# OCSYT/SoftwareRenderer

Measured on AMD Instinct MI355X. Metric: Mfragments/s (depth-tested + textured fragments, whole frame), higher is better.
Workload: dtype f32; 1 GPU; cfg3: 4096x4096, 1000000 triangles in 16 u16 meshes, 2048^2 RGBA8 nearest texture, program Dust2LambertFog, Back/LessEqual/Alpha; pipelining=1, parallelism=1 GPU

## Files before the change

softwarerenderer_amd/csrc/swr_binning.hip.h:

```cpp
#pragma once
#include "swr_device.h"

#define SWR_ORDER_BUCKETS 256

namespace swr {

struct BinArgs {
    const unsigned long long* __restrict__ slot_tb;
    const TriRec* __restrict__ recs;
    uint32_t slot_lo, slot_hi;
    uint32_t spt;
    int tiles_x;
    int band_ty0, band_ty1;
    BandMap band;
    int width, height;
    uint32_t* __restrict__ tile_count;
    const uint32_t* __restrict__ tile_start;
    uint32_t* __restrict__ tile_list;
    uint32_t list_capacity;
    Counters* __restrict__ counters;
    Ctrl* __restrict__ ctrl;
    uint32_t seq;
    uint32_t replayable;
    const unsigned long long* __restrict__ total;
    uint8_t* __restrict__ want;
    uint32_t tpw;
    uint32_t bin_blocks;
    int order_tiles_y;
    const uint8_t* __restrict__ tile_bucket;
    const uint32_t* __restrict__ order_hist;
    uint32_t* __restrict__ order_cursor;
    uint4* __restrict__ tile_order;
};

__device__ __forceinline__ bool pair_may_cover(const float sx[3], const float sy[3], int minX, int maxX, int minY, int maxY,
                                               int tx, int ty, int width, int height, bool is_line) {
    if (is_line) return true;
    const int x0 = tx * SWR_TILE, y0 = ty * SWR_TILE;
    const int startX = max(minX, x0), endX = min(maxX, min(x0 + SWR_TILE - 1, width - 1));
    const int startY = max(minY, y0), endY = min(maxY, min(y0 + SWR_TILE - 1, height - 1));
    if (startX > endX || startY > endY) return false;
    const float ea[3] = { sy[1] - sy[2], sy[2] - sy[0], sy[0] - sy[1] };
    const float eb[3] = { sx[2] - sx[1], sx[0] - sx[2], sx[1] - sx[0] };
    const float rx[3] = { sx[1], sx[2], sx[0] };
    const float ry[3] = { sy[1], sy[2], sy[0] };
    const float fxs = (float)startX, fxe = (float)endX, fys = (float)startY, fye = (float)endY;
    const float lim = 1.0e15f;
    const bool tame = fabsf(sx[0]) < lim && fabsf(sx[1]) < lim && fabsf(sx[2]) < lim && fabsf(sy[0]) < lim && fabsf(sy[1]) < lim && fabsf(sy[2]) < lim;
    if (!tame) return true;
    bool any_neg = false, any_pos = false;
#pragma unroll
    for (int k = 0; k < 3; ++k) {
        const float a = ea[k], b = eb[k];
        const float dxs = fxs - rx[k], dxe = fxe - rx[k], dys = fys - ry[k], dye = fye - ry[k];
        const float ax_s = a * dxs, ax_e = a * dxe, by_s = b * dys, by_e = b * dye;
        const float emax = fmaxf(ax_s, ax_e) + fmaxf(by_s, by_e);
        const float emin = fminf(ax_s, ax_e) + fminf(by_s, by_e);
        const float m = fabsf(a) * fmaxf(fabsf(dxs), fabsf(dxe)) + fabsf(b) * fmaxf(fabsf(dys), fabsf(dye));
        const float delta = m * (64.0f / 16777216.0f);
        any_neg = any_neg || emax < -delta;
        any_pos = any_pos || emin > delta;
    }
    return !(any_neg && any_pos);
}

__device__ __forceinline__ void bin_overflow(const BinArgs& a) {
    a.counters->overflow = 1u;
    if (a.ctrl->host_flag) __hip_atomic_store(a.ctrl->host_flag + 1, 1u, __ATOMIC_RELAXED, __HIP_MEMORY_SCOPE_SYSTEM);
    if (a.replayable) {
        atomicMin(&a.ctrl->first_bad, a.seq);
        atomicMax(&a.ctrl->need, 2ull * (unsigned long long)a.list_capacity + 4096ull);
        __hip_atomic_store(&a.ctrl->poison, 1u, __ATOMIC_RELAXED, __HIP_MEMORY_SCOPE_AGENT);
        if (a.ctrl->host_flag) __hip_atomic_store(a.ctrl->host_flag, 1u, __ATOMIC_RELAXED, __HIP_MEMORY_SCOPE_SYSTEM);
    }
}

__device__ __forceinline__ uint32_t order_bucket(uint32_t w) {
    if (w == 0u) return 0u;
    const int e = 31 - __clz((int)w);
    const uint32_t m = e >= 3 ? ((w >> (e - 3)) & 7u) : ((w << (3 - e)) & 7u);
    return min((uint32_t)(e * 8) + m + 1u, (uint32_t)SWR_ORDER_BUCKETS - 1u);
}
__device__ __forceinline__ uint32_t tile_weight(uint32_t frags, uint32_t pairs) { return frags + 16u * pairs; }

__device__ __forceinline__ uint32_t order_tile_of_thread(uint32_t block, int tiles_x, int tiles_y) {
    const int sbx = (tiles_x + 15) >> 4;
    const int bx = (int)(block % (uint32_t)sbx), by = (int)(block / (uint32_t)sbx);
    const int t = threadIdx.x, q = t >> 6, w = t & 63;
    const int tx = bx * 16 + (q & 1) * 8 + (w & 7), ty = by * 16 + (q >> 1) * 8 + (w >> 3);
    return (tx < tiles_x && ty < tiles_y) ? (uint32_t)(ty * tiles_x + tx) : 0xffffffffu;
}
__host__ __device__ inline uint32_t order_blocks(int tiles_x, int tiles_y) { return (uint32_t)(((tiles_x + 15) / 16) * ((tiles_y + 15) / 16)); }

__device__ __forceinline__ void tile_place_block(const BinArgs& a, uint32_t block, uint32_t* s_suf, uint32_t* s_cnt) {
    const uint32_t t = threadIdx.x;
    s_suf[t] = a.order_hist[t];
    s_cnt[t] = 0u;
    __syncthreads();
    for (uint32_t off = 1; off < (uint32_t)SWR_ORDER_BUCKETS; off <<= 1) {
        const uint32_t v = t + off < (uint32_t)SWR_ORDER_BUCKETS ? s_suf[t + off] : 0u;
        __syncthreads();
        s_suf[t] += v;
        __syncthreads();
    }
    const uint32_t i = order_tile_of_thread(block, a.tiles_x, a.order_tiles_y);
    uint32_t b = 0, rank = 0;
    if (i != 0xffffffffu) {
        b = a.tile_bucket[i];
        rank = atomicAdd(&s_cnt[b], 1u);
    }
    __syncthreads();
    const uint32_t mine = s_cnt[t];
    __syncthreads();
    if (mine) s_cnt[t] = (s_suf[t] - a.order_hist[t]) + atomicAdd(&a.order_cursor[t], mine);
    __syncthreads();
    if (i != 0xffffffffu) {
        const uint32_t n_tiles = (uint32_t)(a.tiles_x * a.order_tiles_y);
        const uint32_t st = a.tile_start[i];
        const unsigned long long nxt = i + 1u < n_tiles ? (unsigned long long)a.tile_start[i + 1u] : *a.total;
        a.tile_order[s_cnt[b] + rank] = make_uint4(i, st, (uint32_t)(nxt - st), 0u);
    }
}

struct SlotData {
    int tminx, tminy, nx, ny;
    float sx[3], sy[3];
    int minX, maxX, minY, maxY;
    bool is_line;
};
__device__ __forceinline__ SlotData slot_none() {
    SlotData s;
    s.tminx = s.tminy = s.nx = s.ny = 0;
    s.sx[0] = s.sx[1] = s.sx[2] = s.sy[0] = s.sy[1] = s.sy[2] = 0.f;
    s.minX = s.minY = 0; s.maxX = s.maxY = -1; s.is_line = false;
    return s;
}
__device__ __forceinline__ bool slot_tiles(const BinArgs& a, unsigned long long tb, SlotData& s) {
    if (tb == SWR_TB_INVALID) return false;
    s.tminx = (int)(tb & 0xffff);
    const int tmaxx = (int)((tb >> 16) & 0xffff);
    s.tminy = max((int)((tb >> 32) & 0xffff), a.band_ty0);
    const int tmaxy = min((int)((tb >> 48) & 0xffff), a.band_ty1 - 1);
    s.nx = tmaxx - s.tminx + 1;
    s.ny = tmaxy - s.tminy + 1;
    if (s.ny <= 0) { s.nx = 0; s.ny = 0; return false; }
    return true;
}
__device__ __forceinline__ SlotData slot_load(const BinArgs& a, uint32_t slot, unsigned long long tb, bool with_rec_small) {
    SlotData s = slot_none();
    if (slot_tiles(a, tb, s) && (with_rec_small || s.nx * s.ny > 8)) {
        const float4* __restrict__ rq = reinterpret_cast<const float4*>(a.recs + slot);
        const float4 r0 = rq[0], r1 = rq[1], r3 = rq[3];
        s.sx[0] = r0.x; s.sx[1] = r0.y; s.sx[2] = r0.z; s.sy[0] = r0.w; s.sy[1] = r1.x; s.sy[2] = r1.y;
        const uint32_t bbx = __float_as_uint(r3.y), bby = __float_as_uint(r3.z);
        s.minX = (int)(bbx & 0xffffu); s.maxX = (int)(bbx >> 16); s.minY = (int)(bby & 0xffffu); s.maxY = (int)(bby >> 16);
        s.is_line = (__float_as_uint(r3.w) & SWR_FLAG_LINE) != 0u;
    }
    return s;
}

template <bool FILL>
__device__ __forceinline__ void bin_big(const BinArgs& a, const SlotData& sd, uint32_t slot, bool big) {
    const int lane = threadIdx.x & 63;
    const int nt = sd.nx * sd.ny;
    unsigned long long med = __ballot(big && nt <= 64);
    while (med) {
        bool want[4];
        uint32_t tile[4], sslot[4], base[4];
#pragma unroll
        for (int j = 0; j < 4; ++j) {
            want[j] = false; tile[j] = 0u; sslot[j] = 0u; base[j] = 0u;
            if (med) {
                const int src = __ffsll((long long)med) - 1;
                med &= med - 1;
                const int s_tminx = __shfl(sd.tminx, src), s_tminy = __shfl(sd.tminy, src);
                const int s_nx = __shfl(sd.nx, src), s_nt = __shfl(nt, src);
                sslot[j] = (uint32_t)__shfl((int)slot, src);
                float bsx[3], bsy[3];
#pragma unroll
                for (int k = 0; k < 3; ++k) { bsx[k] = __shfl(sd.sx[k], src); bsy[k] = __shfl(sd.sy[k], src); }
                const int bminX = __shfl(sd.minX, src), bmaxX = __shfl(sd.maxX, src), bminY = __shfl(sd.minY, src), bmaxY = __shfl(sd.maxY, src);
                const bool b_line = __shfl((int)sd.is_line, src) != 0;
                if (lane < s_nt) {
                    const int ty = s_tminy + lane / s_nx, tx = s_tminx + lane % s_nx;
                    want[j] = band_local_row(a.band, ty) >= 0 && pair_may_cover(bsx, bsy, bminX, bmaxX, bminY, bmaxY, tx, ty, a.width, a.height, b_line);
                    tile[j] = (uint32_t)(band_local_row(a.band, ty) * a.tiles_x + tx);
                }
                if (want[j]) {
                    if (FILL) base[j] = atomicAdd(&a.tile_count[tile[j]], 1u);
                    else atomicAdd(&a.tile_count[tile[j]], 1u);
                }
            }
        }
        if (FILL) {
#pragma unroll
            for (int j = 0; j < 4; ++j) {
                if (want[j]) {
                    const uint32_t at = a.tile_start[tile[j]] + base[j];
                    if (at < a.list_capacity) a.tile_list[at] = sslot[j];
                    else bin_overflow(a);
                }
            }
        }
    }
    unsigned long long m = __ballot(big && nt > 64);
    while (m) {
        const int src = __ffsll((long long)m) - 1;
        m &= m - 1;
        const int s_tminx = __shfl(sd.tminx, src), s_tminy = __shfl(sd.tminy, src);
        const int s_nx = __shfl(sd.nx, src), s_nt = __shfl(nt, src);
        const uint32_t s_slot = (uint32_t)__shfl((int)slot, src);
        float bsx[3], bsy[3];
#pragma unroll
        for (int k = 0; k < 3; ++k) { bsx[k] = __shfl(sd.sx[k], src); bsy[k] = __shfl(sd.sy[k], src); }
        const int bminX = __shfl(sd.minX, src), bmaxX = __shfl(sd.maxX, src), bminY = __shfl(sd.minY, src), bmaxY = __shfl(sd.maxY, src);
        const bool b_line = __shfl((int)sd.is_line, src) != 0;
        for (int i0 = 0; i0 < s_nt; i0 += 64) {
            const int i = i0 + lane;
            bool want = i < s_nt;
            int ty = 0, tx = 0;
            if (want) {
                ty = s_tminy + i / s_nx; tx = s_tminx + i % s_nx;
                want = band_local_row(a.band, ty) >= 0 && pair_may_cover(bsx, bsy, bminX, bmaxX, bminY, bmaxY, tx, ty, a.width, a.height, b_line);
            }
            if (want) {
                const uint32_t tile = (uint32_t)(band_local_row(a.band, ty) * a.tiles_x + tx);
                if (FILL) {
                    const uint32_t at = a.tile_start[tile] + atomicAdd(&a.tile_count[tile], 1u);
                    if (at < a.list_capacity) a.tile_list[at] = s_slot;
                    else bin_overflow(a);
                } else {
                    atomicAdd(&a.tile_count[tile], 1u);
                }
            }
        }
    }
}

#define SWR_BIN_TABLE_LOG2 8
#define SWR_BIN_TABLE (1 << SWR_BIN_TABLE_LOG2)
template <bool FILL>
__device__ __forceinline__ void bin_block_slots(const BinArgs& a, uint32_t slot, unsigned long long tb, uint32_t want_in, uint32_t* s_key, uint32_t* s_val) {
    const SlotData sd = slot_load(a, slot, tb, !FILL);
    const int nt = sd.nx * sd.ny;
    const bool big = nt > 8;
    const int nt_small = big ? 0 : nt;
    if (!__syncthreads_or(nt != 0)) return;
    for (int e = threadIdx.x; e < SWR_BIN_TABLE; e += 256) { s_key[e] = 0u; s_val[e] = 0u; }
    __syncthreads();
    uint32_t packed[8];
    int wtx = sd.tminx, wty = sd.tminy;
    uint32_t wmask = (FILL && nt_small) ? want_in : 0u;
#pragma unroll
    for (int i = 0; i < 8; ++i) {
        packed[i] = 0u;
        if (i < nt_small) {
            bool want;
            if (FILL) want = ((wmask >> i) & 1u) != 0u;
            else {
                want = band_local_row(a.band, wty) >= 0 && pair_may_cover(sd.sx, sd.sy, sd.minX, sd.maxX, sd.minY, sd.maxY, wtx, wty, a.width, a.height, sd.is_line);
                wmask |= want ? (1u << i) : 0u;
            }
            if (want) {
                const uint32_t tile = (uint32_t)(band_local_row(a.band, wty) * a.tiles_x + wtx);
                uint32_t e = (tile * 0x9E3779B1u) >> (32 - SWR_BIN_TABLE_LOG2);
                bool placed = false;
                for (int probe = 0; probe < 16; ++probe) {
                    const uint32_t prev = atomicCAS(&s_key[e], 0u, tile + 1u);
                    if (prev == 0u || prev == tile + 1u) { placed = true; break; }
                    e = (e + 1u) & (SWR_BIN_TABLE - 1u);
                }
                if (placed) {
                    const uint32_t rank = atomicAdd(&s_val[e], 1u);
                    packed[i] = e | (rank << 12) | 0x80000000u;
                } else if (FILL) {
                    const uint32_t at = a.tile_start[tile] + atomicAdd(&a.tile_count[tile], 1u);
                    if (at < a.list_capacity) a.tile_list[at] = slot;
                    else bin_overflow(a);
                } else {
                    atomicAdd(&a.tile_count[tile], 1u);
                }
            }
            ++wtx;
            if (wtx >= sd.tminx + sd.nx) { wtx = sd.tminx; ++wty; }
        }
    }
    if (!FILL && nt_small) a.want[slot] = (uint8_t)wmask;
    __syncthreads();
    for (int e = threadIdx.x; e < SWR_BIN_TABLE; e += 256) {
        const uint32_t key = s_key[e];
        if (key) {
            const uint32_t tile = key - 1u, n = s_val[e];
            if (FILL) s_val[e] = a.tile_start[tile] + atomicAdd(&a.tile_count[tile], n);
            else atomicAdd(&a.tile_count[tile], n);
        }
    }
    if (FILL) {
        __syncthreads();
#pragma unroll
        for (int i = 0; i < 8; ++i) {
            if (packed[i] & 0x80000000u) {
                const uint32_t at = s_val[packed[i] & 0xfffu] + ((packed[i] >> 12) & 0x7ffffu);
                if (at < a.list_capacity) a.tile_list[at] = slot;
                else bin_overflow(a);
            }
        }
    }
    bin_big<FILL>(a, sd, slot, big);
}

template <bool FILL>
__global__ __launch_bounds__(256) void k_bin(BinArgs a) {
    SWR_FRONT_ENTER();
    __shared__ uint32_t s_key[SWR_BIN_TABLE];
    __shared__ uint32_t s_val[SWR_BIN_TABLE];
    if (FILL && batch_poisoned(a.ctrl, a.seq)) return;
    if (FILL && blockIdx.x >= a.bin_blocks) {
        static_assert(SWR_BIN_TABLE >= SWR_ORDER_BUCKETS, "tile_place_block borrows the hash table's LDS");
        tile_place_block(a, blockIdx.x - a.bin_blocks, s_key, s_val);
        return;
    }
    const uint32_t wave_id = (blockIdx.x * 256u + threadIdx.x) >> 6, lane_id = threadIdx.x & 63u;
    const bool has_tri = lane_id < a.tpw;
    const uint32_t first = a.slot_lo + (wave_id * a.tpw + lane_id) * a.spt;
    auto in_round = [&](uint32_t si) { return has_tri && si < a.spt && first + si < a.slot_hi; };
    auto tb_of = [&](uint32_t si) { return in_round(si) ? a.slot_tb[first + si] : SWR_TB_INVALID; };
    auto want_of = [&](uint32_t si) { return (FILL && in_round(si)) ? (uint32_t)a.want[first + si] : 0u; };
    unsigned long long tb = tb_of(0);
    uint32_t wm = want_of(0);
    for (uint32_t si = 0; si < a.spt; ++si) {
        const unsigned long long tb_next = tb_of(si + 1);
        const uint32_t wm_next = want_of(si + 1);
        bin_block_slots<FILL>(a, first + si, tb, wm, s_key, s_val);
        tb = tb_next; wm = wm_next;
    }
}

#define SWR_SCAN_BLOCK 256
__device__ __forceinline__ unsigned long long block_sum(unsigned long long v, unsigned long long* s_part) {
#pragma unroll
    for (int off = 32; off > 0; off >>= 1) {
        unsigned lo = (unsigned)v, hi = (unsigned)(v >> 32);
        v += ((unsigned long long)(unsigned)__shfl_xor((int)hi, off) << 32) | (unsigned)__shfl_xor((int)lo, off);
    }
    if ((threadIdx.x & 63u) == 0u) s_part[threadIdx.x >> 6] = v;
    __syncthreads();
    unsigned long long t = 0;
    for (int w = 0; w < SWR_SCAN_BLOCK / 64; ++w) t += s_part[w];
    return t;
}

__global__ __launch_bounds__(SWR_SCAN_BLOCK) void k_scan_sums(const uint32_t* __restrict__ count, uint32_t n,
                                                    unsigned long long* __restrict__ sums) {
    SWR_FRONT_ENTER();
    __shared__ unsigned long long s_part[SWR_SCAN_BLOCK / 64];
    const uint32_t i = blockIdx.x * (uint32_t)SWR_SCAN_BLOCK + threadIdx.x;
    const unsigned long long t = block_sum(i < n ? count[i] : 0u, s_part);
    if (threadIdx.x == 0) sums[blockIdx.x] = t;
}

__global__ __launch_bounds__(SWR_SCAN_BLOCK) void k_scan_apply(uint32_t* __restrict__ count, uint32_t* __restrict__ start,
                                                     uint32_t n, const unsigned long long* __restrict__ sums,
                                                     unsigned long long* __restrict__ total_out,
                                                     unsigned long long capacity, uint32_t seq, Ctrl* __restrict__ ctrl,
                                                     Counters* __restrict__ counters, int poison_on_overflow,
                                                     const uint32_t* __restrict__ tile_work, uint32_t* __restrict__ order_hist,
                                                     uint8_t* __restrict__ tile_bucket) {
    SWR_FRONT_ENTER();
    __shared__ unsigned long long s_part[SWR_SCAN_BLOCK / 64];
    __shared__ unsigned long long s_wave[SWR_SCAN_BLOCK / 64];
    __shared__ uint32_t s_oh[SWR_ORDER_BUCKETS];
    static_assert(SWR_ORDER_BUCKETS <= SWR_SCAN_BLOCK, "one thread per bucket clears / flushes the block's histogram");
    const uint32_t tid = threadIdx.x, lane = tid & 63u, wv = tid >> 6;
    if (tid < (uint32_t)SWR_ORDER_BUCKETS) s_oh[tid] = 0u;
    unsigned long long mine = 0ull;
    for (uint32_t j = tid; j < blockIdx.x; j += (uint32_t)SWR_SCAN_BLOCK) mine += sums[j];
    const unsigned long long off = block_sum(mine, s_part);
    const uint32_t i = blockIdx.x * (uint32_t)SWR_SCAN_BLOCK + tid;
    const uint32_t c = i < n ? count[i] : 0u;
    if (i < n) {
        const uint32_t ob = order_bucket(tile_weight(tile_work[i], c));
        tile_bucket[i] = (uint8_t)ob;
        atomicAdd(&s_oh[ob], 1u);
    }
    unsigned long long incl = c;
#pragma unroll
    for (int o = 1; o < 64; o <<= 1) {
        unsigned lo = (unsigned)incl, hi = (unsigned)(incl >> 32);
        unsigned long long v = ((unsigned long long)(unsigned)__shfl_up((int)hi, o) << 32) | (unsigned)__shfl_up((int)lo, o);
        if (lane >= (uint32_t)o) incl += v;
    }
    if (lane == 63u) s_wave[wv] = incl;
    __syncthreads();
    if (tid < (uint32_t)SWR_ORDER_BUCKETS && s_oh[tid]) atomicAdd(&order_hist[tid], s_oh[tid]);
    unsigned long long wave_off = 0;
    for (uint32_t w = 0; w < wv; ++w) wave_off += s_wave[w];
    const unsigned long long excl = off + wave_off + incl - c;
    if (i < n) {
        start[i] = (uint32_t)min(excl, 0xffffffffull);
        count[i] = 0u;
    }
    if (blockIdx.x == gridDim.x - 1 && tid == (uint32_t)SWR_SCAN_BLOCK - 1u) {
        const unsigned long long total = excl + c;
        *total_out = total;
        if (total > capacity) {
            if (!poison_on_overflow) return;
            atomicMin(&ctrl->first_bad, seq);
            atomicMax(&ctrl->need, total);
            __hip_atomic_store(&ctrl->poison, 1u, __ATOMIC_RELAXED, __HIP_MEMORY_SCOPE_AGENT);
            if (ctrl->host_flag) __hip_atomic_store(ctrl->host_flag, 1u, __ATOMIC_RELAXED, __HIP_MEMORY_SCOPE_SYSTEM);
        } else if (poison_on_overflow && !batch_poisoned(ctrl, seq)) {
            atomicAdd(&counters->tile_pairs, total);
        }
    }
}

#define SWR_SORT_LDS 2048

__device__ __forceinline__ void cmpx_lds(uint32_t* s, uint32_t i, uint32_t p, uint32_t n) {
    if (p < n) {
        uint32_t a = s[i], b = s[p];
        if (a > b) { s[i] = b; s[p] = a; }
    }
}
__device__ __forceinline__ void cmpx_glb(uint32_t* g, uint32_t i, uint32_t p, uint32_t n) {
    if (p < n) {
        uint32_t a = g[i], b = g[p];
        if (a > b) { g[i] = b; g[p] = a; }
    }
}

#define SWR_SORT_TPB 1
#define SWR_SORT_TPW 4
#define SWR_SORT_WAVE_SYNC() do { __builtin_amdgcn_fence(__ATOMIC_ACQ_REL, "workgroup"); __builtin_amdgcn_wave_barrier(); } while (0)
__device__ __forceinline__ void sort_tile(uint32_t n, uint32_t start, uint32_t* __restrict__ tile_list, uint32_t tile,
                                          uint32_t* __restrict__ pair_tile, uint32_t* s_keys, uint32_t key_in) {
    if (n == 0) return;
    const uint32_t lane = threadIdx.x & 63u;
    for (uint32_t i = lane; i < n; i += 64) pair_tile[start + i] = tile;
    if (n < 2) return;
    uint32_t* seg = tile_list + start;

    if (n <= 64) {
        uint32_t key = lane < n ? key_in : 0xffffffffu;
#define SWR_CMPX(other_expr, lower_cond) { const uint32_t other = (uint32_t)(other_expr); \
                                            key = (lower_cond) ? min(key, other) : max(key, other); }
#define SWR_DPP(ctrl) __builtin_amdgcn_update_dpp(0, (int)key, ctrl, 0xf, 0xf, false)
#define SWR_XOR1  SWR_CMPX(SWR_DPP(0xB1), (lane & 1u) == 0u)
#define SWR_XOR2  SWR_CMPX(SWR_DPP(0x4E), (lane & 2u) == 0u)
#define SWR_XOR4  { const int up = SWR_DPP(0x124), dn = SWR_DPP(0x12C);               \
                    SWR_CMPX((lane & 4u) ? up : dn, (lane & 4u) == 0u) }
#define SWR_XOR8  SWR_CMPX(SWR_DPP(0x128), (lane & 8u) == 0u)
#define SWR_XOR16 SWR_CMPX(__shfl((int)key, (int)(lane ^ 16u)), (lane & 16u) == 0u)
        SWR_XOR1
        SWR_CMPX(SWR_DPP(0x1B), (lane & 2u) == 0u) SWR_XOR1
        SWR_CMPX(SWR_DPP(0x141), (lane & 4u) == 0u) SWR_XOR2 SWR_XOR1
        SWR_CMPX(SWR_DPP(0x140), (lane & 8u) == 0u) SWR_XOR4 SWR_XOR2 SWR_XOR1
        SWR_CMPX(__shfl((int)key, (int)(lane ^ 31u)), (lane & 16u) == 0u) SWR_XOR8 SWR_XOR4 SWR_XOR2 SWR_XOR1
        SWR_CMPX(__shfl((int)key, (int)(lane ^ 63u)), (lane & 32u) == 0u) SWR_XOR16 SWR_XOR8 SWR_XOR4 SWR_XOR2 SWR_XOR1
#undef SWR_XOR16
#undef SWR_XOR8
#undef SWR_XOR4
#undef SWR_XOR2
#undef SWR_XOR1
#undef SWR_DPP
#undef SWR_CMPX
        if (lane < n) seg[lane] = key;
        return;
    }

    uint32_t m = 1;
    while (m < n) m <<= 1;
    const bool in_lds = n <= SWR_SORT_LDS;
    uint32_t* buf = in_lds ? s_keys : seg;
    if (in_lds) {
        for (uint32_t i = lane; i < n; i += 64) s_keys[i] = seg[i];
        SWR_SORT_WAVE_SYNC();
    }
    for (uint32_t k = 2; k <= m; k <<= 1) {
        for (uint32_t t = lane; t < (m >> 1); t += 64) {
            uint32_t blk = t / (k >> 1), off = t % (k >> 1);
            uint32_t i = blk * k + off, p = blk * k + (k - 1 - off);
            if (i < n) { if (in_lds) cmpx_lds(buf, i, p, n); else cmpx_glb(buf, i, p, n); }
        }
        SWR_SORT_WAVE_SYNC();
        for (uint32_t j = k >> 2; j > 0; j >>= 1) {
            for (uint32_t t = lane; t < (m >> 1); t += 64) {
                uint32_t i = 2 * j * (t / j) + (t % j), p = i + j;
                if (i < n) { if (in_lds) cmpx_lds(buf, i, p, n); else cmpx_glb(buf, i, p, n); }
            }
            SWR_SORT_WAVE_SYNC();
        }
    }
    if (in_lds) {
        for (uint32_t i = lane; i < n; i += 64) seg[i] = s_keys[i];
    }
}

__global__ __launch_bounds__(64 * SWR_SORT_TPB) void k_sort_tiles(const uint32_t* __restrict__ tile_start,
                                                   const uint32_t* __restrict__ tile_count,
                                                   uint32_t* __restrict__ tile_list, uint32_t n_tiles,
                                                   uint32_t* __restrict__ pair_tile, const Ctrl* __restrict__ ctrl, uint32_t seq,
                                                   const uint4* __restrict__ tile_order ) {
    SWR_FRONT_ENTER();
    __shared__ uint32_t s_keys_all[SWR_SORT_TPB][SWR_SORT_LDS];
    static_assert(sizeof(s_keys_all) <= SWR_FRONT_MAX_LDS, "k_sort_tiles must fit beside the raster kernel (swr_device.h)");
    if (batch_poisoned(ctrl, seq)) return;
    static_assert(SWR_SORT_TPW <= 64, "one lane per tile of the wave fetches its count and start");
    const uint32_t first = (blockIdx.x * SWR_SORT_TPB + (threadIdx.x >> 6)) * SWR_SORT_TPW;
    const uint32_t lane = threadIdx.x & 63u;
    const uint32_t waves = gridDim.x * SWR_SORT_TPB, entry = (first / SWR_SORT_TPW) + lane * waves;
    const bool mine = lane < SWR_SORT_TPW && entry < n_tiles;
    const uint4 desc_l = mine ? tile_order[entry] : make_uint4(0u, 0u, 0u, 0u);
    const uint32_t tile_l = desc_l.x;
    const uint32_t cnt_l = desc_l.z, st_l = desc_l.y;
    uint32_t keys[SWR_SORT_TPW];
#pragma unroll
    for (int t = 0; t < SWR_SORT_TPW; ++t) {
        const uint32_t n = (uint32_t)__builtin_amdgcn_readlane((int)cnt_l, t), start = (uint32_t)__builtin_amdgcn_readlane((int)st_l, t);
        keys[t] = (lane < n && n <= 64u) ? tile_list[start + lane] : 0xffffffffu;
    }
#pragma unroll
    for (int t = 0; t < SWR_SORT_TPW; ++t) {
        const uint32_t n = (uint32_t)__builtin_amdgcn_readlane((int)cnt_l, t), start = (uint32_t)__builtin_amdgcn_readlane((int)st_l, t);
        sort_tile(n, start, tile_list, (uint32_t)__builtin_amdgcn_readlane((int)tile_l, t), pair_tile, s_keys_all[threadIdx.x >> 6], keys[t]);
        SWR_SORT_WAVE_SYNC();
    }
}

}
```

softwarerenderer_amd/csrc/swr_device.h:

```cpp
#pragma once

#ifndef __HIPCC_RTC__
#include <hip/hip_runtime.h>
#include <stdint.h>
#endif
#include "swr.h"

#ifndef SWR_NUMERICS_FMA
#define SWR_NUMERICS_FMA 0
#endif
#define SWR_NM_TRANSFORM_FMA        1u
#define SWR_NM_TRANSFORM_NORMAL_FMA 2u
#ifndef SWR_DOT_PAIRWISE
#define SWR_DOT_PAIRWISE 0
#endif

#define SWR_PROG_CUSTOM 5
#define SWR_TILE 16
#define SWR_FLOAT_MINVALUE (-3.40282347e+38f)
#define SWR_EPSILON 1e-6f
#define SWR_FLAG_INTERP 0x80000000u
#define SWR_FLAG_LINE   0x40000000u
#define SWR_FLAG_FASTDIV 0x20000000u
#define SWR_FLAG_SIMPLE 0x10000000u
#define SWR_DRAW_MASK   0x0fffffffu
#define SWR_INFO_SIMPLE 0x80000000u

#define SWR_TB_INVALID 0xffffffffffffffffull

#define SWR_FRONT_MAX_LDS 10240
#define SWR_FRONT_MAX_VGPRS 96
#define SWR_RASTER_MAX_VGPRS 104
#define SWR_FRONT_ENTER() __builtin_amdgcn_s_setprio(3)
#define SWR_GEOM_BLOCK 128

namespace swr {

struct VOut {
    float clip[4];
    float color[4];
    float uv[2];
    float wn[3];
    float wpos[3];
};
static_assert(sizeof(VOut) == 64, "VOut must be 64 bytes");

struct TriRec {
    float sx[3], sy[3];
    float depth[3];
    float inv_area;
    uint32_t vref[3];
    uint32_t bbox_x;
    uint32_t bbox_y;
    uint32_t draw_flags;
};
static_assert(sizeof(TriRec) == 64, "TriRec must be 64 bytes");

struct DrawParams {
    float model[16], view[16], proj[16];
    swr_uniforms u;
    const swr_vertex* verts;
    const uint16_t* idx;
    const uint8_t* tex;
    int tex_w, tex_h;
    int program, cull, depth_test, blend;
    uint32_t n_verts, n_tris;
    uint32_t vert_base;
    uint32_t tri_base;
    float fog_r1;
    float tex_wf, tex_hf;
    float fog_den;
    uint32_t frag_draw;
    uint32_t nm_flags;
};
static_assert(offsetof(DrawParams, fog_den) == offsetof(DrawParams, fog_r1) + 12, "k_vertex writes fog_den three floats after fog_r1");

struct Counters {
    unsigned long long triangles_in, triangles_setup, triangles_clipped;
    unsigned long long fragments_tested, fragments_shaded, fragments_written;
    unsigned long long tile_pairs;
    unsigned int overflow;
    unsigned int pad;
};

struct Ctrl {
    uint32_t poison;
    uint32_t first_bad;
    unsigned long long need;
    uint32_t* host_flag;
};
__device__ __forceinline__ bool batch_poisoned(const Ctrl* __restrict__ c, uint32_t seq) { return c->first_bad <= seq; }

struct FrameParams {
    int width, height;
    int tiles_x, tiles_y;
    int band_ty0, band_ty1;
    int band_y0;
    int band_rows;
    int il_k, il_world, il_rank;
    int band_tile_rows;
    float near_clip;
};

struct BandMap { int ty0, ty1, il_k, il_world, il_rank; };
__host__ __device__ __forceinline__ int band_local_row(const BandMap& b, int ty) {
    if (b.il_k <= 0) return (ty >= b.ty0 && ty < b.ty1) ? ty - b.ty0 : -1;
    const int stripe = ty / b.il_k;
    if (stripe % b.il_world != b.il_rank) return -1;
    return (stripe / b.il_world) * b.il_k + (ty - stripe * b.il_k);
}
__host__ __device__ __forceinline__ int band_global_row(const BandMap& b, int local) {
    if (b.il_k <= 0) return b.ty0 + local;
    const int ls = local / b.il_k;
    return (ls * b.il_world + b.il_rank) * b.il_k + (local - ls * b.il_k);
}
__host__ __device__ __forceinline__ BandMap band_map(const FrameParams& fp) {
    BandMap b; b.ty0 = fp.band_ty0; b.ty1 = fp.band_ty1; b.il_k = fp.il_k; b.il_world = fp.il_world; b.il_rank = fp.il_rank;
    return b;
}

__device__ __forceinline__ bool is_neg_bits(float f) { return (__float_as_uint(f) >> 31) != 0u; }
__device__ __forceinline__ bool is_nan(float f) { return f != f; }
__device__ __forceinline__ bool is_nan_or_inf(float f) { return (__float_as_uint(f) & 0x7f800000u) == 0x7f800000u; }

__device__ __forceinline__ int f2i(float f) {
    int r;
    asm("v_cvt_i32_f32 %0, %1" : "=v"(r) : "v"(f));
    return r;
}
__device__ __forceinline__ float mathf_min(float a, float b) {
    if (a != b) { if (!is_nan(a)) return a < b ? a : b; return a; }
    return is_neg_bits(a) ? a : b;
}
__device__ __forceinline__ float mathf_max(float a, float b) {
    if (a != b) { if (!is_nan(a)) return b < a ? a : b; return a; }
    return is_neg_bits(b) ? a : b;
}
__device__ __forceinline__ float math_clamp(float v, float lo, float hi) {
    if (v < lo) return lo;
    else if (v > hi) return hi;
    return v;
}

__device__ __forceinline__ float rcp_refined(float d) {
    const float r0 = __builtin_amdgcn_rcpf(d);
    const float e = __builtin_fmaf(-d, r0, 1.0f);
    return __builtin_fmaf(e, r0, r0);
}
__device__ __forceinline__ float div_core(float n, float d, float r1) {
    const float q0 = n * r1;
    const float e2 = __builtin_fmaf(-d, q0, n);
    const float q1 = __builtin_fmaf(e2, r1, q0);
    const float e3 = __builtin_fmaf(-d, q1, n);
    return __builtin_fmaf(e3, r1, q1);
}
#define SWR_DIV_LO_BITS 0x2B800000u
#define SWR_DIV_HI_BITS 0x53800000u
__device__ __forceinline__ bool div_operand_safe(float v) {
    return __builtin_fabsf(v) >= 0x1p-40f && __builtin_fabsf(v) <= 0x1p40f;
}
__device__ __forceinline__ bool div_operands_safe3(float a, float b, float c) {
    const uint32_t ua = __float_as_uint(a) & 0x7fffffffu, ub = __float_as_uint(b) & 0x7fffffffu, uc = __float_as_uint(c) & 0x7fffffffu;
    return min(min(ua, ub), uc) >= SWR_DIV_LO_BITS && max(max(ua, ub), uc) <= SWR_DIV_HI_BITS;
}
__device__ __forceinline__ bool div_operands_safe3_arith(float a, float b, float c) {
    const float fa = __builtin_fabsf(a), fb = __builtin_fabsf(b), fc = __builtin_fabsf(c);
    const float sum = (fa + fb) + fc;
    const float lo = __builtin_fminf(__builtin_fminf(fa, fb), fc);
    return lo >= 0x1p-40f && sum <= 0x1p40f;
}
#define SWR_RCP_HI_BITS 0x69000000u
__device__ __forceinline__ float recip_core(float d) {
    const float r1 = rcp_refined(d);
    const float e2 = __builtin_fmaf(-d, r1, 1.0f);
    const float q1 = __builtin_fmaf(e2, r1, r1);
    const float e3 = __builtin_fmaf(-d, q1, 1.0f);
    return __builtin_fmaf(e3, r1, q1);
}
__device__ __forceinline__ float sqrt_core(float x) {
    const float s = __builtin_amdgcn_sqrtf(x);
    const float sd = __uint_as_float(__float_as_uint(s) - 1u), su = __uint_as_float(__float_as_uint(s) + 1u);
    const float rd = __builtin_fmaf(-sd, s, x), ru = __builtin_fmaf(-su, s, x);
    float r = rd <= 0.0f ? sd : s;
    r = ru > 0.0f ? su : r;
    return r;
}

template <bool FUSED>
__device__ __forceinline__ float nm_madd(float a, float b, float c) {
    if (FUSED) return __builtin_fmaf(a, b, c);
    float p = a * b;
    return p + c;
}
template <bool FUSED>
__device__ __forceinline__ void vec4_transform_t(const float v[4], const float* __restrict__ m, float out[4]) {
#pragma unroll
    for (int j = 0; j < 4; ++j) {
        float r = m[j] * v[0];
        r = nm_madd<FUSED>(m[4 + j], v[1], r);
        r = nm_madd<FUSED>(m[8 + j], v[2], r);
        r = nm_madd<FUSED>(m[12 + j], v[3], r);
        out[j] = r;
    }
}
template <bool FUSED>
__device__ __forceinline__ void vec3_transform_normal_t(const float n[3], const float* __restrict__ m, float out[3]) {
#pragma unroll
    for (int j = 0; j < 3; ++j) {
        float r = m[j] * n[0];
        r = nm_madd<FUSED>(m[4 + j], n[1], r);
        r = nm_madd<FUSED>(m[8 + j], n[2], r);
        out[j] = r;
    }
}
__device__ __forceinline__ void vec4_transform(const float v[4], const float* __restrict__ m, float out[4], bool fused) {
    if (fused) vec4_transform_t<true>(v, m, out); else vec4_transform_t<false>(v, m, out);
}
__device__ __forceinline__ void vec3_transform_normal(const float n[3], const float* __restrict__ m, float out[3], bool fused) {
    if (fused) vec3_transform_normal_t<true>(n, m, out); else vec3_transform_normal_t<false>(n, m, out);
}
__device__ __forceinline__ float dot3(float ax, float ay, float az, float bx, float by, float bz) {
#if SWR_DOT_PAIRWISE == 1
    const float p = ax * bx + ay * by, q = az * bz + 0.0f;
    return p + q;
#elif SWR_DOT_PAIRWISE == 2
    const float p = ax * bx + az * bz, q = ay * by + 0.0f;
    return p + q;
#else
    return (ax * bx + ay * by) + az * bz;
#endif
}
__device__ __forceinline__ float nm_lerp(float a, float b, float t) {
#if SWR_NUMERICS_FMA
    return __builtin_fmaf(a, 1.0f - t, b * t);
#else
    float x = a * (1.0f - t);
    float y = b * t;
    return x + y;
#endif
}

__device__ __forceinline__ float edge_function(float ax, float ay, float bx, float by, float cx, float cy) {
    float p = (cx - ax) * (by - ay);
    float q = (cy - ay) * (bx - ax);
    return p - q;
}

__device__ __forceinline__ bool depth_func(int test, float nd, float od) {
    switch (test) {
    case SWR_DEPTH_LESSEQUAL:    return nd >= od;
    case SWR_DEPTH_LESS:         return nd > od;
    case SWR_DEPTH_GREATER:      return nd < od;
    case SWR_DEPTH_GREATEREQUAL: return nd <= od;
    case SWR_DEPTH_EQUAL:        return fabsf(nd - od) < SWR_EPSILON;
    case SWR_DEPTH_NOTEQUAL:     return fabsf(nd - od) >= SWR_EPSILON;
    default:                     return true;
    }
}

__device__ __forceinline__ float4 blend(float4 s, float4 d, int mode) {
    float4 o;
    switch (mode) {
    case SWR_BLEND_ALPHA: {
        float a = s.w, ia = 1.0f - s.w;
        float x;
        x = s.x * a; o.x = x + d.x * ia;
        x = s.y * a; o.y = x + d.y * ia;
        x = s.z * a; o.z = x + d.z * ia;
        x = s.w * a; o.w = x + d.w * ia;
        return o; }
    case SWR_BLEND_ADDITIVE:
        o.x = mathf_min(s.x + d.x, 1.0f); o.y = mathf_min(s.y + d.y, 1.0f);
        o.z = mathf_min(s.z + d.z, 1.0f); o.w = mathf_min(s.w + d.w, 1.0f);
        return o;
    case SWR_BLEND_MULTIPLY:
        o.x = s.x * d.x; o.y = s.y * d.y; o.z = s.z * d.z; o.w = s.w * d.w;
        return o;
    default:
        return s;
    }
}

__device__ __forceinline__ bool line_test(float p0x, float p0y, float p1x, float p1y, int x, int y, float& t_out) {
    const float dx = p1x - p0x, dy = p1y - p0y;
    const float len_sq = dx * dx + dy * dy;
    const float px = (float)x + 0.5f - p0x, py = (float)y + 0.5f - p0y;
    float t = 0.0f;
    if (len_sq > 0) t = (px * dx + py * dy) / len_sq;
    t = mathf_max(0.0f, mathf_min(1.0f, t));
    const float cx = p0x + t * dx, cy = p0y + t * dy;
    const float ddx = ((float)x + 0.5f) - cx, ddy = ((float)y + 0.5f) - cy;
    const float dist_sq = ddx * ddx + ddy * ddy;
    t_out = t;
    return dist_sq <= 0.5f * 0.5f;
}

__device__ __forceinline__ float4 texture_unpack(uint32_t p) {
    const float inv255 = 1.0f / 255.0f;
    float4 o;
    o.x = (float)(p & 0xffu) * inv255;
    o.y = (float)((p >> 8) & 0xffu) * inv255;
    o.z = (float)((p >> 16) & 0xffu) * inv255;
    o.w = (float)(p >> 24) * inv255;
    return o;
}
__device__ __forceinline__ uint32_t texture_nearest_index(int w, int h, float wf, float hf, float tu, float tv) {
    float u = tu - (float)f2i(tu);
    float v = tv - (float)f2i(tv);
    u += (u < 0) ? 1.0f : 0.0f;
    v += (v < 0) ? 1.0f : 0.0f;
    int x = f2i(u * wf);
    int y = f2i(v * hf);
    if ((uint32_t)x >= (uint32_t)w) { x = (x == w) ? 0 : x % w; if (x < 0) x += w; }
    if ((uint32_t)y >= (uint32_t)h) { y = (y == h) ? 0 : y % h; if (y < 0) y += h; }
    return (uint32_t)y * (uint32_t)w + (uint32_t)x;
}
__device__ __forceinline__ uint32_t texture_nearest_index(int w, int h, float tu, float tv) {
    return texture_nearest_index(w, h, (float)w, (float)h, tu, tv);
}
__device__ __forceinline__ float4 texture_sample(const uint8_t* __restrict__ tex, int w, int h, float tu, float tv) {
    return texture_unpack(reinterpret_cast<const uint32_t*>(tex)[texture_nearest_index(w, h, tu, tv)]);
}

template <bool BLOCKED>
__device__ __forceinline__ uint32_t bilinear_texel_offset(int w, int x, int y) {
    if (BLOCKED) return ((((uint32_t)y >> 2) * ((uint32_t)w >> 2) + ((uint32_t)x >> 2)) << 4) + (((uint32_t)y & 3u) << 2) + ((uint32_t)x & 3u);
    return (uint32_t)y * (uint32_t)w + (uint32_t)x;
}
template <bool BLOCKED>
__device__ __forceinline__ float4 texture_sample_bilinear(const uint8_t* __restrict__ tex, int w, int h, float tu, float tv) {
    const float x = tu * (float)w - 0.5f, y = tv * (float)h - 0.5f;
    const float x0 = floorf(x), y0 = floorf(y);
    const float fx = x - x0, fy = y - y0;
    int ix0 = f2i(x0) % w; if (ix0 < 0) ix0 += w;
    int iy0 = f2i(y0) % h; if (iy0 < 0) iy0 += h;
    const int ix1 = ix0 + 1 == w ? 0 : ix0 + 1, iy1 = iy0 + 1 == h ? 0 : iy0 + 1;
    const uint32_t* __restrict__ t32 = reinterpret_cast<const uint32_t*>(tex);
    const uint32_t p00 = t32[bilinear_texel_offset<BLOCKED>(w, ix0, iy0)];
    const uint32_t p10 = t32[bilinear_texel_offset<BLOCKED>(w, ix1, iy0)];
    const uint32_t p01 = t32[bilinear_texel_offset<BLOCKED>(w, ix0, iy1)];
    const uint32_t p11 = t32[bilinear_texel_offset<BLOCKED>(w, ix1, iy1)];
    const float inv255 = 1.0f / 255.0f;
    float o[4];
#pragma unroll
    for (int c = 0; c < 4; ++c) {
        const float c00 = (float)((p00 >> (8 * c)) & 0xffu) * inv255, c10 = (float)((p10 >> (8 * c)) & 0xffu) * inv255;
        const float c01 = (float)((p01 >> (8 * c)) & 0xffu) * inv255, c11 = (float)((p11 >> (8 * c)) & 0xffu) * inv255;
        const float top = c00 * (1.0f - fx) + c10 * fx;
        const float bot = c01 * (1.0f - fx) + c11 * fx;
        o[c] = top * (1.0f - fy) + bot * fy;
    }
    return make_float4(o[0], o[1], o[2], o[3]);
}
__device__ __forceinline__ float4 texture_fetch(const uint8_t* __restrict__ tex, int w_signed, int h_signed, float tu, float tv) {
    if (h_signed >= 0) return texture_sample(tex, w_signed, h_signed, tu, tv);
    return w_signed < 0 ? texture_sample_bilinear<true>(tex, -w_signed, -h_signed, tu, tv) : texture_sample_bilinear<false>(tex, w_signed, -h_signed, tu, tv);
}

}
```

softwarerenderer_amd/csrc/swr_flush.h:

```cpp
#pragma once
#include "swr_raster_select.h"

namespace {
int kernel_class(int program) { return program == SWR_PROG_DEBUG_VARYINGS || program >= SWR_PROG_USER_BASE ? program : 0; }

void destroy_mesh(swr_mesh* m) {
    if (m->d_verts) (void)hipFree(m->d_verts);
    if (m->d_idx) (void)hipFree(m->d_idx);
    if (m->d_bounds) (void)hipFree(m->d_bounds);
    delete m;
}
const size_t kMeshPoolBytes = (size_t)1 << 30;
void trim_mesh_pool(swr_context* c) {
    while (c->mesh_pool_bytes > kMeshPoolBytes && !c->mesh_pool.empty()) {
        swr_mesh* m = c->mesh_pool.front();
        c->mesh_pool.erase(c->mesh_pool.begin());
        c->mesh_pool_bytes -= m->cap_verts + m->cap_idx;
        destroy_mesh(m);
    }
}
void pool_mesh(swr_context* c, swr_mesh* m) {
    c->mesh_pool.push_back(m);
    c->mesh_pool_bytes += m->cap_verts + m->cap_idx;
    if (c->mesh_pool_bytes > 2 * kMeshPoolBytes) trim_mesh_pool(c);
}
void free_garbage(swr_context* c) {
    for (swr_mesh* m : c->garbage) pool_mesh(c, m);
    c->garbage.clear();
    c->prog_garbage.clear();
    trim_mesh_pool(c);
}

int validate_locked(swr_context* c);

int drain_streams(swr_context* c) {
    SWR_HIP(c, hipStreamSynchronize(c->stream));
    if (c->front_stream) SWR_HIP(c, hipStreamSynchronize(c->front_stream));
    for (auto& s : c->sets) s.raster_pending = false;
    c->f_tail_pending = c->r_front_pending = false;
    return SWR_OK;
}

int sync_locked(swr_context* c) {
    ++c->host_syncs;
    int rc = drain_streams(c);
    if (rc) return rc;
    rc = validate_locked(c);
    collect_spans(c);
    free_garbage(c);
    for (auto& fs : c->slots) fs.busy = false;
    return rc;
}

enum { MODE_SYNC = 0, MODE_ASYNC = 1 };
struct UploadLayout { size_t off_vb, off_tb, off_bp, off_vis, off_consts, bytes; };
static UploadLayout upload_layout(size_t nd, size_t v_blocks, size_t t_blocks, bool any_cull, bool user) {
    const auto r256 = [](size_t x) { return (x + 255) & ~(size_t)255; };
    UploadLayout u;
    u.off_vb = r256(nd * sizeof(DrawParams));
    u.off_tb = r256(u.off_vb + v_blocks * sizeof(BlockMap));
    u.off_bp = r256(u.off_tb + t_blocks * sizeof(BlockMap));
    u.off_vis = r256(u.off_bp + (any_cull ? nd * sizeof(void*) : 0));
    const size_t vis_end = u.off_vis + (any_cull ? nd * 4 : 0);
    u.off_consts = r256(vis_end);
    u.bytes = user ? u.off_consts + nd * 64 * sizeof(float) : vis_end;
    return u;
}
template <class T> T* at(void* base, size_t off) { return reinterpret_cast<T*>(static_cast<char*>(base) + off); }

struct OrderView { uint4* tile_order; uint32_t* tile_work; uint32_t* hist; uint32_t* cursor; uint8_t* tile_bucket; };
static size_t order_bytes(uint32_t n_tiles) { return (size_t)n_tiles * (sizeof(uint4) + 4 + 1 + 4) + 2 * SWR_ORDER_BUCKETS * 4; }
static OrderView order_view(RasterSet& S, uint32_t n_tiles) {
    uint4* order = S.d_order.as<uint4>();
    uint32_t* work = reinterpret_cast<uint32_t*>(order + n_tiles), *hist = work + n_tiles, *cursor = hist + SWR_ORDER_BUCKETS;
    return { order, work, hist, cursor, reinterpret_cast<uint8_t*>(cursor + SWR_ORDER_BUCKETS) };
}

struct Pass {
    const Batch& b;
    RasterSet& S;
    hipStream_t F;
    int mode;
    bool cc, cd;
    UploadLayout up = {};
};

static bool b_needs_vnorm(const Batch& b) { return !b.draws.empty() && kernel_class(b.draws[0].p.program) != 0; }
static bool b_has_user_program(const Batch& b) { return !b.draws.empty() && b.draws[0].p.program >= SWR_PROG_USER_BASE; }
static bool b_has_user_vertex(const Batch& b) { return b_has_user_program(b) && b.draws[0].prog && b.draws[0].prog->vertex_fn; }
const unsigned long long kMaxPairs = 1ull << 30;

size_t pair_capacity(const swr_context* c) {
    size_t cap = std::min(c->d_tile_list.cap / 4, c->d_pair_tile.cap / 4);
    for (int i = 0; i < (c->pipelining ? 2 : 1); ++i) {
        const RasterSet& s = c->sets[i];
        cap = std::min(cap, std::min(std::min(s.d_masks.cap / 32, s.d_pcounts.cap / 8), s.d_pair_refs.cap / 16));
    }
    return cap;
}
int ensure_pairs(swr_context* c, size_t n) {
    int rc;
    if ((rc = ensure(c, c->d_tile_list, n * 4))) return rc;
    if ((rc = ensure(c, c->d_pair_tile, n * 4))) return rc;
    for (int i = 0; i < (c->pipelining ? 2 : 1); ++i) {
        RasterSet& s = c->sets[i];
        if ((rc = ensure(c, s.d_masks, n * 32))) return rc;
        if ((rc = ensure(c, s.d_pair_refs, n * 16))) return rc;
        if ((rc = ensure(c, s.d_pcounts, n * 8 + 64))) return rc;
    }
    return SWR_OK;
}

int run_clear(swr_context* c, const Batch& b, bool& cc, bool& cd) {
    size_t n = band_pixels(c);
    if (n && (cc || cd)) {
        ScopedSpan sp(c, ST_CLEAR);
        int blocks = (int)std::min<size_t>((n + 255) / 256, 2048 * 8);
        float4 rgba = make_float4(b.clear_rgba[0], b.clear_rgba[1], b.clear_rgba[2], b.clear_rgba[3]);
        hipLaunchKernelGGL(k_clear, dim3(blocks), dim3(256), 0, c->stream, b.color, b.depth, n, rgba,
                           cc ? 1 : 0, cd ? 1 : 0, (const Ctrl*)c->d_ctrl.as<Ctrl>(), b.seq);
        SWR_HIP(c, hipGetLastError());
    }
    cc = cd = false;
    return SWR_OK;
}

int launch_raster(swr_context* c, Pass& P, uint32_t n_tiles);

int bin_and_raster(swr_context* c, Pass& P, uint32_t lo, uint32_t hi, bool counts_clear = false) {
    const uint32_t n_tiles = (uint32_t)c->tiles_x * (uint32_t)c->band_tile_rows;
    if (n_tiles == 0 || lo >= hi) return SWR_OK;
    int rc;
    const Batch& b = P.b; RasterSet& S = P.S;
    const hipStream_t F = P.F; const int mode = P.mode;
    const Ctrl* ctrl = c->d_ctrl.as<Ctrl>();
    unsigned long long* d_total = c->d_total.as<unsigned long long>();
    const OrderView ov = order_view(S, n_tiles);
    BinArgs ba;
    ba.slot_tb = c->d_slot_tb.as<unsigned long long>();
    ba.recs = S.d_recs.as<TriRec>();
    ba.slot_lo = lo; ba.slot_hi = hi;
    ba.spt = b.wireframe ? 6u : 2u;
    ba.width = c->W; ba.height = c->H;
    ba.tiles_x = c->tiles_x; ba.band_ty0 = c->band_ty0; ba.band_ty1 = c->band_ty1;
    ba.band = host_band_map(c);
    ba.tile_count = S.d_tile_count.as<uint32_t>();
    ba.tile_start = S.d_tile_start.as<uint32_t>();
    ba.tile_list = c->d_tile_list.as<uint32_t>();
    ba.list_capacity = (uint32_t)std::min<size_t>(pair_capacity(c), 0xffffffffu);
    ba.counters = c->d_counters.as<Counters>();
    ba.ctrl = c->d_ctrl.as<Ctrl>();
    ba.seq = b.seq; ba.replayable = mode == MODE_ASYNC ? 1u : 0u;
    ba.total = c->d_total.as<unsigned long long>();
    ba.want = c->d_want.as<uint8_t>();
    const uint32_t bin_threads = (hi - lo + ba.spt - 1u) / ba.spt;
    ba.tpw = 64u;
    while (ba.tpw > 4u && bin_threads < ba.tpw * 1024u) ba.tpw >>= 1;
    const uint32_t bin_blocks = (bin_threads + 4u * ba.tpw - 1u) / (4u * ba.tpw);
    {
        ScopedSpan sp(c, ST_BIN, F);
        if (!counts_clear) {
            SWR_HIP(c, hipMemsetAsync(ba.tile_count, 0, (size_t)n_tiles * 4, F));
            SWR_HIP(c, hipMemsetAsync(ov.hist, 0, 2 * SWR_ORDER_BUCKETS * 4, F));
        }
        hipLaunchKernelGGL(k_bin<false>, dim3(bin_blocks), dim3(256), 0, F, ba);
        const unsigned scan_blocks = (n_tiles + (unsigned)SWR_SCAN_BLOCK - 1u) / (unsigned)SWR_SCAN_BLOCK;
        unsigned long long* sums = d_total + 32;
        hipLaunchKernelGGL(k_scan_sums, dim3(scan_blocks), dim3(SWR_SCAN_BLOCK), 0, F, (const uint32_t*)ba.tile_count, n_tiles, sums);
        const unsigned long long cap = mode == MODE_ASYNC ? (unsigned long long)ba.list_capacity : ~0ull;
        hipLaunchKernelGGL(k_scan_apply, dim3(scan_blocks), dim3(SWR_SCAN_BLOCK), 0, F, ba.tile_count,
                           S.d_tile_start.as<uint32_t>(), n_tiles, (const unsigned long long*)sums, d_total,
                           cap, b.seq, c->d_ctrl.as<Ctrl>(), c->d_counters.as<Counters>() + 64,
                           mode == MODE_ASYNC ? 1 : 0, (const uint32_t*)ov.tile_work, ov.hist, ov.tile_bucket);
        SWR_HIP(c, hipGetLastError());
    }
    uint32_t cover_items = ba.list_capacity;
    if (mode == MODE_SYNC) {
        unsigned long long total = 0;
        SWR_HIP(c, hipMemcpyAsync(&total, d_total, 8, hipMemcpyDeviceToHost, F));
        SWR_HIP(c, hipStreamSynchronize(F));
        if (total > kMaxPairs && hi - lo > 2) {
            uint32_t mid = lo + (((hi - lo) / 2u) & ~1u);
            if (mid == lo) mid = lo + 2;
            if ((rc = bin_and_raster(c, P, lo, mid))) return rc;
            return bin_and_raster(c, P, mid, hi);
        }
        if (total == 0) return run_clear(c, b, P.cc, P.cd);
        if (total > 0xffffffffull) return fail(c, SWR_ERR_UNSUPPORTED, "a single triangle covers more tile pairs than one round can hold");
        c->host_tile_pairs += total;
        if ((rc = ensure_pairs(c, (size_t)std::min<unsigned long long>(total + total / 4 + 4096, std::max(total, kMaxPairs))))) return rc;
        ba.tile_list = c->d_tile_list.as<uint32_t>();
        ba.list_capacity = (uint32_t)std::min<size_t>(pair_capacity(c), 0xffffffffu);
        cover_items = (uint32_t)total;
    }
    {
        ScopedSpan sp(c, ST_BIN, F);
        BinArgs bf = ba;
        if (mode == MODE_ASYNC && c->debug_fill_capacity) bf.list_capacity = std::min(bf.list_capacity, c->debug_fill_capacity);
        bf.bin_blocks = bin_blocks;
        bf.order_tiles_y = c->band_tile_rows;
        bf.tile_bucket = ov.tile_bucket; bf.order_hist = ov.hist; bf.order_cursor = ov.cursor; bf.tile_order = ov.tile_order;
        hipLaunchKernelGGL(k_bin<true>, dim3(bin_blocks + order_blocks(c->tiles_x, c->band_tile_rows)), dim3(256), 0, F, bf);
        SWR_HIP(c, hipGetLastError());
    }
    {
        ScopedSpan sp(c, ST_SORT, F);
        hipLaunchKernelGGL(k_sort_tiles, dim3((n_tiles + SWR_SORT_TPB * SWR_SORT_TPW - 1u) / (SWR_SORT_TPB * SWR_SORT_TPW)), dim3(64 * SWR_SORT_TPB), 0, F, S.d_tile_start.as<uint32_t>(),
                           S.d_tile_count.as<uint32_t>(), c->d_tile_list.as<uint32_t>(), n_tiles, c->d_pair_tile.as<uint32_t>(), ctrl, b.seq,
                           (const uint4*)ov.tile_order);
        SWR_HIP(c, hipGetLastError());
    }
    if (cover_items) {
        ScopedSpan sp(c, ST_COVER, F);
        CoverArgs ca;
        ca.recs = S.d_recs.as<TriRec>();
        ca.tile_list = c->d_tile_list.as<uint32_t>();
        ca.pair_tile = c->d_pair_tile.as<uint32_t>();
        ca.masks = S.d_masks.as<uint4>();
        ca.info = S.d_pcounts.as<uint2>();
        ca.refs = S.d_pair_refs.as<uint4>();
        ca.n_pairs = d_total;
        ca.ctrl = ctrl; ca.seq = b.seq;
        ca.fp = frame_params(c, b.near_clip);
        ca.dbg = d_total + 8;
        const dim3 cg((unsigned)((((cover_items + (uint32_t)SWR_COVER_BLOCK - 1u) / (uint32_t)SWR_COVER_BLOCK) + 7u) & ~7u)), cb(SWR_COVER_BLOCK);
        if (b.wireframe) hipLaunchKernelGGL(k_cover<true>, cg, cb, 0, F, ca);
        else hipLaunchKernelGGL(k_cover<false>, cg, cb, 0, F, ca);
        SWR_HIP(c, hipGetLastError());
    }
    if (F != c->stream) {
        SWR_HIP(c, hipEventRecord(S.front_done, F));
        SWR_HIP(c, hipStreamWaitEvent(c->stream, S.front_done, 0));
    } else if (c->pipelining && mode == MODE_ASYNC) {
        SWR_HIP(c, hipEventRecord(c->r_front_ev, c->stream));
        c->r_front_pending = true;
    }
    if ((rc = launch_raster(c, P, n_tiles))) return rc;
    if (c->pipelining && S.raster_done) {
        SWR_HIP(c, hipEventRecord(S.raster_done, c->stream));
        S.raster_pending = true;
    }
    return SWR_OK;
}

int launch_raster(swr_context* c, Pass& P, uint32_t n_tiles) {
    const Batch& b = P.b; RasterSet& S = P.S;
    const OrderView ov = order_view(S, n_tiles);
    ScopedSpan sp(c, ST_RASTER);
    RasterArgs ra;
    ra.fp = frame_params(c, b.near_clip);
    ra.recs = S.d_recs.as<TriRec>();
    ra.vout = S.d_vout.as<VOut>();
    ra.vout_bytes = (uint32_t)std::min<size_t>(S.d_vout.cap, 0xfffffff0u);
    ra.vnorm = b_needs_vnorm(b) ? S.d_vnorm.as<float4>() : nullptr;
    ra.user_consts = b_has_user_program(b) ? at<const float>(S.d_upload.p, P.up.off_consts) : nullptr;
    ra.draws = at<const DrawParams>(S.d_upload.p, 0);
    ra.tile_start = S.d_tile_start.as<uint32_t>();
    ra.tile_count = S.d_tile_count.as<uint32_t>();
    ra.pair_refs = S.d_pair_refs.as<uint4>();
    ra.color = b.color; ra.depth = b.depth;
    ra.tile_stats = c->d_tile_stats.as<uint32_t>();
    memcpy(ra.clear_rgba, b.clear_rgba, 16);
    ra.clear_color_on = P.cc ? 1 : 0;
    ra.clear_depth_on = P.cd ? 1 : 0;
    ra.tile_order = ov.tile_order;
    ra.tile_work = ov.tile_work;
    ra.n_tiles = n_tiles;
    ra.dbg = c->d_total.as<unsigned long long>() + 8;
    ra.ctrl = c->d_ctrl.as<Ctrl>(); ra.seq = b.seq;
    RasterTraits traits;
    traits.wireframe = b.wireframe;
    for (auto& d : b.draws) traits.add(d.p.program, d.p.blend, d.p.depth_test);
    ra.depth_only_grows = traits.depth_only_grows ? 1 : 0;
    const RasterKernel kernel = select_raster_kernel(traits);
    using RasterFn = void (*)(RasterArgs, const uint4*, const uint2*);
    static const RasterFn table[] = {
        k_raster_c<false, true, SWR_PROG_DEBUG_VARYINGS, -1, -1, true>,
        k_raster_c<false, true, SWR_PROG_DEBUG_VARYINGS>,
        k_raster_c<true, true>,
        k_raster_c<false, true, -1, -1, -1, true>,
        k_raster_c<false, true, SWR_PROG_PHONG_4POINT, SWR_BLEND_ALPHA, SWR_DEPTH_LESSEQUAL>,
        k_raster_c<false, true>,
        k_raster_c<false, false, SWR_PROG_DUST2_LAMBERT_FOG, SWR_BLEND_ALPHA, SWR_DEPTH_LESSEQUAL>,
        k_raster_c<false, false, SWR_PROG_GOURAUD, SWR_BLEND_ALPHA, SWR_DEPTH_LESSEQUAL>,
        k_raster_c<false, false>,
    };
    static_assert(sizeof table / sizeof table[0] == (size_t)RasterKernel::user, "one kernel per built-in RasterKernel, in its order");
    const dim3 g((n_tiles + 511u) & ~511u), t(64);
    const uint4* mk = (const uint4*)S.d_masks.as<uint4>();
    const uint2* pc = (const uint2*)S.d_pcounts.as<uint2>();
    if (kernel == RasterKernel::user || kernel == RasterKernel::user_none) {
        void* args[] = { &ra, &mk, &pc };
        hipFunction_t fn = b.draws[0].prog->fn[kernel == RasterKernel::user_none ? 1 : 0];
        SWR_HIP(c, hipModuleLaunchKernel(fn, g.x, 1, 1, t.x, 1, 1, 0, c->stream, args, nullptr));
    } else {
        hipLaunchKernelGGL(table[(int)kernel], g, t, 0, c->stream, ra, mk, pc);
    }
    SWR_HIP(c, hipGetLastError());
    P.cc = P.cd = false;
    return SWR_OK;
}

struct BatchGeometry {
    std::vector<DrawParams> hp;
    std::vector<BlockMap> vblocks, tblocks;
    uint64_t V = 0, T = 0; bool any_cull = false;
};
static BatchGeometry batch_geometry(const Batch& b) {
    BatchGeometry g;
    const size_t nd = b.draws.size();
    g.hp.resize(nd);
    std::vector<uint32_t> frag_reps;
    for (size_t i = 0; i < nd; ++i) {
        DrawParams p = b.draws[i].p;
        p.vert_base = (uint32_t)g.V; p.tri_base = (uint32_t)g.T;
        for (uint32_t f = 0; f < p.n_verts; f += SWR_GEOM_BLOCK) g.vblocks.push_back({ (uint32_t)i, f });
        for (uint32_t f = 0; f < p.n_tris; f += SWR_GEOM_BLOCK) g.tblocks.push_back({ (uint32_t)i, f });
        g.V += p.n_verts; g.T += p.n_tris;
        g.any_cull = g.any_cull || b.draws[i].frustum_cull;
        p.frag_draw = (uint32_t)i;
        for (uint32_t j : frag_reps) {
            const DrawParams& q = g.hp[j];
            if (q.program == p.program && q.blend == p.blend && q.depth_test == p.depth_test && q.tex == p.tex && q.tex_w == p.tex_w &&
                q.tex_h == p.tex_h && memcmp(&q.u, &p.u, sizeof p.u) == 0 &&
                (p.program < SWR_PROG_USER_BASE || *b.draws[j].uconsts == *b.draws[i].uconsts)) { p.frag_draw = j; break; }
        }
        if (p.frag_draw == (uint32_t)i && p.n_verts > 0 && !b.draws[i].frustum_cull && frag_reps.size() < 64) frag_reps.push_back((uint32_t)i);
        g.hp[i] = p;
    }
    return g;
}

int launch_geometry(swr_context* c, const Pass& P, const BatchGeometry& g, uint32_t n_tiles, int count_stats) {
    const Batch& b = P.b; RasterSet& S = P.S; const hipStream_t F = P.F;
    const UserProg* vprog = b_has_user_vertex(b) ? b.draws[0].prog.get() : nullptr;
    const auto launch = [&](hipFunction_t user_fn, const void* builtin, size_t blocks, void** args) {
        return user_fn ? hipModuleLaunchKernel(user_fn, (unsigned)blocks, 1, 1, SWR_GEOM_BLOCK, 1, 1, 0, F, args, nullptr)
                       : hipLaunchKernel(builtin, dim3((unsigned)blocks), dim3(SWR_GEOM_BLOCK), args, 0, F);
    };
    const uint32_t nd = (uint32_t)b.draws.size();
    const DrawParams* d_draws = at<const DrawParams>(S.d_upload.p, 0);
    const BlockMap* d_vblocks = at<const BlockMap>(S.d_upload.p, P.up.off_vb);
    const BlockMap* d_tblocks = at<const BlockMap>(S.d_upload.p, P.up.off_tb);
    const uint32_t* d_visible = nullptr;
    if (g.any_cull) {
        ScopedSpan sp(c, ST_VERTEX, F);
        uint32_t* vis = at<uint32_t>(S.d_upload.p, P.up.off_vis);
        hipLaunchKernelGGL(k_frustum_cull, dim3((nd + 63) / 64), dim3(64), 0, F, d_draws,
                           at<const float4* const>(S.d_upload.p, P.up.off_bp), nd, vis);
        SWR_HIP(c, hipGetLastError());
        d_visible = vis;
    }
    float4* a_vnorm = b_needs_vnorm(b) ? S.d_vnorm.as<float4>() : (float4*)nullptr;
    if (!g.vblocks.empty()) {
        ScopedSpan sp(c, ST_VERTEX, F);
        VOut* a_vout = S.d_vout.as<VOut>();
        float* a_fog = at<float>(S.d_upload.p, offsetof(DrawParams, fog_r1));
        uint32_t* a_zero = S.d_tile_count.as<uint32_t>();
        uint32_t a_n_zero = n_tiles;
        uint32_t* a_hist = order_view(S, n_tiles).hist;
        const float* a_consts = at<const float>(S.d_upload.p, P.up.off_consts);
        void* args[] = { &d_draws, &d_vblocks, &a_vout, &d_visible, &a_fog, &a_vnorm, &a_zero, &a_n_zero, &a_hist, &a_consts };
        SWR_HIP(c, launch(vprog ? vprog->vertex_fn : nullptr, (const void*)k_vertex, g.vblocks.size(), args));
    }
    {
        ScopedSpan sp(c, ST_SETUP, F);
        FrameParams fp = frame_params(c, b.near_clip);
        const VOut* a_vout = S.d_vout.as<VOut>();
        VOut* a_pool = S.d_vout.as<VOut>() + g.V;
        uint32_t a_pool_base = (uint32_t)g.V;
        TriRec* a_recs = S.d_recs.as<TriRec>();
        unsigned long long* a_tb = c->d_slot_tb.as<unsigned long long>();
        Counters* a_counters = c->d_counters.as<Counters>();
        const Ctrl* a_ctrl = c->d_ctrl.as<Ctrl>();
        uint32_t a_seq = b.seq;
        int a_count = count_stats, a_wire = b.wireframe ? 1 : 0;
        void* args[] = { &d_draws, &d_tblocks, &a_vout, &a_pool, &a_pool_base, &a_recs, &a_tb, &fp, &a_counters, &a_ctrl, &a_seq,
                         &a_count, &a_wire, &d_visible, &a_vnorm };
        SWR_HIP(c, launch(vprog ? vprog->setup_fn : nullptr, (const void*)k_setup, g.tblocks.size(), args));
    }
    return SWR_OK;
}

int execute_batch(swr_context* c, const Batch& b, int mode, int count_stats) {
    bool cc = b.clear_color, cd = b.clear_depth;
    if (b.draws.empty()) return run_clear(c, b, cc, cd);
    int rc;
    if ((rc = ensure_front_stream(c))) return rc;
    const BatchGeometry g = batch_geometry(b);
    const uint64_t V = g.V, T = g.T;
    const uint32_t n_tiles = (uint32_t)c->tiles_x * (uint32_t)c->band_tile_rows;
    const bool piped = mode == MODE_ASYNC && (c->pipelining == 1 || (c->pipelining == 2 && (T <= c->pipeline_max_tris ||
                                                                                            n_tiles <= c->pipeline_max_tiles)));
    Pass P{ b, c->sets[c->pipelining ? (b.seq & 1u) : 0u], piped ? c->front_stream : c->stream, mode, cc, cd };
    RasterSet& S = P.S; const hipStream_t F = P.F;
    if (c->pipelining && mode != MODE_ASYNC) SWR_HIP(c, hipStreamSynchronize(c->front_stream));
    if (c->pipelining && mode == MODE_ASYNC) {
        if (!piped && c->f_tail_pending) {
            SWR_HIP(c, hipEventRecord(c->f_tail_ev, c->front_stream));
            SWR_HIP(c, hipStreamWaitEvent(c->stream, c->f_tail_ev, 0));
            c->f_tail_pending = false;
        }
        if (piped && c->r_front_pending) {
            SWR_HIP(c, hipStreamWaitEvent(c->front_stream, c->r_front_ev, 0));
            c->r_front_pending = false;
        }
        if (piped) c->f_tail_pending = true;
    }
    const uint64_t spt = b.wireframe ? 6 : 2;
    if (V + 4 * T >= (1ull << 26) || spt * T >= 0xffffffffull)
        return fail(c, SWR_ERR_UNSUPPORTED, "internal error: a batch beyond 2^26 vertex-stage records reached execute_batch (record_draw flushes before)");
    if (T == 0) return run_clear(c, b, cc, cd);
    if (n_tiles > (1u << 20))
        return fail(c, SWR_ERR_UNSUPPORTED, "more than 2^20 tiles in one band (a target beyond 16384 x 16384): render it in tile-row bands (swr_set_band)");

    P.up = upload_layout(b.draws.size(), g.vblocks.size(), g.tblocks.size(), g.any_cull, b_has_user_program(b));
    if ((rc = ensure(c, S.d_upload, P.up.bytes))) return rc;
    if ((rc = ensure(c, S.d_vout, (size_t)(V + 4 * T) * sizeof(VOut)))) return rc;
    if (b_needs_vnorm(b) && (rc = ensure(c, S.d_vnorm, S.d_vout.cap / 4))) return rc;
    if ((rc = ensure(c, S.d_recs, (size_t)(spt * T) * sizeof(TriRec)))) return rc;
    if ((rc = ensure(c, c->d_slot_tb, (size_t)(spt * T) * 8))) return rc;
    if ((rc = ensure(c, c->d_want, (size_t)(spt * T) + 64))) return rc;
    if ((rc = ensure(c, S.d_tile_count, (size_t)n_tiles * 4))) return rc;
    if ((rc = ensure(c, S.d_tile_start, (size_t)n_tiles * 4))) return rc;
    if ((rc = ensure(c, S.d_order, order_bytes(n_tiles)))) return rc;
    if (c->tile_stats_tiles != n_tiles) {
        if (c->tile_stats_tiles) {
            hipLaunchKernelGGL(k_reduce_tile_stats, dim3(1), dim3(1024), 0, c->stream, c->d_tile_stats.as<uint32_t>(),
                               (uint32_t)c->tile_stats_tiles, c->d_total.as<unsigned long long>() + 4, 1);
            SWR_HIP(c, hipGetLastError());
        }
        if ((rc = ensure(c, c->d_tile_stats, (size_t)n_tiles * 12))) return rc;
        SWR_HIP(c, hipMemsetAsync(c->d_tile_stats.p, 0, (size_t)n_tiles * 12, c->stream));
        c->tile_stats_tiles = n_tiles;
    }
    if (piped && S.raster_pending) SWR_HIP(c, hipStreamWaitEvent(F, S.raster_done, 0));
    if (S.hist_tiles != n_tiles) {
        SWR_HIP(c, hipMemsetAsync(order_view(S, n_tiles).tile_work, 0, (size_t)n_tiles * 4, F));
        S.hist_tiles = n_tiles;
    }
    const size_t nd = b.draws.size();
    char* stage = (char*)slot_acquire(c, P.up.bytes);
    if (!stage) return fail(c, SWR_ERR_OOM, "hipHostMalloc failed for the upload staging block");
    memcpy(stage, g.hp.data(), nd * sizeof(DrawParams));
    if (!g.vblocks.empty()) memcpy(stage + P.up.off_vb, g.vblocks.data(), g.vblocks.size() * sizeof(BlockMap));
    memcpy(stage + P.up.off_tb, g.tblocks.data(), g.tblocks.size() * sizeof(BlockMap));
    if (g.any_cull) {
        const float4** bp = at<const float4*>(stage, P.up.off_bp);
        for (size_t i = 0; i < nd; ++i) bp[i] = b.draws[i].frustum_cull ? b.draws[i].mesh->d_bounds : nullptr;
    }
    if (b_has_user_program(b)) {
        float* uc = at<float>(stage, P.up.off_consts);
        for (size_t i = 0; i < nd; ++i) memcpy(uc + 64 * i, b.draws[i].uconsts->data(), 64 * sizeof(float));
    }
    SWR_HIP(c, hipMemcpyAsync(S.d_upload.p, stage, P.up.bytes, hipMemcpyHostToDevice, F));
    if ((rc = launch_geometry(c, P, g, n_tiles, count_stats))) return rc;
    const bool counts_clear = !g.vblocks.empty() && n_tiles != 0;
    rc = bin_and_raster(c, P, 0, (uint32_t)(spt * T), counts_clear);
    slot_submit(c);
    if (rc) return rc;
    if (c->pipelining && mode != MODE_ASYNC) SWR_HIP(c, hipStreamSynchronize(c->stream));
    if (P.cc || P.cd) return run_clear(c, b, P.cc, P.cd);
    return SWR_OK;
}

void retire_batch(swr_context* c, Batch& b, bool complete = false) {
    for (auto& d : b.draws) {
        if (d.mesh && d.mesh->transient) { if (complete) pool_mesh(c, d.mesh); else c->garbage.push_back(d.mesh); }
        if (d.prog && !complete) c->prog_garbage.push_back(std::move(d.prog));
    }
    b.draws.clear();
}

int check_list_overflow(swr_context* c) {
    if (!c->host_poison || !((volatile uint32_t*)c->host_poison)[1]) return SWR_OK;
    c->host_poison[1] = 0;
    return fail(c, SWR_ERR_HIP, "internal error: a (triangle, tile) pair did not fit its tile list and was dropped (Counters::overflow)");
}

int reset_ctrl(swr_context* c) {
    Ctrl fresh; fresh.poison = 0; fresh.first_bad = 0xffffffffu; fresh.need = 0; fresh.host_flag = c->host_poison;
    SWR_HIP(c, hipMemcpy(c->d_ctrl.p, &fresh, sizeof fresh, hipMemcpyHostToDevice));
    return SWR_OK;
}

int validate_locked(swr_context* c) {
    if (c->inflight.empty()) return check_list_overflow(c);
    int rc = SWR_OK;
    if (*(volatile uint32_t*)c->host_poison) {
        Ctrl h;
        SWR_HIP(c, hipMemcpy(&h, c->d_ctrl.p, sizeof h, hipMemcpyDeviceToHost));
        *c->host_poison = 0;
        c->host_poison[1] = 0;
        if ((rc = reset_ctrl(c))) return rc;
        std::vector<Batch> todo;
        todo.swap(c->inflight);
        c->replays++;
        for (auto& b : todo) {
            if (!rc && b.seq >= h.first_bad) {
                rc = execute_batch(c, b, MODE_SYNC, b.seq != h.first_bad);
                retire_batch(c, b);
            } else {
                retire_batch(c, b, true);
            }
        }
        if (!rc) rc = drain_streams(c);
        if (!rc) rc = check_list_overflow(c);
        return rc;
    }
    for (auto& b : c->inflight) retire_batch(c, b, true);
    c->inflight.clear();
    return check_list_overflow(c);
}

int flush_locked(swr_context* c) {
    if (c->W <= 0 || c->H <= 0 || band_pixels(c) == 0) {
        for (auto& d : c->draws) if (d.mesh && d.mesh->transient) c->garbage.push_back(d.mesh);
        c->draws.clear(); c->pend_verts = c->pend_tris = 0;
        c->pend_clear_color = c->pend_clear_depth = false;
        return SWR_OK;
    }
    if (c->draws.empty() && !c->pend_clear_color && !c->pend_clear_depth) return SWR_OK;
    Batch b;
    b.draws.swap(c->draws);
    b.clear_color = c->pend_clear_color; b.clear_depth = c->pend_clear_depth;
    memcpy(b.clear_rgba, c->clear_rgba, 16);
    b.near_clip = c->near_clip;
    b.wireframe = c->debug_mode == SWR_DEBUG_WIREFRAME;
    if (b.wireframe && b_needs_vnorm(b)) {
        for (auto& d : b.draws) if (d.mesh && d.mesh->transient) c->garbage.push_back(d.mesh);
        c->pend_verts = c->pend_tris = 0;
        return fail(c, SWR_ERR_UNSUPPORTED, b_has_user_program(b) ? "user programs are not available in DebugMode.Wireframe"
                                                                   : "SWR_PROG_DEBUG_VARYINGS is not available in DebugMode.Wireframe");
    }
    b.seq = c->next_seq++;
    b.color = c->color; b.depth = c->depth;
    c->pend_clear_color = c->pend_clear_depth = false;
    c->pend_verts = c->pend_tris = 0;
    if (!b.draws.empty()) c->totals.flushes++;
    const bool optimistic = !c->sync_flush && pair_capacity(c) > 0;
    int rc = execute_batch(c, b, optimistic ? MODE_ASYNC : MODE_SYNC, 1);
    if (optimistic && !rc) {
        c->inflight.push_back(std::move(b));
        if (c->inflight.size() >= 64) {
            if ((rc = drain_streams(c))) return rc;
            rc = validate_locked(c);
        }
    } else {
        retire_batch(c, b);
    }
    return rc;
}

int flush_and_sync_locked(swr_context* c) {
    int rc = flush_locked(c);
    return rc ? rc : sync_locked(c);
}

int ensure_bounds(swr_context* c, swr_mesh* m) {
    if (m->bounds_ready) return SWR_OK;
    if (!m->d_bounds) SWR_HIP(c, hipMalloc((void**)&m->d_bounds, sizeof(float4)));
    hipLaunchKernelGGL(k_bounding_sphere, dim3(1), dim3(1024), 0, use_front_stream(c), (const swr_vertex*)m->d_verts, (uint32_t)m->n_verts, m->d_bounds);
    SWR_HIP(c, hipGetLastError());
    m->bounds_ready = true;
    return SWR_OK;
}

static bool band_rejects(const swr_context* c, const swr_mesh* m, const float* model, const float* view, const float* proj) {
    if (!m->has_box || c->il_k > 0 || (c->band_ty0 <= 0 && c->band_ty1 >= c->tiles_y)) return false;
    double mv[16], M[16], amv[16], A[16];
    for (int r = 0; r < 4; ++r)
        for (int k = 0; k < 4; ++k) {
            double a = 0, b = 0;
            for (int j = 0; j < 4; ++j) { a += (double)model[r * 4 + j] * (double)view[j * 4 + k]; b += std::fabs((double)model[r * 4 + j]) * std::fabs((double)view[j * 4 + k]); }
            mv[r * 4 + k] = a; amv[r * 4 + k] = b;
        }
    for (int r = 0; r < 4; ++r)
        for (int k = 0; k < 4; ++k) {
            double a = 0, b = 0;
            for (int j = 0; j < 4; ++j) { a += mv[r * 4 + j] * (double)proj[j * 4 + k]; b += amv[r * 4 + j] * std::fabs((double)proj[j * 4 + k]); }
            M[r * 4 + k] = a; A[r * 4 + k] = b;
        }
    const double u16 = 16.0 / 16777216.0;
    double smin = 1e300, smax = -1e300, ey = 0, ew = 0, wmin = 1e300, ndc_abs = 0;
    for (int corner = 0; corner < 8; ++corner) {
        const double x = (corner & 1) ? m->box_hi[0] : m->box_lo[0];
        const double y = (corner & 2) ? m->box_hi[1] : m->box_lo[1];
        const double z = (corner & 4) ? m->box_hi[2] : m->box_lo[2];
        const double cy = x * M[1] + y * M[5] + z * M[9] + M[13];
        const double cw = x * M[3] + y * M[7] + z * M[11] + M[15];
        const double sy_abs = std::fabs(x) * A[1] + std::fabs(y) * A[5] + std::fabs(z) * A[9] + A[13];
        const double sw_abs = std::fabs(x) * A[3] + std::fabs(y) * A[7] + std::fabs(z) * A[11] + A[15];
        if (!std::isfinite(cy) || !std::isfinite(cw) || !std::isfinite(sy_abs) || !std::isfinite(sw_abs)) return false;
        ey = std::max(ey, u16 * sy_abs); ew = std::max(ew, u16 * sw_abs);
        if (!(cw > 0)) return false;
        wmin = std::min(wmin, cw);
        const double ndc = cy / cw;
        ndc_abs = std::max(ndc_abs, std::fabs(ndc));
        const double sy = (1.0 - (ndc * 0.5 + 0.5)) * (double)c->H;
        if (!std::isfinite(sy)) return false;
        smin = std::min(smin, sy); smax = std::max(smax, sy);
    }
    if (!(wmin - ew > 1e-6 * wmin)) return false;
    const double margin = 2.0 + 0.5 * (double)c->H * (ey + ndc_abs * ew) / (wmin - ew);
    if (!std::isfinite(margin)) return false;
    const double y0 = (double)band_y0(c), y1 = (double)std::min(c->H, c->band_ty1 * SWR_TILE);
    return smax + margin < y0 || smin - margin > y1;
}

int record_draw(swr_context* c, swr_mesh* mesh, const float* model, const float* view, const float* proj,
                int program, const swr_uniforms* u, const swr_texture* tex, int cull, int depth_test, int blend, bool frustum_cull = false) {
    if (!mesh || !model || !view || !proj) return fail(c, SWR_ERR_INVALID_ARG, "null argument to render_mesh");
    std::shared_ptr<UserProg> uprog;
    if (program >= SWR_PROG_USER_BASE) {
        auto it = c->progs.find(program);
        if (it == c->progs.end()) return fail(c, SWR_ERR_INVALID_ARG, "unknown or destroyed user program id");
        if (c->debug_mode == SWR_DEBUG_WIREFRAME)
            return fail(c, SWR_ERR_UNSUPPORTED, "user programs are not available in DebugMode.Wireframe");
        uprog = it->second;
    } else if (program < SWR_PROG_FLAT_COLOR || program > SWR_PROG_DEBUG_VARYINGS) {
        return fail(c, SWR_ERR_INVALID_ARG, "unknown program id");
    }
    if ((program == SWR_PROG_DUST2_LAMBERT_FOG || program == SWR_PROG_PHONG_4POINT) && !u)
        return fail(c, SWR_ERR_INVALID_ARG, "this program needs a uniform block");
    if (cull < 0 || cull > 2 || depth_test < 0 || depth_test > 7 || blend < 0 || blend > 3)
        return fail(c, SWR_ERR_INVALID_ARG, "enum value out of range");
    if (c->W <= 0 || c->H <= 0) return SWR_OK;
    const int n_tris = mesh->n_idx / 3;
    if (n_tris == 0) return SWR_OK;
    if (!(uprog && uprog->vertex_fn) && band_rejects(c, mesh, model, view, proj)) return SWR_OK;
    if ((uint64_t)mesh->n_verts + 4 * (uint64_t)n_tris >= (1ull << 26))
        return fail(c, SWR_ERR_UNSUPPORTED, "mesh exceeds 2^26 vertex-stage records (vertices + 4 x triangles: about 16.7 M triangles): split it");
    if (c->pend_verts + (uint64_t)mesh->n_verts + 4 * (c->pend_tris + (uint64_t)n_tris) >= (1ull << 26)) {
        int rc = flush_locked(c); if (rc) return rc;
    }
    if (!c->draws.empty() && kernel_class(c->draws.back().p.program) != kernel_class(program)) {
        int rc = flush_locked(c); if (rc) return rc;
    }
    DrawCmd d;
    memset(&d.p, 0, sizeof d.p);
    memcpy(d.p.model, model, 64); memcpy(d.p.view, view, 64); memcpy(d.p.proj, proj, 64);
    if (u) d.p.u = *u;
    d.p.verts = mesh->d_verts; d.p.idx = mesh->d_idx;
    d.p.tex = tex ? tex->d_rgba : nullptr;
    d.p.tex_w = tex ? tex->w : 0; d.p.tex_h = tex ? (tex->bilinear ? -tex->h : tex->h) : 0;
    if (tex && tex->bilinear && tex->d_blocked) { d.p.tex = tex->d_blocked; d.p.tex_w = -tex->w; }
    d.p.tex_wf = tex ? (float)tex->w : 0.0f; d.p.tex_hf = tex ? (float)tex->h : 0.0f;
    d.p.program = program; d.p.cull = cull; d.p.depth_test = depth_test; d.p.blend = blend;
    d.p.n_verts = (uint32_t)mesh->n_verts; d.p.n_tris = (uint32_t)n_tris;
    d.p.nm_flags = c->nm_flags;
    d.mesh = mesh;
    d.frustum_cull = frustum_cull;
    if (uprog) {
        d.uconsts = std::make_shared<const std::vector<float>>(uprog->constants, uprog->constants + 64);
        d.prog = std::move(uprog);
    }
    if (frustum_cull) { int rc = ensure_bounds(c, mesh); if (rc) return rc; }
    c->draws.push_back(d);
    c->pend_verts += mesh->n_verts; c->pend_tris += n_tris;
    return SWR_OK;
}

int make_mesh(swr_context* c, const swr_vertex* v, int nv, const uint16_t* idx, int ni, bool transient, swr_mesh** out) {
    if (nv < 0 || ni < 0 || (nv > 0 && !v) || (ni > 0 && !idx) || !out) return fail(c, SWR_ERR_INVALID_ARG, "bad mesh arguments");
    const int used = (ni / 3) * 3;
    for (int i = 0; i < used; ++i)
        if ((int)idx[i] >= nv) return fail(c, SWR_ERR_INVALID_ARG, "index out of range (C#: IndexOutOfRangeException)");
    swr_mesh* m = nullptr;
    if (transient) {
        size_t best = (size_t)-1;
        for (size_t i = 0; i < c->mesh_pool.size(); ++i) {
            swr_mesh* q = c->mesh_pool[i];
            if (q->cap_verts >= (size_t)nv * sizeof(swr_vertex) && q->cap_idx >= (size_t)ni * 2 + 8 &&
                (best == (size_t)-1 || q->cap_verts + q->cap_idx < c->mesh_pool[best]->cap_verts + c->mesh_pool[best]->cap_idx)) best = i;
        }
        if (best != (size_t)-1) {
            m = c->mesh_pool[best];
            c->mesh_pool.erase(c->mesh_pool.begin() + (std::ptrdiff_t)best);
            c->mesh_pool_bytes -= m->cap_verts + m->cap_idx;
            m->bounds_ready = false; m->has_box = false;
        }
    }
    if (!m) m = new swr_mesh();
    m->n_verts = nv; m->n_idx = ni; m->transient = transient;
    if (nv > 0) {
        bool ok = true;
        for (int k = 0; k < 3; ++k) { m->box_lo[k] = v[0].position[k]; m->box_hi[k] = v[0].position[k]; }
        for (int i = 0; i < nv; ++i)
            for (int k = 0; k < 3; ++k) {
                const float p = v[i].position[k];
                if (!(p == p)) ok = false;
                m->box_lo[k] = std::min(m->box_lo[k], p); m->box_hi[k] = std::max(m->box_hi[k], p);
            }
        m->has_box = ok;
    }
    hipError_t e = hipSuccess;
    if (nv && m->cap_verts < (size_t)nv * sizeof(swr_vertex)) {
        e = hipMalloc((void**)&m->d_verts, (size_t)nv * sizeof(swr_vertex));
        if (e == hipSuccess) m->cap_verts = (size_t)nv * sizeof(swr_vertex);
    }
    if (e == hipSuccess && ni && m->cap_idx < (size_t)ni * 2 + 8) {
        e = hipMalloc((void**)&m->d_idx, (size_t)ni * 2 + 8);
        if (e == hipSuccess) m->cap_idx = (size_t)ni * 2 + 8;
    }
    if (e == hipSuccess && nv) e = hipMemcpyAsync(m->d_verts, v, (size_t)nv * sizeof(swr_vertex), hipMemcpyHostToDevice, use_front_stream(c));
    if (e == hipSuccess && ni) e = hipMemcpyAsync(m->d_idx, idx, (size_t)ni * 2, hipMemcpyHostToDevice, use_front_stream(c));
    if (e != hipSuccess) {
        destroy_mesh(m);
        c->err = std::string("mesh upload failed: ") + hipGetErrorString(e);
        return e == hipErrorOutOfMemory ? SWR_ERR_OOM : SWR_ERR_HIP;
    }
    *out = m;
    return SWR_OK;
}

int present_is_stale(swr_context* c, int slot, bool& stale) {
    stale = false;
    if (!*(volatile uint32_t*)c->host_poison) return SWR_OK;
    Ctrl h;
    SWR_HIP(c, hipMemcpy(&h, c->d_ctrl.p, sizeof h, hipMemcpyDeviceToHost));
    stale = h.first_bad <= c->present_seq[slot];
    return SWR_OK;
}
}
```

softwarerenderer_amd/csrc/swr_geometry.hip.h:

```cpp
#pragma once
#include "swr_device.h"

namespace swr {

struct BlockMap { uint32_t draw; uint32_t first; };

#ifndef SWR_USER_VERTEX
__global__ __launch_bounds__(SWR_GEOM_BLOCK) void k_vertex(const DrawParams* __restrict__ draws,
                                                const BlockMap* __restrict__ blocks,
                                                VOut* __restrict__ vout, const uint32_t* __restrict__ visible,
                                                float* __restrict__ fog_r1_of_draw0 ,
                                                float4* __restrict__ vnorm ,
                                                uint32_t* __restrict__ zero_words, uint32_t n_zero ,
                                                uint32_t* __restrict__ zero_hist ) {
    SWR_FRONT_ENTER();
    for (uint32_t i = blockIdx.x * (uint32_t)SWR_GEOM_BLOCK + threadIdx.x; i < n_zero; i += gridDim.x * (uint32_t)SWR_GEOM_BLOCK) zero_words[i] = 0u;
    if (blockIdx.x == 0) for (uint32_t i = threadIdx.x; i < 512u; i += (uint32_t)SWR_GEOM_BLOCK) zero_hist[i] = 0u;
    const BlockMap bm = blocks[blockIdx.x];
    if (visible && !visible[bm.draw]) return;
    const DrawParams* __restrict__ dp = draws + bm.draw;
    const uint32_t local = bm.first + threadIdx.x;
    __shared__ float4 s_out[SWR_GEOM_BLOCK / 64][256];
    static_assert(sizeof(s_out) <= SWR_FRONT_MAX_LDS, "k_vertex must fit beside the raster kernel (swr_device.h)");
    float4 o0 = make_float4(0.f, 0.f, 0.f, 0.f), o1 = o0, o2 = o0, o3 = o0;
    const bool live = local < dp->n_verts;
    const uint32_t wv_ = threadIdx.x >> 6, lane_ = threadIdx.x & 63u;
    const uint32_t first_ = bm.first + wv_ * 64u;
    const uint32_t n_live_ = dp->n_verts > first_ ? min(dp->n_verts - first_, 64u) : 0u;
    {
        const float4* __restrict__ src = reinterpret_cast<const float4*>(dp->verts + first_);
        float4* sw = &s_out[wv_][0];
#pragma unroll
        for (int k = 0; k < 3; ++k) {
            const uint32_t e = (uint32_t)k * 64u + lane_;
            if (e < 3u * n_live_) sw[e] = src[e];
        }
        __builtin_amdgcn_fence(__ATOMIC_ACQ_REL, "workgroup");
        __builtin_amdgcn_wave_barrier();
    }
    if (live) {
    if (local == 0u) {
        const float den = dp->u.fog_end - dp->u.fog_start;
        fog_r1_of_draw0[(size_t)bm.draw * (sizeof(DrawParams) / sizeof(float))] = div_operand_safe(den) ? rcp_refined(den) : 0.0f;
        fog_r1_of_draw0[(size_t)bm.draw * (sizeof(DrawParams) / sizeof(float)) + 3] = den;
    }

    const float4 q0 = s_out[wv_][3 * lane_], q1 = s_out[wv_][3 * lane_ + 1], q2 = s_out[wv_][3 * lane_ + 2];

    float p[4] = { q0.x, q0.y, q0.z, 1.0f };
    float world[4], viewp[4], clip[4];
    const bool fma_t = (dp->nm_flags & SWR_NM_TRANSFORM_FMA) != 0u, fma_tn = (dp->nm_flags & SWR_NM_TRANSFORM_NORMAL_FMA) != 0u;
    vec4_transform(p, dp->model, world, fma_t);
    vec4_transform(world, dp->view, viewp, fma_t);
    vec4_transform(viewp, dp->proj, clip, fma_t);
    float n[3] = { q1.y, q1.z, q1.w }, tn[3];
    vec3_transform_normal(n, dp->model, tn, fma_tn);
    float len = sqrtf(dot3(tn[0], tn[1], tn[2], tn[0], tn[1], tn[2]));

    o0 = make_float4(clip[0], clip[1], clip[2], clip[3]);
    o1 = q2;
    o2 = make_float4(q0.w, q1.x, tn[0] / len, tn[1] / len);
    o3 = make_float4(tn[2] / len, world[0], world[1], world[2]);
    if (vnorm) vnorm[dp->vert_base + local] = make_float4(n[0], n[1], n[2], 0.0f);
    }
    {
        const uint32_t wv = wv_, lane = lane_;
        float4* sw = &s_out[wv][0];
        __builtin_amdgcn_fence(__ATOMIC_ACQ_REL, "workgroup");
        __builtin_amdgcn_wave_barrier();
        sw[4 * lane + 0] = o0; sw[4 * lane + 1] = o1; sw[4 * lane + 2] = o2; sw[4 * lane + 3] = o3;
        __builtin_amdgcn_fence(__ATOMIC_ACQ_REL, "workgroup");
        __builtin_amdgcn_wave_barrier();
        const uint32_t first = first_, n_live = n_live_;
        float4* dst = reinterpret_cast<float4*>(vout + dp->vert_base + first);
#pragma unroll
        for (int k = 0; k < 4; ++k) {
            const uint32_t e = (uint32_t)k * 64u + lane;
            if ((e >> 2) < n_live) dst[e] = sw[e];
        }
    }
}
#else
__global__ __launch_bounds__(SWR_GEOM_BLOCK) void k_vertex_user(const DrawParams* __restrict__ draws,
                                                const BlockMap* __restrict__ blocks,
                                                VOut* __restrict__ vout, const uint32_t* __restrict__ visible,
                                                float* __restrict__ fog_r1_of_draw0,
                                                float4* __restrict__ vnorm ,
                                                uint32_t* __restrict__ zero_words, uint32_t n_zero,
                                                uint32_t* __restrict__ zero_hist,
                                                const float* __restrict__ user_consts ) {
    SWR_FRONT_ENTER();
    for (uint32_t i = blockIdx.x * (uint32_t)SWR_GEOM_BLOCK + threadIdx.x; i < n_zero; i += gridDim.x * (uint32_t)SWR_GEOM_BLOCK) zero_words[i] = 0u;
    if (blockIdx.x == 0) for (uint32_t i = threadIdx.x; i < 512u; i += (uint32_t)SWR_GEOM_BLOCK) zero_hist[i] = 0u;
    const BlockMap bm = blocks[blockIdx.x];
    if (visible && !visible[bm.draw]) return;
    const DrawParams* __restrict__ dp = draws + bm.draw;
    const uint32_t local = bm.first + threadIdx.x;
    __shared__ float4 s_out[SWR_GEOM_BLOCK / 64][256];
    static_assert(sizeof(s_out) <= SWR_FRONT_MAX_LDS, "k_vertex_user must fit beside the raster kernel (swr_device.h)");
    float4 o0 = make_float4(0.f, 0.f, 0.f, 0.f), o1 = o0, o2 = o0, o3 = o0;
    const bool live = local < dp->n_verts;
    const uint32_t wv = threadIdx.x >> 6, lane = threadIdx.x & 63u;
    const uint32_t first = bm.first + wv * 64u;
    const uint32_t n_live = dp->n_verts > first ? min(dp->n_verts - first, 64u) : 0u;
    float4* sw = &s_out[wv][0];
    {
        const float4* __restrict__ src = reinterpret_cast<const float4*>(dp->verts + first);
#pragma unroll
        for (int k = 0; k < 3; ++k) {
            const uint32_t e = (uint32_t)k * 64u + lane;
            if (e < 3u * n_live) sw[e] = src[e];
        }
        __builtin_amdgcn_fence(__ATOMIC_ACQ_REL, "workgroup");
        __builtin_amdgcn_wave_barrier();
    }
    if (live) {
        if (local == 0u) {
            const float den = dp->u.fog_end - dp->u.fog_start;
            fog_r1_of_draw0[(size_t)bm.draw * (sizeof(DrawParams) / sizeof(float))] = div_operand_safe(den) ? rcp_refined(den) : 0.0f;
            fog_r1_of_draw0[(size_t)bm.draw * (sizeof(DrawParams) / sizeof(float)) + 3] = den;
        }
        const float4 q0 = sw[3 * lane], q1 = sw[3 * lane + 1], q2 = sw[3 * lane + 2];
        swr_vs_in in;
        in.position = make_float3(q0.x, q0.y, q0.z);
        in.uv = make_float2(q0.w, q1.x);
        in.normal = make_float3(q1.y, q1.z, q1.w);
        in.color = q2;
        const swr_vs_env env = { dp->model, dp->view, dp->proj, dp->u, user_consts + 64u * bm.draw, dp->nm_flags };
        swr_vs_out out;
        out.clip_position = make_float4(0.f, 0.f, 0.f, 0.f); out.color = make_float4(0.f, 0.f, 0.f, 0.f);
        out.tex_coord = make_float2(0.f, 0.f); out.normal = make_float3(0.f, 0.f, 0.f);
        out.world_normal = make_float3(0.f, 0.f, 0.f); out.data4 = make_float4(0.f, 0.f, 0.f, 0.f);
        swr_vertex(in, env, out);
        o0 = out.clip_position;
        o1 = out.color;
        o2 = make_float4(out.tex_coord.x, out.tex_coord.y, out.world_normal.x, out.world_normal.y);
        o3 = make_float4(out.world_normal.z, out.data4.x, out.data4.y, out.data4.z);
        vnorm[dp->vert_base + local] = make_float4(out.normal.x, out.normal.y, out.normal.z, out.data4.w);
    }
    {
        __builtin_amdgcn_fence(__ATOMIC_ACQ_REL, "workgroup");
        __builtin_amdgcn_wave_barrier();
        sw[4 * lane + 0] = o0; sw[4 * lane + 1] = o1; sw[4 * lane + 2] = o2; sw[4 * lane + 3] = o3;
        __builtin_amdgcn_fence(__ATOMIC_ACQ_REL, "workgroup");
        __builtin_amdgcn_wave_barrier();
        float4* dst = reinterpret_cast<float4*>(vout + dp->vert_base + first);
#pragma unroll
        for (int k = 0; k < 4; ++k) {
            const uint32_t e = (uint32_t)k * 64u + lane;
            if ((e >> 2) < n_live) dst[e] = sw[e];
        }
    }
}
#endif

struct SVert {
    VOut v; bool interp; float nrm[3];
#ifdef SWR_USER_VERTEX
    float d4w;
#endif
};

__device__ __forceinline__ void svert_lerp(const SVert& a, const SVert& b, float t, SVert& r) {
#pragma unroll
    for (int i = 0; i < 4; ++i) r.v.clip[i] = nm_lerp(a.v.clip[i], b.v.clip[i], t);
#pragma unroll
    for (int i = 0; i < 2; ++i) r.v.uv[i] = nm_lerp(a.v.uv[i], b.v.uv[i], t);
#pragma unroll
    for (int i = 0; i < 4; ++i) r.v.color[i] = nm_lerp(a.v.color[i], b.v.color[i], t);
#pragma unroll
    for (int i = 0; i < 3; ++i) r.v.wn[i] = nm_lerp(a.v.wn[i], b.v.wn[i], t);
#pragma unroll
    for (int i = 0; i < 3; ++i) r.v.wpos[i] = nm_lerp(a.v.wpos[i], b.v.wpos[i], t);
#pragma unroll
    for (int i = 0; i < 3; ++i) r.nrm[i] = nm_lerp(a.nrm[i], b.nrm[i], t);
#ifdef SWR_USER_VERTEX
    r.d4w = nm_lerp(a.d4w, b.d4w, t);
#endif
    r.interp = true;
}

__device__ __forceinline__ void store_vout(VOut* __restrict__ dst, const VOut& v) {
    float4* o = reinterpret_cast<float4*>(dst);
    o[0] = make_float4(v.clip[0], v.clip[1], v.clip[2], v.clip[3]);
    o[1] = make_float4(v.color[0], v.color[1], v.color[2], v.color[3]);
    o[2] = make_float4(v.uv[0], v.uv[1], v.wn[0], v.wn[1]);
    o[3] = make_float4(v.wn[2], v.wpos[0], v.wpos[1], v.wpos[2]);
}
__device__ __forceinline__ void load_vout(const VOut* __restrict__ src, VOut& v) {
    const float4* s = reinterpret_cast<const float4*>(src);
    float4 a = s[0], b = s[1], c = s[2], d = s[3];
    v.clip[0] = a.x; v.clip[1] = a.y; v.clip[2] = a.z; v.clip[3] = a.w;
    v.color[0] = b.x; v.color[1] = b.y; v.color[2] = b.z; v.color[3] = b.w;
    v.uv[0] = c.x; v.uv[1] = c.y; v.wn[0] = c.z; v.wn[1] = c.w;
    v.wn[2] = d.x; v.wpos[0] = d.y; v.wpos[1] = d.z; v.wpos[2] = d.w;
}

__device__ __forceinline__ int setup_triangle(const FrameParams& fp, int cull, uint32_t draw,
                                              const SVert& v0, const SVert& v1, const SVert& v2,
                                              uint32_t r0, uint32_t r1, uint32_t r2,
                                              TriRec* __restrict__ rec, unsigned long long* __restrict__ tb, bool wireframe,
                                              float4* __restrict__ rec_regs = nullptr ) {
    const int rw = fp.width, rh = fp.height;
    const SVert* o[3] = { &v2, &v1, &v0 };
    float sx[3], sy[3], dz[3];
#pragma unroll
    for (int i = 0; i < 3; ++i) {
        float invW = 1.0f / o[i]->v.clip[3];
        float nx = o[i]->v.clip[0] * invW, ny = o[i]->v.clip[1] * invW, nz = o[i]->v.clip[2] * invW;
        if (is_nan_or_inf(nx) || is_nan_or_inf(ny) || is_nan_or_inf(nz)) return 0;
        sx[i] = (nx * 0.5f + 0.5f) * (float)rw;
        sy[i] = (1.0f - (ny * 0.5f + 0.5f)) * (float)rh;
        dz[i] = (nz + 1.0f) * 0.5f;
    }
    if (v0.v.clip[3] == 0 || v1.v.clip[3] == 0 || v2.v.clip[3] == 0) return 0;
    float area = edge_function(sx[0], sy[0], sx[1], sy[1], sx[2], sy[2]);
    if (area == 0) return 0;
    bool front = area < 0;
    if ((cull == SWR_CULL_BACK && !front) || (cull == SWR_CULL_FRONT && front)) return 0;
    const uint32_t flags = draw | (o[0]->interp ? SWR_FLAG_INTERP : 0u);

    if (wireframe) {
#pragma unroll
        for (int e = 0; e < 3; ++e) {
            const int i0 = e, i1 = (e + 1) % 3;
            const float p0x = sx[i0], p0y = sy[i0], p1x = sx[i1], p1y = sy[i1];
            const int minX = f2i(mathf_max(mathf_min(p0x, p1x), 0.0f));
            const int maxX = f2i(mathf_min(mathf_max(p0x, p1x), (float)(rw - 1)));
            const int minY = f2i(mathf_max(mathf_min(p0y, p1y), 0.0f));
            const int maxY = f2i(mathf_min(mathf_max(p0y, p1y), (float)(rh - 1)));
            if (minX > maxX || minY > maxY) continue;
            float4* out = reinterpret_cast<float4*>(rec + e);
            out[0] = make_float4(p0x, p1x, 0.0f, p0y);
            out[1] = make_float4(p1y, 0.0f, dz[0], dz[1]);
            out[2] = make_float4(dz[2], 0.0f, __uint_as_float(r2), __uint_as_float(r1));
            out[3] = make_float4(__uint_as_float(r2),
                                 __uint_as_float((uint32_t)minX | ((uint32_t)maxX << 16)),
                                 __uint_as_float((uint32_t)minY | ((uint32_t)maxY << 16)),
                                 __uint_as_float(flags | SWR_FLAG_LINE));
            tb[e] = (unsigned long long)(minX / SWR_TILE) | ((unsigned long long)(maxX / SWR_TILE) << 16) |
                    ((unsigned long long)(minY / SWR_TILE) << 32) | ((unsigned long long)(maxY / SWR_TILE) << 48);
        }
        return 0;
    }

    float inv_area = 1.0f / area;
    float minXf = mathf_min(mathf_min(sx[0], sx[1]), sx[2]);
    float maxXf = mathf_max(mathf_max(sx[0], sx[1]), sx[2]);
    float minYf = mathf_min(mathf_min(sy[0], sy[1]), sy[2]);
    float maxYf = mathf_max(mathf_max(sy[0], sy[1]), sy[2]);
    int minX = max(f2i(floorf(minXf)), 0);
    int maxX = min(f2i(ceilf(maxXf)), rw - 1);
    int minY = max(f2i(floorf(minYf)), 0);
    int maxY = min(f2i(ceilf(maxYf)), rh - 1);
    if (minX > maxX || minY > maxY) return 0;

    float4* out = rec_regs ? rec_regs : reinterpret_cast<float4*>(rec);
    {
    out[0] = make_float4(sx[0], sx[1], sx[2], sy[0]);
    out[1] = make_float4(sy[1], sy[2], dz[0], dz[1]);
    out[2] = make_float4(dz[2], inv_area, __uint_as_float(r2), __uint_as_float(r1));
    out[3] = make_float4(__uint_as_float(r0),
                         __uint_as_float((uint32_t)minX | ((uint32_t)maxX << 16)),
                         __uint_as_float((uint32_t)minY | ((uint32_t)maxY << 16)),
                         __uint_as_float(flags));
    }
    tb[0] = (unsigned long long)(minX / SWR_TILE) | ((unsigned long long)(maxX / SWR_TILE) << 16) |
            ((unsigned long long)(minY / SWR_TILE) << 32) | ((unsigned long long)(maxY / SWR_TILE) << 48);
    return 1;
}

#define SWR_FRAG_DRAW(dp, bm) ((dp)->frag_draw)
__global__ __launch_bounds__(SWR_GEOM_BLOCK) void k_setup(const DrawParams* __restrict__ draws,
                                               const BlockMap* __restrict__ blocks,
                                               const VOut* __restrict__ vout_ro,
                                               VOut* __restrict__ clip_pool,
                                               uint32_t clip_pool_base,
                                               TriRec* __restrict__ recs,
                                               unsigned long long* __restrict__ slot_tb,
                                               FrameParams fp,
                                               Counters* __restrict__ counters ,
                                               const Ctrl* __restrict__ ctrl, uint32_t seq, int count_stats, int wireframe,
                                               const uint32_t* __restrict__ visible,
                                               float4* __restrict__ vnorm ) {
    SWR_FRONT_ENTER();
    const BlockMap bm = blocks[blockIdx.x];
    const DrawParams* __restrict__ dp = draws + bm.draw;
    const uint32_t local = bm.first + threadIdx.x;
    const bool in_range = local < dp->n_tris;
    const bool drawn = !visible || visible[bm.draw] != 0u;
    const bool active = in_range && drawn;
    unsigned n_setup = 0, n_clipped = 0;
    float4 rec_q[4] = { make_float4(0.f, 0.f, 0.f, 0.f), make_float4(0.f, 0.f, 0.f, 0.f), make_float4(0.f, 0.f, 0.f, 0.f), make_float4(0.f, 0.f, 0.f, 0.f) };
    bool rec_valid = false;

    if (in_range && !drawn) {
        const uint32_t per_fan = wireframe ? 3u : 1u;
        const uint32_t slot = 2u * per_fan * (dp->tri_base + local);
        for (uint32_t k = 0; k < 2u * per_fan; ++k) slot_tb[slot + k] = SWR_TB_INVALID;
    }
    if (active) {
        const uint32_t gt = dp->tri_base + local;
        const uint32_t per_fan = wireframe ? 3u : 1u;
        const uint32_t slot = 2u * per_fan * gt;
        unsigned long long tbs[6] = { SWR_TB_INVALID, SWR_TB_INVALID, SWR_TB_INVALID, SWR_TB_INVALID, SWR_TB_INVALID, SWR_TB_INVALID };

        const uint16_t* __restrict__ ip = dp->idx + 3u * local;
        const uint32_t r0 = dp->vert_base + ip[0], r1 = dp->vert_base + ip[1], r2 = dp->vert_base + ip[2];
        SVert v[3];
        {
            const float4 c0 = reinterpret_cast<const float4*>(vout_ro + r0)[0], c1 = reinterpret_cast<const float4*>(vout_ro + r1)[0],
                         c2 = reinterpret_cast<const float4*>(vout_ro + r2)[0];
            v[0].v.clip[0] = c0.x; v[0].v.clip[1] = c0.y; v[0].v.clip[2] = c0.z; v[0].v.clip[3] = c0.w;
            v[1].v.clip[0] = c1.x; v[1].v.clip[1] = c1.y; v[1].v.clip[2] = c1.z; v[1].v.clip[3] = c1.w;
            v[2].v.clip[0] = c2.x; v[2].v.clip[1] = c2.y; v[2].v.clip[2] = c2.z; v[2].v.clip[3] = c2.w;
        }
        const bool interp = dp->program != SWR_PROG_FLAT_COLOR;
        v[0].interp = v[1].interp = v[2].interp = interp;

        const bool b0 = v[0].v.clip[3] <= 0, b1 = v[1].v.clip[3] <= 0, b2 = v[2].v.clip[3] <= 0;
        if (!(b0 && b1 && b2)) {
            if (b0 || b1 || b2) {
                n_clipped = 1;
                load_vout(vout_ro + r0, v[0].v);
                load_vout(vout_ro + r1, v[1].v);
                load_vout(vout_ro + r2, v[2].v);
                if (vnorm) {
                    const float4 n0 = vnorm[r0], n1 = vnorm[r1], n2 = vnorm[r2];
                    v[0].nrm[0] = n0.x; v[0].nrm[1] = n0.y; v[0].nrm[2] = n0.z;
                    v[1].nrm[0] = n1.x; v[1].nrm[1] = n1.y; v[1].nrm[2] = n1.z;
                    v[2].nrm[0] = n2.x; v[2].nrm[1] = n2.y; v[2].nrm[2] = n2.z;
#ifdef SWR_USER_VERTEX
                    v[0].d4w = n0.w; v[1].d4w = n1.w; v[2].d4w = n2.w;
#endif
                } else {
                    for (int i = 0; i < 3; ++i) v[i].nrm[0] = v[i].nrm[1] = v[i].nrm[2] = 0.0f;
#ifdef SWR_USER_VERTEX
                    for (int i = 0; i < 3; ++i) v[i].d4w = 0.0f;
#endif
                }
                SVert poly[4];
                int n = 0;
                const float nearc = fp.near_clip;
#pragma unroll
                for (int i = 0; i < 3; ++i) {
                    const SVert& cur = v[i];
                    const SVert& nxt = v[(i + 1) % 3];
                    bool cur_in = cur.v.clip[2] >= nearc * cur.v.clip[3];
                    bool nxt_in = nxt.v.clip[2] >= nearc * nxt.v.clip[3];
                    if (cur_in) { poly[n & 3] = cur; ++n; }
                    if (cur_in != nxt_in) {
                        float z0 = cur.v.clip[2], w0 = cur.v.clip[3], z1 = nxt.v.clip[2], w1 = nxt.v.clip[3];
                        float denom = (z1 - z0) - nearc * (w1 - w0);
                        float t;
                        if (fabsf(denom) < SWR_EPSILON) {
                            t = 0.5f;
                        } else {
                            t = (z0 - nearc * w0) / (nearc * (w1 - w0) - (z1 - z0));
                            t = math_clamp(t, 0.0f, 1.0f);
                        }
                        svert_lerp(cur, nxt, t, poly[n & 3]); ++n;
                    }
                }
                if (n >= 3) {
                    VOut* pool = clip_pool + 4ull * gt;
                    const uint32_t pbase = clip_pool_base + 4u * gt;
                    for (int k = 0; k < n; ++k) store_vout(pool + k, poly[k].v);
#ifdef SWR_USER_VERTEX
                    if (vnorm) for (int k = 0; k < n; ++k) vnorm[pbase + (uint32_t)k] = make_float4(poly[k].nrm[0], poly[k].nrm[1], poly[k].nrm[2], poly[k].d4w);
#else
                    if (vnorm) for (int k = 0; k < n; ++k) vnorm[pbase + (uint32_t)k] = make_float4(poly[k].nrm[0], poly[k].nrm[1], poly[k].nrm[2], 0.0f);
#endif
                    n_setup += setup_triangle(fp, dp->cull, SWR_FRAG_DRAW(dp, bm), poly[0], poly[1], poly[2],
                                              pbase, pbase + 1, pbase + 2, recs + slot, &tbs[0], wireframe != 0);
                    if (n == 4) n_setup += setup_triangle(fp, dp->cull, SWR_FRAG_DRAW(dp, bm), poly[0], poly[2], poly[3],
                                                          pbase, pbase + 2, pbase + 3, recs + slot + per_fan, &tbs[3], wireframe != 0);
                }
            } else {
                if (!wireframe) {
                    rec_valid = setup_triangle(fp, dp->cull, SWR_FRAG_DRAW(dp, bm), v[0], v[1], v[2], r0, r1, r2, recs + slot, &tbs[0], false, rec_q) != 0;
                    n_setup += rec_valid ? 1u : 0u;
                } else
                n_setup += setup_triangle(fp, dp->cull, SWR_FRAG_DRAW(dp, bm), v[0], v[1], v[2], r0, r1, r2, recs + slot, &tbs[0], wireframe != 0);
            }
        }
        if (wireframe) {
#pragma unroll
            for (int k = 0; k < 6; ++k) slot_tb[slot + k] = tbs[k];
        } else {
            *reinterpret_cast<ulonglong2*>(slot_tb + slot) = make_ulonglong2(tbs[0], tbs[3]);
        }
    }

    {
        __shared__ float4 s_rec[SWR_GEOM_BLOCK / 64][256];
        static_assert(sizeof(s_rec) + 16 <= SWR_FRONT_MAX_LDS, "k_setup must fit beside the raster kernel (swr_device.h)");
        const uint32_t wv = threadIdx.x >> 6, lane = threadIdx.x & 63u;
        const unsigned long long vmask = __ballot(rec_valid);
        if (vmask) {
            float4* sw = &s_rec[wv][0];
            sw[4 * lane + 0] = rec_q[0]; sw[4 * lane + 1] = rec_q[1]; sw[4 * lane + 2] = rec_q[2]; sw[4 * lane + 3] = rec_q[3];
            __builtin_amdgcn_fence(__ATOMIC_ACQ_REL, "workgroup");
            __builtin_amdgcn_wave_barrier();
            float4* dst = reinterpret_cast<float4*>(recs + 2u * (size_t)(dp->tri_base + bm.first + wv * 64u));
#pragma unroll
            for (int k = 0; k < 4; ++k) {
                const uint32_t e = (uint32_t)k * 64u + lane, j = e >> 2;
                if ((vmask >> j) & 1ull) dst[8u * j + (e & 3u)] = sw[e];
            }
        }
    }
    __shared__ unsigned s_cnt[3];
    if (threadIdx.x < 3) s_cnt[threadIdx.x] = 0;
    __syncthreads();
    unsigned long long act_mask = __ballot(active);
    unsigned long long set_mask1 = __ballot(n_setup >= 1), set_mask2 = __ballot(n_setup >= 2);
    unsigned long long clip_mask = __ballot(n_clipped != 0);
    if ((threadIdx.x & 63) == 0) {
        atomicAdd(&s_cnt[0], (unsigned)__popcll(act_mask));
        atomicAdd(&s_cnt[1], (unsigned)(__popcll(set_mask1) + __popcll(set_mask2)));
        atomicAdd(&s_cnt[2], (unsigned)__popcll(clip_mask));
    }
    __syncthreads();
    if (threadIdx.x == 0 && count_stats && !batch_poisoned(ctrl, seq)) {
        Counters* c = counters + (blockIdx.x & 63);
        atomicAdd(&c->triangles_in, (unsigned long long)s_cnt[0]);
        if (s_cnt[1]) atomicAdd(&c->triangles_setup, (unsigned long long)s_cnt[1]);
        if (s_cnt[2]) atomicAdd(&c->triangles_clipped, (unsigned long long)s_cnt[2]);
    }
}

}
```

softwarerenderer_amd/csrc/swr_raster_c.hip.h:

```cpp
#pragma once
#ifndef __HIPCC_RTC__
#include <type_traits>
#endif
#include "swr_device.h"
#include "swr_raster.hip.h"

namespace swr {

#define SWR_WAVE_LDS_FENCE_REAL() do { __builtin_amdgcn_fence(__ATOMIC_RELEASE, "wavefront"); __builtin_amdgcn_wave_barrier(); \
                                       __builtin_amdgcn_fence(__ATOMIC_ACQUIRE, "wavefront"); } while (0)
#ifndef SWR_WAVE_LDS_SYNC
#ifdef SWR_WAVE_LDS_FENCE
#define SWR_WAVE_LDS_SYNC() SWR_WAVE_LDS_FENCE_REAL()
#else
#define SWR_WAVE_LDS_SYNC() ((void)0)
#endif
#endif

#define SWR_BALLOT(cond) __builtin_amdgcn_ballot_w64((bool)(cond))

__device__ __forceinline__ int wave_incl_scan(int v, int lane) {
    (void)lane;
    v += __builtin_amdgcn_update_dpp(0, v, 0x111, 0xf, 0xf, false);
    v += __builtin_amdgcn_update_dpp(0, v, 0x112, 0xf, 0xf, false);
    v += __builtin_amdgcn_update_dpp(0, v, 0x114, 0xf, 0xf, false);
    v += __builtin_amdgcn_update_dpp(0, v, 0x118, 0xf, 0xf, false);
    v += __builtin_amdgcn_update_dpp(0, v, 0x142, 0xa, 0xf, false);
    v += __builtin_amdgcn_update_dpp(0, v, 0x143, 0xc, 0xf, false);
    return v;
}
__device__ __forceinline__ float wave_min(float x) {
    asm("s_nop 1\n"
                 "v_min_f32_dpp %0, %0, %0 row_shr:1 row_mask:0xf bank_mask:0xf\n s_nop 1\n"
                 "v_min_f32_dpp %0, %0, %0 row_shr:2 row_mask:0xf bank_mask:0xf\n s_nop 1\n"
                 "v_min_f32_dpp %0, %0, %0 row_shr:4 row_mask:0xf bank_mask:0xf\n s_nop 1\n"
                 "v_min_f32_dpp %0, %0, %0 row_shr:8 row_mask:0xf bank_mask:0xf\n s_nop 1\n"
                 "v_min_f32_dpp %0, %0, %0 row_bcast:15 row_mask:0xa bank_mask:0xf\n s_nop 1\n"
                 "v_min_f32_dpp %0, %0, %0 row_bcast:31 row_mask:0xc bank_mask:0xf\n s_nop 1"
                 : "+v"(x));
    return __int_as_float(__builtin_amdgcn_readlane(__float_as_int(x), 63));
}

struct CoverArgs {
    const TriRec* __restrict__ recs;
    const uint32_t* __restrict__ tile_list;
    const uint32_t* __restrict__ pair_tile;
    uint4* __restrict__ masks;
    uint2* __restrict__ info;
    uint4* __restrict__ refs;
    const unsigned long long* __restrict__ n_pairs;
    const Ctrl* __restrict__ ctrl;
    uint32_t seq;
    FrameParams fp;
    unsigned long long* dbg;
};

#define SWR_COVER_BLOCK 256
#define SWR_COVER_HQ 1
#define SWR_COVER_WQ 4
template <bool LINES>
__global__ __launch_bounds__(SWR_COVER_BLOCK) void k_cover(CoverArgs a) {
    SWR_FRONT_ENTER();
    constexpr int CB = SWR_COVER_BLOCK;
    constexpr int NB = 1 + (16 / SWR_COVER_HQ) * (16 / SWR_COVER_WQ);
    __shared__ uint16_t s_rows[CB][18];
    __shared__ uint32_t s_hist[NB];
    __shared__ uint16_t s_perm[CB];
    __shared__ uint32_t s_wmax[CB / 64];
    static_assert(sizeof(s_rows) + sizeof(s_hist) + sizeof(s_perm) + sizeof(s_wmax) + 64 <= SWR_FRONT_MAX_LDS, "k_cover must fit beside the raster kernel");
    if (batch_poisoned(a.ctrl, a.seq)) return;
    const uint32_t n_pairs = (uint32_t)*a.n_pairs;
    uint32_t block;
    {
        const uint32_t nb = (n_pairs + (uint32_t)CB - 1u) / (uint32_t)CB, per_xcd = (nb + 7u) >> 3;
        const uint32_t xcd = blockIdx.x & 7u, k = blockIdx.x >> 3;
        if (k >= per_xcd) return;
        block = xcd * per_xcd + k;
    }
    const uint32_t p_own = block * (uint32_t)CB + threadIdx.x;
    for (int i = threadIdx.x; i < NB; i += CB) s_hist[i] = 0u;
    if (threadIdx.x < CB / 64) s_wmax[threadIdx.x] = 0u;
    __syncthreads();
    uint32_t bucket = 0, rank = 0;
    {
        int area = 0;
        if (p_own < n_pairs) {
            const uint32_t slot = a.tile_list[p_own], tile = a.pair_tile[p_own];
            s_rows[threadIdx.x][0] = (uint16_t)slot; s_rows[threadIdx.x][1] = (uint16_t)(slot >> 16);
            s_rows[threadIdx.x][2] = (uint16_t)tile; s_rows[threadIdx.x][3] = (uint16_t)(tile >> 16);
            const int tx = (int)(tile % (uint32_t)a.fp.tiles_x), ty = band_global_row(band_map(a.fp), (int)(tile / (uint32_t)a.fp.tiles_x));
            const int x0 = tx * SWR_TILE, y0 = ty * SWR_TILE;
            const float4 r3 = reinterpret_cast<const float4*>(a.recs + slot)[3];
            {
                const float2 r2zw = reinterpret_cast<const float2*>(a.recs + slot)[5];
                a.refs[p_own] = make_uint4(slot, __float_as_uint(r2zw.x), __float_as_uint(r2zw.y), __float_as_uint(r3.x));
            }
            const uint32_t bbx = __float_as_uint(r3.y), bby = __float_as_uint(r3.z);
            const int w = min((int)(bbx >> 16), min(x0 + SWR_TILE - 1, a.fp.width - 1)) - max((int)(bbx & 0xffffu), x0) + 1;
            const int h = min((int)(bby >> 16), min(y0 + SWR_TILE - 1, a.fp.height - 1)) - max((int)(bby & 0xffffu), y0) + 1;
            area = (w > 0 && h > 0) ? w * h : 0;
            if (area > 0) area = 1 + ((h + SWR_COVER_HQ - 1) / SWR_COVER_HQ - 1) * (16 / SWR_COVER_WQ) + ((w + SWR_COVER_WQ - 1) / SWR_COVER_WQ - 1);
        }
        bucket = (uint32_t)area;
        rank = atomicAdd(&s_hist[bucket], 1u);
    }
    __syncthreads();
    static_assert(NB == 65, "one lane per bucket 1..64");
    if (threadIdx.x < 64) {
        const uint32_t b = (uint32_t)(NB - 1) - threadIdx.x;
        const uint32_t cnt_b = s_hist[b];
        const uint32_t incl = (uint32_t)wave_incl_scan((int)cnt_b, (int)threadIdx.x);
        s_hist[b] = incl - cnt_b;
        if (threadIdx.x == 63) s_hist[0] = incl;
    }
    __syncthreads();
    s_perm[s_hist[bucket] + rank] = (uint16_t)threadIdx.x;
    __syncthreads();
    const uint32_t owner = s_perm[threadIdx.x];
    const uint32_t p = block * (uint32_t)CB + owner;
    uint16_t* mrow16 = s_rows[owner];
    const uint32_t slot_w = (uint32_t)mrow16[0] | ((uint32_t)mrow16[1] << 16), tile_w = (uint32_t)mrow16[2] | ((uint32_t)mrow16[3] << 16);
#pragma unroll
    for (int i = 0; i < 16; ++i) mrow16[i] = 0;
    auto emit = [&a](const uint16_t* rows, uint32_t pi, float zb) {
        uint32_t mw[8];
        int cnt = 0;
#ifdef SWR_NO_SIMPLE_SELECT
        uint32_t not_run = 1u;
#else
        uint32_t not_run = 0u;
#endif
#pragma unroll
        for (int i = 0; i < 8; ++i) {
            const uint32_t lo = rows[2 * i], hi = rows[2 * i + 1];
            not_run |= (lo & (lo + (lo & (0u - lo)))) | (hi & (hi + (hi & (0u - hi))));
            mw[i] = lo | (hi << 16);
            cnt += __popc(mw[i]);
        }
        if (cnt) {
            a.masks[2 * (size_t)pi] = make_uint4(mw[0], mw[1], mw[2], mw[3]);
            a.masks[2 * (size_t)pi + 1] = make_uint4(mw[4], mw[5], mw[6], mw[7]);
        }
        a.info[pi] = make_uint2((uint32_t)cnt | (not_run == 0u ? SWR_INFO_SIMPLE : 0u), __float_as_uint(zb));
    };
    if (p < n_pairs) {
        const uint32_t slot = slot_w, tile = tile_w;
        const int tx = (int)(tile % (uint32_t)a.fp.tiles_x), ty = band_global_row(band_map(a.fp), (int)(tile / (uint32_t)a.fp.tiles_x));
        const int x0 = tx * SWR_TILE, y0 = ty * SWR_TILE;
        const int tile_end_x = min(x0 + SWR_TILE - 1, a.fp.width - 1), tile_end_y = min(y0 + SWR_TILE - 1, a.fp.height - 1);
        const float4* __restrict__ rq = reinterpret_cast<const float4*>(a.recs + slot);
        const float4 r0 = rq[0], r1 = rq[1], r2 = rq[2], r3 = rq[3];
        const float s0x = r0.x, s1x = r0.y, s2x = r0.z, s0y = r0.w, s1y = r1.x, s2y = r1.y;
        const uint32_t bbx = __float_as_uint(r3.y), bby = __float_as_uint(r3.z);
        const int startX = max((int)(bbx & 0xffffu), x0), endX = min((int)(bbx >> 16), tile_end_x);
        const int startY = max((int)(bby & 0xffffu), y0), endY = min((int)(bby >> 16), tile_end_y);
        const bool is_line = LINES && (__float_as_uint(r3.w) & SWR_FLAG_LINE) != 0u;
        float zbound = __uint_as_float(0x7f800000u);
        if (!is_line && startX <= endX && startY <= endY) {
            const float fxs = (float)startX, fxe = (float)endX, fys = (float)startY, fye = (float)endY;
            const float sx[3] = { r0.x, r0.y, r0.z }, sy[3] = { r0.w, r1.x, r1.y };
            const float dd[3] = { r1.z, r1.w, r2.x };
            const float inv_area = r2.y;
            const float ea[3] = { sy[1] - sy[2], sy[2] - sy[0], sy[0] - sy[1] };
            const float eb[3] = { sx[2] - sx[1], sx[0] - sx[2], sx[1] - sx[0] };
            const float rx[3] = { sx[1], sx[2], sx[0] }, ry[3] = { sy[1], sy[2], sy[0] };
            float c00 = 0.f, c10 = 0.f, c01 = 0.f, c11 = 0.f, S = 0.f, T = 0.f;
#pragma unroll
            for (int k = 0; k < 3; ++k) {
                const float kk = dd[k] * inv_area;
                const float dxs = fxs - rx[k], dxe = fxe - rx[k], dys = fys - ry[k], dye = fye - ry[k];
                const float xs = ea[k] * dxs, xe = ea[k] * dxe, ys = eb[k] * dys, ye = eb[k] * dye;
                c00 += kk * (xs + ys); c10 += kk * (xe + ys); c01 += kk * (xs + ye); c11 += kk * (xe + ye);
                const float mk = fabsf(ea[k]) * fmaxf(fabsf(dxs), fabsf(dxe)) + fabsf(eb[k]) * fmaxf(fabsf(dys), fabsf(dye));
                S += fabsf(kk) * mk;
                T += ((mk + fabsf(kk)) + fabsf(dd[k])) + 1.0f;
            }
            const float U = (fmaxf(fmaxf(c00, c10), fmaxf(c01, c11)) + S * (64.0f / 16777216.0f)) + T * 0x1p-146f;
            const bool finite = S < 1.0e30f && c00 == c00 && c10 == c10 && c01 == c01 && c11 == c11;
            if (finite) zbound = U;
        }
        if (is_line && startX <= endX && startY <= endY) {
            for (int y = startY; y <= endY; ++y) {
                uint32_t rowbits = 0;
                for (int x = startX; x <= endX; ++x) {
                    float t;
                    if (line_test(s0x, s0y, s1x, s1y, x, y, t)) rowbits |= 1u << (x - x0);
                }
                mrow16[y - y0] = (uint16_t)rowbits;
            }
        } else if (startX <= endX && startY <= endY) {
            const float a01 = s0y - s1y, b01 = s1x - s0x;
            const float a12 = s1y - s2y, b12 = s2x - s1x;
            const float a20 = s2y - s0y, b20 = s0x - s2x;
            const float fsx = (float)startX, fsy = (float)startY;
            float w0r = a12 * (fsx - s1x) + b12 * (fsy - s1y);
            float w1r = a20 * (fsx - s2x) + b20 * (fsy - s2y);
            float w2r = a01 * (fsx - s0x) + b01 * (fsy - s0y);
            const float lim = 1.0e30f;
            const bool fast = fabsf(a12) < lim && fabsf(a20) < lim && fabsf(a01) < lim && fabsf(b12) < lim && fabsf(b20) < lim &&
                              fabsf(b01) < lim && fabsf(w0r) < lim && fabsf(w1r) < lim && fabsf(w2r) < lim;
            if (fast) {
                const int width = endX - startX + 1;
                atomicMax(&s_wmax[threadIdx.x >> 6], (uint32_t)width);
                SWR_WAVE_LDS_FENCE_REAL();
                const int wsteps = __builtin_amdgcn_readfirstlane((int)s_wmax[threadIdx.x >> 6]);
                const uint32_t colmask = (1u << width) - 1u;
                const int sh = startX - x0;
                for (int y = startY; y <= endY; ++y) {
                    float w0 = w0r, w1 = w1r, w2 = w2r;
                    uint32_t acc = 0;
                    for (int i = 0; i < wsteps; ++i) {
                        {
                            const unsigned long long in_mask = SWR_BALLOT(fminf(fminf(w0, w1), w2) >= 0.0f) | SWR_BALLOT(fmaxf(fmaxf(w0, w1), w2) <= 0.0f);
                            unsigned long long carry_out;
                            asm("v_addc_co_u32 %0, %1, %2, %2, %3" : "=v"(acc), "=s"(carry_out) : "v"(acc), "s"(in_mask));
                        }
                        w0 += a12; w1 += a20; w2 += a01;
                    }
                    const uint32_t rowbits = ((__brev(acc) >> (32 - wsteps)) & colmask) << sh;
                    mrow16[y - y0] = (uint16_t)rowbits;
                    w0r += b12; w1r += b20; w2r += b01;
                }
            } else {
                float w0 = w0r, w1 = w1r, w2 = w2r;
                const int area = (endX - startX + 1) * (endY - startY + 1);
                int x = startX, y = startY;
                uint32_t rowbits = 0;
                for (int it = 0; it < area; ++it) {
                    const bool inside = (w0 >= 0 && w1 >= 0 && w2 >= 0) || (w0 <= 0 && w1 <= 0 && w2 <= 0);
                    rowbits |= inside ? (1u << (x - x0)) : 0u;
                    if (x == endX) {
                        mrow16[y - y0] = (uint16_t)rowbits;
                        rowbits = 0;
                        w0r += b12; w1r += b20; w2r += b01;
                        w0 = w0r; w1 = w1r; w2 = w2r;
                        x = startX; ++y;
                    } else {
                        w0 += a12; w1 += a20; w2 += a01;
                        ++x;
                    }
                }
            }
        }
        mrow16[16] = (uint16_t)__float_as_uint(zbound); mrow16[17] = (uint16_t)(__float_as_uint(zbound) >> 16);
    }
    __syncthreads();
    if (p_own < n_pairs) {
        const uint16_t* own = s_rows[threadIdx.x];
        emit(own, p_own, __uint_as_float((uint32_t)own[16] | ((uint32_t)own[17] << 16)));
    }
}

#define SWR_BATCH 16
#define SWR_BATCH_FRAGS 2048
#define SWR_WINDOW 32
#define SWR_VROW(r, idx) L.stage[r][idx]
template <bool PHONG>
struct __attribute__((aligned(16))) WaveLdsC {
    static constexpr bool VG = PHONG;
    static constexpr int NQ = VG ? 7 : 13;
    static constexpr int BATCH = SWR_BATCH;
    static constexpr int WINDOW = SWR_WINDOW;
    static constexpr int RT_ROWS = VG ? 8 : 4;
    static constexpr int RT_N = 16 / RT_ROWS - 1;
    float4 col[256];
    float z[256];
    float4 stage[NQ][BATCH];
    uint32_t mask[BATCH][8];
    uint32_t wpre[BATCH][4];
    uint32_t head[SWR_BATCH_FRAGS / 32 + 4];
    uint32_t touched[32];
    float rowtab3[VG ? 1 : RT_N][3][VG ? 1 : BATCH];
    float4 rowtab4[VG ? RT_N : 1][VG ? BATCH : 1];
    __device__ __forceinline__ void rt_store(int q, int t, float x, float y, float z, float w) {
        if constexpr (VG) rowtab4[q][t] = make_float4(x, y, z, w);
        else { rowtab3[q][0][t] = x; rowtab3[q][1][t] = y; rowtab3[q][2][t] = z; }
    }
    __device__ __forceinline__ void rt_load(int q, int t, float& x, float& y, float& z) const {
        if constexpr (VG) { const float4 e = rowtab4[q][t]; x = e.x; y = e.y; z = e.z; }
        else { x = rowtab3[q][0][t]; y = rowtab3[q][1][t]; z = rowtab3[q][2][t]; }
    }
    __device__ __forceinline__ float rt_w(int t) const { return rowtab4[0][VG ? t : 0].w; }
};

#ifdef SWR_DEBUG_PHASES
#define SWR_PHASE_DECL unsigned ph_t = (unsigned)__builtin_readcyclecounter(), ph_acc0 = 0u, ph_acc1 = 0u, ph_acc2 = 0u, ph_acc3 = 0u, \
                                ph_acc4 = 0u, ph_acc5 = 0u, ph_acc6 = 0u, ph_acc7 = 0u;
#define SWR_PHASE(i) do { const unsigned now_ = (unsigned)__builtin_readcyclecounter(); ph_acc##i += now_ - ph_t; ph_t = now_; } while (0)
#define SWR_PHASE_FLUSH(dbg) do { if ((threadIdx.x & 63) == 0 && (blockIdx.x & 63u) == 0u && (dbg)) {    \
        atomicAdd(&(dbg)[0], (unsigned long long)ph_acc0); atomicAdd(&(dbg)[1], (unsigned long long)ph_acc1); \
        atomicAdd(&(dbg)[2], (unsigned long long)ph_acc2); atomicAdd(&(dbg)[3], (unsigned long long)ph_acc3); \
        atomicAdd(&(dbg)[4], (unsigned long long)ph_acc4); atomicAdd(&(dbg)[5], (unsigned long long)ph_acc5); \
        atomicAdd(&(dbg)[6], (unsigned long long)ph_acc6); atomicAdd(&(dbg)[7], (unsigned long long)ph_acc7); } } while (0)
#else
#define SWR_PHASE_DECL
#define SWR_PHASE(i) ((void)0)
#define SWR_PHASE_FLUSH(dbg) ((void)0)
#endif

#define SWR_RP_STEP(I) "v_cmpx_lt_i32_e32 vcc, " #I ", %[n]\n v_add_f32_e32 %[w0], %[s0], %[w0]\n v_add_f32_e32 %[w1], %[s1], %[w1]\n v_add_f32_e32 %[w2], %[s2], %[w2]\n"
#define SWR_RP_OUT "s_nop 4\n s_cbranch_execz .Lrp_end_%=\n"
template <int MAXN>
__device__ __forceinline__ void replay_chain(float& w0, float& w1, float& w2, int n, float s0, float s1, float s2) {
    static_assert(MAXN == 3 || MAXN == 7 || MAXN == 15, "row replay (RT_ROWS - 1) or column replay (15)");
    unsigned long long saved;
    if constexpr (MAXN == 3) {
        asm("s_mov_b64 %[sv], exec\n"
            SWR_RP_STEP(0) SWR_RP_STEP(1) SWR_RP_STEP(2)
            "s_mov_b64 exec, %[sv]"
            : [w0] "+v"(w0), [w1] "+v"(w1), [w2] "+v"(w2), [sv] "=&s"(saved) : [n] "v"(n), [s0] "v"(s0), [s1] "v"(s1), [s2] "v"(s2) : "vcc");
    } else if constexpr (MAXN == 7) {
        asm("s_mov_b64 %[sv], exec\n"
            SWR_RP_STEP(0) SWR_RP_STEP(1) SWR_RP_STEP(2) SWR_RP_STEP(3) SWR_RP_OUT
            SWR_RP_STEP(4) SWR_RP_STEP(5) SWR_RP_STEP(6)
            ".Lrp_end_%=:\n s_mov_b64 exec, %[sv]"
            : [w0] "+v"(w0), [w1] "+v"(w1), [w2] "+v"(w2), [sv] "=&s"(saved) : [n] "v"(n), [s0] "v"(s0), [s1] "v"(s1), [s2] "v"(s2) : "vcc");
    } else {
        asm("s_mov_b64 %[sv], exec\n"
            SWR_RP_STEP(0) SWR_RP_STEP(1) SWR_RP_STEP(2) SWR_RP_STEP(3) SWR_RP_OUT
            SWR_RP_STEP(4) SWR_RP_STEP(5) SWR_RP_STEP(6) SWR_RP_STEP(7) SWR_RP_OUT
            SWR_RP_STEP(8) SWR_RP_STEP(9) SWR_RP_STEP(10) SWR_RP_STEP(11) SWR_RP_OUT
            SWR_RP_STEP(12) SWR_RP_STEP(13) SWR_RP_STEP(14)
            ".Lrp_end_%=:\n s_mov_b64 exec, %[sv]"
            : [w0] "+v"(w0), [w1] "+v"(w1), [w2] "+v"(w2), [sv] "=&s"(saved) : [n] "v"(n), [s0] "v"(s0), [s1] "v"(s1), [s2] "v"(s2) : "vcc");
    }
}

__device__ __forceinline__ int kth_set_bit32(uint32_t w, int k) {
    int base = 0;
#pragma unroll
    for (int width = 16; width >= 1; width >>= 1) {
        const uint32_t lowmask = (width == 32) ? 0xffffffffu : ((1u << width) - 1u);
        const int c = __popc((w >> base) & lowmask);
        const bool up = k >= c;
        k -= up ? c : 0;
        base += up ? width : 0;
    }
    return base;
}

static_assert(sizeof(WaveLdsC<false>) <= 10240 && sizeof(WaveLdsC<true>) <= 8960, "16 (18) waves per CU need <= 10,240 (8,960) B of LDS per wave");
template <bool LINES, bool PHONG, int PROG = -1, int BLEND = -1, int DT = -1, bool EARLYOUT = false>
__global__ __launch_bounds__(64, (PHONG && PROG != SWR_PROG_PHONG_4POINT) ? 5 : 4) void k_raster_c(RasterArgs a, const uint4* __restrict__ masks,
                                                                  const uint2* __restrict__ info) {
    __shared__ WaveLdsC<PHONG> s_w;
    if (batch_poisoned(a.ctrl, a.seq)) return;
    SWR_PHASE_DECL

    const int lane = threadIdx.x & 63;
    const bool HIZ = !LINES && (DT == SWR_DEPTH_LESS || DT == SWR_DEPTH_LESSEQUAL || (DT < 0 && a.depth_only_grows != 0));
    uint4 desc;
    {
        const uint32_t xcd = blockIdx.x & 7u, k = blockIdx.x >> 3;
        const uint32_t j = (((k >> 6) << 3) + xcd) * 64u + (k & 63u);
        if (j >= a.n_tiles) return;
        desc = a.tile_order[j];
    }
    const uint32_t tile_o = desc.x;
    const int tx = (int)(tile_o % (uint32_t)a.fp.tiles_x), ty_local = (int)(tile_o / (uint32_t)a.fp.tiles_x);
    if (tx >= a.fp.tiles_x || ty_local >= a.fp.band_tile_rows) return;
    const int ty = band_global_row(band_map(a.fp), ty_local);
    const uint32_t tile = (uint32_t)(ty_local * a.fp.tiles_x + tx);
    const uint32_t n = desc.z;
    if (n == 0 && !a.clear_color_on && !a.clear_depth_on) {
        if (threadIdx.x == 0) a.tile_work[tile] = 0u;
        return;
    }
    const uint32_t start = desc.y;
    WaveLdsC<PHONG>& L = s_w;
    constexpr bool VG = WaveLdsC<PHONG>::VG;
    constexpr int RT_ROWS = WaveLdsC<PHONG>::RT_ROWS;
    const __amdgpu_buffer_rsrc_t vout_rsrc = __builtin_amdgcn_make_buffer_rsrc((void*)a.vout, 0, (int)a.vout_bytes, 0x00020000);
    auto shade_debug = [&L, &a](int t, float w0f, float w1f, float w2f) {
        if (!(PHONG && VG && PROG == SWR_PROG_DEBUG_VARYINGS)) return make_float4(0.f, 0.f, 0.f, 0.f);
        const __amdgpu_buffer_rsrc_t nrm_rsrc = __builtin_amdgcn_make_buffer_rsrc((void*)a.vnorm, 0, (int)(a.vout_bytes >> 2), 0x00020000);
        const __amdgpu_buffer_rsrc_t rec_rsrc = __builtin_amdgcn_make_buffer_rsrc((void*)a.recs, 0, 0x7ffffff0, 0x00020000);
        const float4 q4 = L.stage[VG ? 4 : 0][t], q5 = L.stage[VG ? 5 : 0][t], q6 = L.stage[VG ? 6 : 0][t];
        auto ld4 = [](__amdgpu_buffer_rsrc_t r, uint32_t off) {
            const auto v = __builtin_amdgcn_raw_buffer_load_b128(r, (int)off, 0, 0);
            return make_float4(__uint_as_float(v[0]), __uint_as_float(v[1]), __uint_as_float(v[2]), __uint_as_float(v[3]));
        };
        const float4 na = ld4(nrm_rsrc, __float_as_uint(q4.x) >> 2), nb = ld4(nrm_rsrc, __float_as_uint(q4.y) >> 2), nc = ld4(nrm_rsrc, __float_as_uint(q4.z) >> 2);
        const uint32_t ro = __float_as_uint(q6.x);
        const float4 r0 = ld4(rec_rsrc, ro), r1 = ld4(rec_rsrc, ro + 16u);
        const float sx[3] = { r0.x, r0.y, r0.z }, sy[3] = { r0.w, r1.x, r1.y };
        float wc_clip = 0.0f;
        if constexpr (VG) wc_clip = L.rt_w(t);
        const float inv_w = 1.0f / (float)(a.fp.width - 1), inv_h = 1.0f / (float)(a.fp.height - 1);
        return shade_debug_varyings(w0f, w1f, w2f, q4.w, q5.w, wc_clip, na, nb, nc, sx, sy, inv_w, inv_h);
    };
    auto shade_user = [&L, &a, vout_rsrc](int t, float w0f, float w1f, float w2f, const DrawConsts& dc, uint32_t draw, int px, int py) {
#ifdef SWR_RTC_PROGRAM
        if constexpr (PHONG && VG && PROG == SWR_PROG_CUSTOM) {
            const __amdgpu_buffer_rsrc_t nrm_rsrc = __builtin_amdgcn_make_buffer_rsrc((void*)a.vnorm, 0, (int)(a.vout_bytes >> 2), 0x00020000);
            const __amdgpu_buffer_rsrc_t rec_rsrc = __builtin_amdgcn_make_buffer_rsrc((void*)a.recs, 0, 0x7ffffff0, 0x00020000);
            auto ld4 = [](__amdgpu_buffer_rsrc_t r, uint32_t off) {
                const auto v = __builtin_amdgcn_raw_buffer_load_b128(r, (int)off, 0, 0);
                return make_float4(__uint_as_float(v[0]), __uint_as_float(v[1]), __uint_as_float(v[2]), __uint_as_float(v[3]));
            };
            const float4 q4 = L.stage[4][t], q6 = L.stage[6][t];
            const uint32_t off[3] = { __float_as_uint(q4.x), __float_as_uint(q4.y), __float_as_uint(q4.z) };
            float4 clip[3], col[3], uvn[3], nrm[3], d4[3];
            float wnz[3];
#pragma unroll
            for (int k = 0; k < 3; ++k) {
                clip[k] = ld4(vout_rsrc, off[k]); col[k] = ld4(vout_rsrc, off[k] + 16u); uvn[k] = ld4(vout_rsrc, off[k] + 32u);
                const float4 r3 = ld4(vout_rsrc, off[k] + 48u);
                wnz[k] = r3.x;
                nrm[k] = ld4(nrm_rsrc, off[k] >> 2);
#ifdef SWR_USER_VERTEX
                d4[k] = make_float4(r3.y, r3.z, r3.w, nrm[k].w);
#else
                d4[k] = make_float4(0.f, 0.f, 0.f, 0.f);
#endif
            }
            const uint32_t ro = __float_as_uint(q6.x);
            const float4 r0 = ld4(rec_rsrc, ro), r1 = ld4(rec_rsrc, ro + 16u);
            const float sx[3] = { r0.x, r0.y, r0.z }, sy[3] = { r0.w, r1.x, r1.y };
            const float inv_w = 1.0f / (float)(a.fp.width - 1), inv_h = 1.0f / (float)(a.fp.height - 1);
            const swr_fs_in in = interpolate_fs_in(w0f, w1f, w2f, clip, col, uvn, wnz, nrm, d4, sx, sy, inv_w, inv_h);
            const swr_fs_env env = { a.draws[draw].u, a.user_consts + 64u * draw, px, py, dc.tex, dc.tex_w, dc.tex_h };
            return swr_fragment(in, env);
        }
#endif
        (void)L; (void)a; (void)vout_rsrc; (void)t; (void)w0f; (void)w1f; (void)w2f; (void)dc; (void)draw; (void)px; (void)py;
        return make_float4(0.f, 0.f, 0.f, 0.f);
    };
    auto load_varyings = [&L, vout_rsrc](int t, bool fastdiv, int part = 0, TriVaryings V = TriVaryings()) {
        if (VG) {
            const float4 q4 = L.stage[VG ? 4 : 0][t], q5 = L.stage[VG ? 5 : 0][t];
            const uint32_t oa = __float_as_uint(q4.x), ob = __float_as_uint(q4.y), oc = __float_as_uint(q4.z);
            auto row = [&](uint32_t off, int r) {
                const auto v = __builtin_amdgcn_raw_buffer_load_b128(vout_rsrc, (int)off + 16 * r, 0, 0);
                return make_float4(__uint_as_float(v[0]), __uint_as_float(v[1]), __uint_as_float(v[2]), __uint_as_float(v[3]));
            };
            auto word = [&](uint32_t off, int byte) { return __uint_as_float(__builtin_amdgcn_raw_buffer_load_b32(vout_rsrc, (int)off + byte, 0, 0)); };
            if (part != 2) { V.a_uvn = row(oa, 2); V.b_uvn = row(ob, 2); V.c_uvn = row(oc, 2); }
            if (part == 1) return V;
            V.a_cz = word(oa, 8); V.b_cz = word(ob, 8); V.c_cz = word(oc, 8);
            V.a_col = row(oa, 1); V.b_col = row(ob, 1); V.c_col = row(oc, 1);
            if (PHONG) {
                const float4 a3 = row(oa, 3), b3 = row(ob, 3), c3 = row(oc, 3);
                V.a_wnz = a3.x; V.b_wnz = b3.x; V.c_wnz = c3.x;
                V.a_wpos[0] = a3.y; V.a_wpos[1] = a3.z; V.a_wpos[2] = a3.w;
                V.b_wpos[0] = b3.y; V.b_wpos[1] = b3.z; V.b_wpos[2] = b3.w;
                V.c_wpos[0] = c3.y; V.c_wpos[1] = c3.z; V.c_wpos[2] = c3.w;
            } else {
                V.a_wnz = word(oa, 48); V.b_wnz = word(ob, 48); V.c_wnz = word(oc, 48);
            }
            V.a_r1 = q5.x; V.b_r1 = q5.y; V.c_r1 = q5.z;
            V.a_w = q4.w; V.b_w = q5.w;
            if constexpr (VG) V.c_w = L.rt_w(t);
            V.fastdiv = fastdiv;
            return V;
        }
        const float4 a_clip = SWR_VROW(VG ? 0 : 4, t), b_clip = SWR_VROW(VG ? 0 : 7, t), c_clip = SWR_VROW(VG ? 0 : 10, t);
        V.a_col = SWR_VROW(VG ? 0 : 5, t); V.a_uvn = SWR_VROW(VG ? 0 : 6, t);
        V.b_col = SWR_VROW(VG ? 0 : 8, t); V.b_uvn = SWR_VROW(VG ? 0 : 9, t);
        V.c_col = SWR_VROW(VG ? 0 : 11, t); V.c_uvn = SWR_VROW(VG ? 0 : 12, t);
        V.a_wnz = a_clip.x; V.b_wnz = b_clip.x; V.c_wnz = c_clip.x;
        V.a_r1 = a_clip.y; V.b_r1 = b_clip.y; V.c_r1 = c_clip.y;
        V.a_cz = a_clip.z; V.b_cz = b_clip.z; V.c_cz = c_clip.z;
        V.a_w = a_clip.w; V.b_w = b_clip.w; V.c_w = c_clip.w;
        V.fastdiv = fastdiv;
        if (PHONG) {
            const float4 a3 = SWR_VROW((PHONG && !VG) ? 13 : 0, t), b3 = SWR_VROW((PHONG && !VG) ? 14 : 0, t), c3 = SWR_VROW((PHONG && !VG) ? 15 : 0, t);
            V.a_wpos[0] = a3.y; V.a_wpos[1] = a3.z; V.a_wpos[2] = a3.w;
            V.b_wpos[0] = b3.y; V.b_wpos[1] = b3.z; V.b_wpos[2] = b3.w;
            V.c_wpos[0] = c3.y; V.c_wpos[1] = c3.z; V.c_wpos[2] = c3.w;
        }
        return V;
    };

    const int W = a.fp.width, H = a.fp.height;
    const int x0 = tx * SWR_TILE, y0 = ty * SWR_TILE;

    uint4 ref_w = make_uint4(0u, 0u, 0u, 0u);
    int cnt_w = 0;
    float zb_w = 0.0f;
    constexpr int BATCH = WaveLdsC<PHONG>::BATCH, WINDOW = WaveLdsC<PHONG>::WINDOW;
    if (lane < WINDOW && (uint32_t)lane < n) {
        ref_w = a.pair_refs[start + (uint32_t)lane];
        const uint2 pi = info[start + (uint32_t)lane];
        cnt_w = (int)pi.x; zb_w = __uint_as_float(pi.y);
    }

#pragma unroll
    for (int rr = 0; rr < 4; ++rr) {
        const int p = rr * 64 + lane;
        const int gx = x0 + (p & 15), gy = y0 + (p >> 4);
        const bool inb = gx < W && gy < H;
        const size_t gi = (size_t)(ty_local * SWR_TILE + (p >> 4)) * (size_t)W + (size_t)gx;
        float4 c;
        if (a.clear_color_on) c = make_float4(a.clear_rgba[0], a.clear_rgba[1], a.clear_rgba[2], a.clear_rgba[3]);
        else c = inb ? a.color[gi] : make_float4(0.f, 0.f, 0.f, 0.f);
        float zz;
        if (a.clear_depth_on) zz = SWR_FLOAT_MINVALUE;
        else zz = inb ? a.depth[gi] : SWR_FLOAT_MINVALUE;
        L.col[p] = c;
        L.z[p] = zz;
    }
    unsigned n_tested = 0, n_shaded = 0, n_written = 0;
    uint32_t carry_key = 0xffffffffu;
    bool carry_dead = false;
#ifdef SWR_DEBUG_COUNTERS
    unsigned dbg_batches = 0, dbg_chunks = 0, dbg_chunk_lanes = 0, dbg_chain = 0, dbg_chain_c = 0, dbg_sum_r = 0, dbg_sum_c = 0, dbg_hidden = 0;
#endif

    DrawConsts dc = {};
    uint32_t dc_draw = 0xffffffffu;
    uint32_t batch_no = 0;
    bool fast_draw = false;
    SWR_PHASE(0);
    for (uint32_t base = 0; base < n; ++batch_no) {
        const uint32_t pidx = start + base + (uint32_t)lane;
        const uint4 ref = ref_w;
        const bool in_window = lane < WINDOW && base + (uint32_t)lane < n;
        const bool simple_in = cnt_w < 0;
        const int cnt_in = in_window ? (cnt_w & 0x7fffffff) : 0;
        int cnt = cnt_in;
        if (HIZ) {
            float zmin = 3.0e38f;
#pragma unroll
            for (int rr = 0; rr < 4; ++rr) {
                const int p = rr * 64 + lane;
                const bool inb = x0 + (p & 15) < W && y0 + (p >> 4) < H;
                zmin = fminf(zmin, inb ? L.z[p] : 3.0e38f);
            }
            zmin = wave_min(zmin);
#ifndef SWR_ABL_NOHIZ
            if (cnt > 0 && zmin > SWR_FLOAT_MINVALUE && zb_w < zmin) cnt = 0;
#endif
        }
        int consumed;
        const int cscan = wave_incl_scan(cnt, lane);
        {
            const unsigned long long surv = SWR_BALLOT(cnt > 0);
            const int rank = __popcll(surv & ((1ull << lane) - 1ull));
            const unsigned long long left_out = SWR_BALLOT(cnt > 0 && (rank >= BATCH || cscan > SWR_BATCH_FRAGS));
            consumed = left_out ? __ffsll((long long)left_out) - 1 : min(WINDOW, (int)(n - base));
            if (lane >= consumed) cnt = 0;
        }
        const int cnt_seen = lane < consumed ? cnt_in : 0;
        n_tested += (unsigned)cnt_seen;
#ifdef SWR_DEBUG_COUNTERS
        dbg_hidden += (unsigned)(cnt_seen - cnt);
#endif
        base += (uint32_t)consumed;
        {
            const uint32_t e = base + (uint32_t)lane;
            ref_w = make_uint4(0u, 0u, 0u, 0u); cnt_w = 0; zb_w = 0.0f;
            if (lane < WINDOW && e < n) {
                ref_w = a.pair_refs[start + e];
                const uint2 pi = info[start + e];
                cnt_w = (int)pi.x; zb_w = __uint_as_float(pi.y);
            }
        }
        const int cincl = cscan;
        const int total = consumed > 0 ? __builtin_amdgcn_readlane(cscan, min(consumed, 64) - 1) : 0;
        SWR_PHASE(1);
        if (total == 0) continue;
        const unsigned long long nzb = SWR_BALLOT(cnt > 0);
        const int ci = __popcll(nzb & ((1ull << lane) - 1ull));
        if (lane < SWR_BATCH_FRAGS / 128 + 1) *reinterpret_cast<uint4*>(&L.head[4 * lane]) = make_uint4(0u, 0u, 0u, 0u);
        if (cnt > 0) {
            const uint4 m0 = masks[2 * (size_t)pidx], m1 = masks[2 * (size_t)pidx + 1];
            const float4* __restrict__ fq = reinterpret_cast<const float4*>(a.recs + ref.x);
            const float4 f0 = fq[0], f1 = fq[1], f2 = fq[2], f3 = fq[3];
            bool fastdiv;
            float wc_stage = 0.0f;
            if (VG) {
                const float wa = a.vout[ref.y].clip[3], wb = a.vout[ref.z].clip[3], wc = a.vout[ref.w].clip[3];
                fastdiv = div_operands_safe3(wa, wb, wc);
                L.stage[VG ? 4 : 0][ci] = make_float4(__uint_as_float(ref.y << 6), __uint_as_float(ref.z << 6), __uint_as_float(ref.w << 6), wa);
                L.stage[VG ? 5 : 0][ci] = make_float4(rcp_refined(wa), rcp_refined(wb), rcp_refined(wc), wb);
                L.stage[VG ? 6 : 0][ci] = make_float4(__uint_as_float(ref.x << 6), 0.0f, 0.0f, 0.0f);
                wc_stage = wc;
            } else {
                const float4* __restrict__ pa = reinterpret_cast<const float4*>(a.vout + ref.y);
                const float4* __restrict__ pb = reinterpret_cast<const float4*>(a.vout + ref.z);
                const float4* __restrict__ pc = reinterpret_cast<const float4*>(a.vout + ref.w);
                const float4 a3 = pa[3], b3 = pb[3], c3 = pc[3];
                float4 a0 = pa[0], b0 = pb[0], c0 = pc[0];
                a0.x = a3.x; b0.x = b3.x; c0.x = c3.x;
                fastdiv = div_operands_safe3(a0.w, b0.w, c0.w);
                a0.y = rcp_refined(a0.w); b0.y = rcp_refined(b0.w); c0.y = rcp_refined(c0.w);
                SWR_VROW(VG ? 0 : 4, ci) = a0; SWR_VROW(VG ? 0 : 5, ci) = pa[1]; SWR_VROW(VG ? 0 : 6, ci) = pa[2];
                SWR_VROW(VG ? 0 : 7, ci) = b0; SWR_VROW(VG ? 0 : 8, ci) = pb[1]; SWR_VROW(VG ? 0 : 9, ci) = pb[2];
                SWR_VROW(VG ? 0 : 10, ci) = c0; SWR_VROW(VG ? 0 : 11, ci) = pc[1]; SWR_VROW(VG ? 0 : 12, ci) = pc[2];
                if (PHONG) { SWR_VROW((PHONG && !VG) ? 13 : 0, ci) = a3; SWR_VROW((PHONG && !VG) ? 14 : 0, ci) = b3; SWR_VROW((PHONG && !VG) ? 15 : 0, ci) = c3; }
            }
            {
                const float t0x = f0.x, t1x = f0.y, t2x = f0.z, t0y = f0.w, t1y = f1.x, t2y = f1.y;
                const uint32_t fbx = __float_as_uint(f3.y), fby = __float_as_uint(f3.z);
                const int fsX = max((int)(fbx & 0xffffu), x0), fsY = max((int)(fby & 0xffffu), y0);
                const uint32_t fs = (uint32_t)(fsX - x0) | ((uint32_t)(fsY - y0) << 8);
                const float a01 = t0y - t1y, b01 = t1x - t0x;
                const float a12 = t1y - t2y, b12 = t2x - t1x;
                const float a20 = t2y - t0y, b20 = t0x - t2x;
                float4 r0;
                if (LINES && (__float_as_uint(f3.w) & SWR_FLAG_LINE) != 0u) {
                    r0 = make_float4(t0x, t1x, t0y, t1y);
                } else {
                    const float fsx = (float)fsX, fsy = (float)fsY;
                    r0.x = a12 * (fsx - t1x) + b12 * (fsy - t1y);
                    r0.y = a20 * (fsx - t2x) + b20 * (fsy - t2y);
                    r0.z = a01 * (fsx - t0x) + b01 * (fsy - t0y);
                    r0.w = f2.y;
                }
                L.stage[0][ci] = r0;
                L.stage[1][ci] = make_float4(f1.z, f1.w, f2.x, __uint_as_float(__float_as_uint(f3.w) | (fastdiv ? SWR_FLAG_FASTDIV : 0u) |
                                                                                 (simple_in ? SWR_FLAG_SIMPLE : 0u)));
                const uint32_t pre = (uint32_t)(cincl - cnt);
                L.stage[2][ci] = make_float4(a12, a20, a01, __uint_as_float(fs));
                L.stage[3][ci] = make_float4(b12, b20, b01, __uint_as_float(pre));
                if (ci > 0) atomicOr(&L.head[(pre - 1u) >> 5], 1u << ((pre - 1u) & 31u));
                float rw0 = r0.x, rw1 = r0.y, rw2 = r0.z;
#pragma unroll
                for (int q = 0; q < WaveLdsC<PHONG>::RT_N; ++q) {
#pragma unroll
                    for (int i = 0; i < RT_ROWS; ++i) { rw0 += b12; rw1 += b20; rw2 += b01; }
                    L.rt_store(q, ci, rw0, rw1, rw2, wc_stage);
                }
            }
            *reinterpret_cast<uint4*>(&L.mask[ci][0]) = m0;
            *reinterpret_cast<uint4*>(&L.mask[ci][4]) = m1;
            const uint32_t p1 = (uint32_t)__popc(m0.x), p2 = p1 + (uint32_t)__popc(m0.y), p3 = p2 + (uint32_t)__popc(m0.z),
                           p4 = p3 + (uint32_t)__popc(m0.w), p5 = p4 + (uint32_t)__popc(m1.x), p6 = p5 + (uint32_t)__popc(m1.y),
                           p7 = p6 + (uint32_t)__popc(m1.z);
            *reinterpret_cast<uint4*>(&L.wpre[ci][0]) = make_uint4(p1 << 16, p2 | (p3 << 16), p4 | (p5 << 16), p6 | (p7 << 16));
        }
#ifdef SWR_DEBUG_COUNTERS
        ++dbg_batches;
#endif

        SWR_WAVE_LDS_SYNC();
        int t0 = 0;
        uint32_t hn0 = L.head[0], hn1 = L.head[1], hn2 = L.head[2];
        int t_n = 0;
        uint4 wp_n = make_uint4(0u, 0u, 0u, 0u);
        uint32_t pre_n = 0u;
        auto lookup_ahead = [&](int pos_n) {
            const int hs_n = pos_n & 31;
            const uint32_t wl = __builtin_amdgcn_alignbit(hn1, hn0, hs_n), wh = __builtin_amdgcn_alignbit(hn2, hn1, hs_n);
            t_n = t0 + (int)__builtin_amdgcn_mbcnt_hi(wh, __builtin_amdgcn_mbcnt_lo(wl, 0u));
            wp_n = *reinterpret_cast<const uint4*>(&L.wpre[t_n][0]);
            pre_n = __float_as_uint(L.stage[3][t_n].w);
        };
        lookup_ahead(0);
        SWR_PHASE(2);
        for (int pos = 0; pos < total;) {
            const int g = pos + lane;
            const bool valid = g < total;
            const unsigned long long validmask = SWR_BALLOT(g < total);
            const int hs = pos & 31;
            const uint32_t h0 = hn0, h1 = hn1, h2 = hn2;
            const uint32_t win_lo = __builtin_amdgcn_alignbit(h1, h0, hs), win_hi = __builtin_amdgcn_alignbit(h2, h1, hs);
            const int t = t_n;
            const float4 f0 = L.stage[0][t], f1 = L.stage[1][t], f2 = L.stage[2][t], f3 = L.stage[3][t];
            TriVaryings Vg = TriVaryings();
            int k = valid ? g - (int)pre_n : 0;
            int pix;
            {
                const uint4 wp = wp_n;
                const uint32_t kk = ((uint32_t)k | ((uint32_t)k << 16)) | 0x80008000u;
                const int nle = __popc((kk - wp.x) & 0x80008000u) + __popc((kk - wp.y) & 0x80008000u) +
                                __popc((kk - wp.z) & 0x80008000u) + __popc((kk - wp.w) & 0x80008000u);
                const int wi = nle - 1;
                const uint32_t wsel = L.mask[t][wi];
                const int kw = k - (int)reinterpret_cast<const uint16_t*>(&L.wpre[t][0])[wi];
                const bool okk = valid;
                const bool simple = (__float_as_uint(f1.w) & SWR_FLAG_SIMPLE) != 0u;
                const uint32_t lo = wsel & 0xffffu;
                const int c0 = __popc(lo);
                const bool up = kw >= c0;
                const uint32_t half = up ? (wsel >> 16) : lo;
                int posw = (up ? 16 + (kw - c0) : kw) + (__ffs((int)half) - 1);
                if (SWR_BALLOT((__float_as_uint(f1.w) & SWR_FLAG_SIMPLE) == 0u) != 0ull) {
                    if (!simple) posw = kth_set_bit32(wsel, okk ? kw : 0);
                }
                pix = (wi * 32 + posw) & 255;
            }
            const uint32_t fs_early = __float_as_uint(f2.w);
            const int nrow_e = (pix >> 4) - (int)(fs_early >> 8);
            const int q_e = nrow_e >> (RT_ROWS == 8 ? 3 : 2), qi_e = max(q_e, 1) - 1;
            float t0r_e = 0.0f, t1r_e = 0.0f, t2r_e = 0.0f, z_old = 0.0f;
            if (!EARLYOUT) {
                L.rt_load(qi_e, t, t0r_e, t1r_e, t2r_e);
                z_old = L.z[pix];
            }
            SWR_PHASE(3);
            const int pix_first = __builtin_amdgcn_readfirstlane(pix);
            unsigned long long dupmask = 0ull;
#ifndef SWR_ABL_NOELECT
            {
                if (lane < 8) *reinterpret_cast<uint4*>(&L.touched[4 * lane]) = make_uint4(0u, 0u, 0u, 0u);
                SWR_WAVE_LDS_SYNC();
                const uint32_t pbit = 1u << (pix >> 5);
                uint32_t before = 0u;
                if (valid) before = atomicOr(&L.touched[pix & 31], pbit);
                dupmask = (SWR_BALLOT((before & pbit) != 0u) | SWR_BALLOT(pix == pix_first)) & ~1ull;
            }
#endif
            const uint32_t dflags = __float_as_uint(f1.w);
            const uint32_t draw = dflags & SWR_DRAW_MASK;
            const uint32_t draw0 = (uint32_t)__builtin_amdgcn_readfirstlane((int)draw);
            const unsigned long long stop = ~validmask | dupmask | SWR_BALLOT(draw != draw0);
            const int cut = stop ? (__ffsll((long long)stop) - 1) : 64;
            {
                const unsigned long long win = ((unsigned long long)(uint32_t)__builtin_amdgcn_readfirstlane((int)win_hi) << 32) |
                                               (unsigned long long)(uint32_t)__builtin_amdgcn_readfirstlane((int)win_lo);
                t0 += __popcll(cut >= 64 ? win : (win & ((1ull << cut) - 1ull)));
            }
            SWR_PHASE(4);
            const bool act = lane < cut;
            if (VG) { if (act) Vg = load_varyings(t, (dflags & SWR_FLAG_FASTDIV) != 0u, 1); }
            {
                const int hw_next = (pos + cut) >> 5;
                hn0 = L.head[hw_next]; hn1 = L.head[hw_next + 1]; hn2 = L.head[hw_next + 2];
            }
#ifdef SWR_DEBUG_COUNTERS
            ++dbg_chunks; dbg_chunk_lanes += (unsigned)cut;
#endif

            const DrawParams* __restrict__ cdp = a.draws + draw0;
            if (draw0 != dc_draw) {
                dc_draw = draw0; dc = load_draw_consts(cdp);
                if (!PHONG && !LINES && PROG == SWR_PROG_DUST2_LAMBERT_FOG) fast_draw = dust2_fast_applies(dc);
                if (PHONG && !LINES && PROG == SWR_PROG_PHONG_4POINT) fast_draw = phong4_fast_applies(dc);
            }
            const int f_program = PROG >= 0 ? PROG : dc.program, f_blend = BLEND >= 0 ? BLEND : dc.blend, f_dt = DT >= 0 ? DT : dc.depth_test;
            const bool f_interp = PROG > SWR_PROG_FLAT_COLOR ? true : (__float_as_uint(f1.w) & SWR_FLAG_INTERP) != 0u;
#ifdef SWR_DEBUG_COUNTERS
            int dbg_nrow = 0, dbg_ncol = 0;
#endif
            bool e_pass = false, e_alpha = false;
            float e_d = 0.0f;
            float4 e_src = make_float4(0.f, 0.f, 0.f, 0.f);
            const bool is_line = LINES && (dflags & SWR_FLAG_LINE) != 0u;
            float w0f = 0.0f, w1f = 0.0f, w2f = 0.0f, d = 0.0f;
            if (act) {
                const float d0 = f1.x, d1 = f1.y, d2 = f1.z;
                const uint32_t fs = __float_as_uint(f2.w);
                if (is_line) {
                    float t;
                    (void)line_test(f0.x, f0.z, f0.y, f0.w, x0 + (pix & 15), y0 + (pix >> 4), t);
                    w0f = 1.0f - t; w1f = t; w2f = 0.0f;
                    d = 1.0f / (d0 * (1.0f - t) + d1 * t);
                } else {
                    float w0 = f0.x, w1 = f0.y, w2 = f0.z;
                    const float inv_area = f0.w;
                    const int nrow = (pix >> 4) - (int)(fs >> 8), ncol = (pix & 15) - (int)(fs & 0xffu);
#ifdef SWR_DEBUG_COUNTERS
                    dbg_nrow = nrow; dbg_ncol = ncol;
#endif
                    {
                        const int q = nrow >> (RT_ROWS == 8 ? 3 : 2);
                        if (EARLYOUT) L.rt_load(qi_e, t, t0r_e, t1r_e, t2r_e);
                        if (q > 0) { w0 = t0r_e; w1 = t1r_e; w2 = t2r_e; }
                        const int rem = nrow & (RT_ROWS - 1);
                        replay_chain<RT_ROWS - 1>(w0, w1, w2, rem, f3.x, f3.y, f3.z);
                    }
                    replay_chain<15>(w0, w1, w2, ncol, f2.x, f2.y, f2.z);
                    w0f = w0 * inv_area; w1f = w1 * inv_area; w2f = w2 * inv_area;
                    d = (d0 * w0f + d1 * w1f) + d2 * w2f;
                }
            }
            SWR_PHASE(5);
            lookup_ahead(pos + cut);
            if (act) {
                if (!EARLYOUT) {
                    if (depth_func(f_dt, d, z_old)) {
                        ++n_shaded;
                        const float4 dst = L.col[pix];
#ifdef SWR_ABL_NOSHADE
                        const float4 src = make_float4(w0f, w1f, w2f, 1.0f);
#else
                        float4 src = make_float4(0.f, 0.f, 0.f, 0.f);
                        constexpr bool FAST = !LINES && ((!PHONG && PROG == SWR_PROG_DUST2_LAMBERT_FOG) || (PHONG && PROG == SWR_PROG_PHONG_4POINT));
                        const TriVaryings Vs = VG ? load_varyings(t, (dflags & SWR_FLAG_FASTDIV) != 0u, 2, Vg) : load_varyings(t, (dflags & SWR_FLAG_FASTDIV) != 0u);
                        bool need_exact = !(FAST && fast_draw);
                        if (FAST && fast_draw) {
                            bool safe;
                            if constexpr (PHONG) src = shade_phong4_fast(cdp, dc, Vs, w0f, w1f, w2f, safe);
                            else src = shade_dust2_fast(dc, Vs, w0f, w1f, w2f, safe);
                            need_exact = SWR_BALLOT(!safe) != 0ull;
                        }
                        if (need_exact)
                            src = (PHONG && PROG == SWR_PROG_DEBUG_VARYINGS) ? shade_debug(t, w0f, w1f, w2f) :
                                  (PHONG && PROG == SWR_PROG_CUSTOM) ? shade_user(t, w0f, w1f, w2f, dc, draw0, x0 + (pix & 15), y0 + (pix >> 4)) :
                                  shade_fragment<PHONG>(cdp, dc, f_program, f_interp, Vs, w0f, w1f, w2f);
#endif
                        if (is_line ? (src.w != 0.0f) : (src.w > 0.0f)) {
                            L.col[pix] = blend(src, dst, f_blend);
                            if (f_dt != SWR_DEPTH_DISABLED) L.z[pix] = d;
                            ++n_written;
                        }
                    }
                } else {
                    e_d = d;
                    e_pass = depth_func(f_dt, d, L.z[pix]);
                    if (e_pass) {
                        e_src = (PHONG && PROG == SWR_PROG_DEBUG_VARYINGS) ? shade_debug(t, w0f, w1f, w2f) :
                                (PHONG && PROG == SWR_PROG_CUSTOM) ? shade_user(t, w0f, w1f, w2f, dc, draw0, x0 + (pix & 15), y0 + (pix >> 4)) :
                                shade_fragment<PHONG>(cdp, dc, f_program, f_interp,
                                                      VG ? load_varyings(t, (dflags & SWR_FLAG_FASTDIV) != 0u, 2, Vg) : load_varyings(t, (dflags & SWR_FLAG_FASTDIV) != 0u),
                                                      w0f, w1f, w2f);
                        e_alpha = is_line ? (e_src.w != 0.0f) : (e_src.w > 0.0f);
                    }
                }
            }
#ifdef SWR_DEBUG_COUNTERS
            {
                int mr = act ? dbg_nrow : 0, mc = act ? dbg_ncol : 0, sr = mr, sc = mc;
                for (int off = 32; off > 0; off >>= 1) { mr = max(mr, __shfl_xor(mr, off)); mc = max(mc, __shfl_xor(mc, off));
                                                         sr += __shfl_xor(sr, off); sc += __shfl_xor(sc, off); }
                dbg_chain += (unsigned)mr; dbg_chain_c += (unsigned)mc; dbg_sum_r += (unsigned)sr; dbg_sum_c += (unsigned)sc;
            }
#endif
            if (EARLYOUT) {
                bool killed = false;
                const bool none = f_blend == SWR_BLEND_NONE;
                const uint32_t key = ((batch_no * (uint32_t)BATCH + (uint32_t)t) << 4) | (uint32_t)(pix >> 4);
                if (none) {
                    const uint32_t prev = (uint32_t)__shfl_up((int)key, 1);
                    const bool head = act && (lane == 0 || key != prev);
                    const unsigned long long H = SWR_BALLOT(head);
                    const unsigned long long F = SWR_BALLOT(act && e_pass && !e_alpha);
                    const unsigned long long below = (1ull << lane) - 1ull;
                    const unsigned long long hm = H & (below | (1ull << lane));
                    const int headlane = hm ? 63 - __clzll((long long)hm) : 0;
                    const unsigned long long seg_below = below & ~((1ull << headlane) - 1ull);
                    killed = act && (F & seg_below) != 0ull;
                    if (act && headlane == 0 && carry_dead && key == carry_key) killed = true;
                    const bool dead_after = killed || (act && e_pass && !e_alpha);
                    carry_key = (uint32_t)__shfl((int)key, cut - 1);
                    carry_dead = __shfl((int)dead_after, cut - 1) != 0;
                } else {
                    carry_dead = false;
                }
                if (act) {
                    if (killed) {
                        --n_tested;
                    } else if (e_pass) {
                        ++n_shaded;
                        if (e_alpha) {
                            const float4 dst = L.col[pix];
                            L.col[pix] = blend(e_src, dst, f_blend);
                            if (f_dt != SWR_DEPTH_DISABLED) L.z[pix] = e_d;
                            ++n_written;
                        }
                    }
                }
            }
            pos += cut;
            SWR_PHASE(6);
        }
    }

    int lane_wb = lane;
    asm volatile("" : "+v"(lane_wb));
#pragma unroll
    for (int rr = 0; rr < 4; ++rr) {
        const int p = rr * 64 + lane_wb;
        const int gx = x0 + (p & 15), gy = y0 + (p >> 4);
        if (gx < W && gy < H) {
            const size_t gi = (size_t)(ty_local * SWR_TILE + (p >> 4)) * (size_t)W + (size_t)gx;
            a.color[gi] = L.col[p];
            a.depth[gi] = L.z[p];
        }
    }

    n_tested = (unsigned)__builtin_amdgcn_readlane(wave_incl_scan((int)n_tested, lane), 63);
    n_shaded = (unsigned)__builtin_amdgcn_readlane(wave_incl_scan((int)n_shaded, lane), 63);
    n_written = (unsigned)__builtin_amdgcn_readlane(wave_incl_scan((int)n_written, lane), 63);
    if (lane == 0) a.tile_work[tile] = n_tested;
    SWR_PHASE(7);
    SWR_PHASE_FLUSH(a.dbg);
    if (lane == 0 && n > 0) {
        uint32_t* ts = a.tile_stats + 3u * tile;
        atomicAdd(&ts[0], n_tested); atomicAdd(&ts[1], n_shaded); atomicAdd(&ts[2], n_written);
    }
#ifdef SWR_DEBUG_COUNTERS
    if (lane == 0 && a.dbg) {
        atomicAdd(&a.dbg[0], (unsigned long long)dbg_batches); atomicAdd(&a.dbg[1], (unsigned long long)dbg_chunks);
        atomicAdd(&a.dbg[4], (unsigned long long)dbg_chunk_lanes); atomicAdd(&a.dbg[3], (unsigned long long)dbg_chain);
        atomicAdd(&a.dbg[2], (unsigned long long)dbg_chain_c); atomicAdd(&a.dbg[5], (unsigned long long)dbg_sum_r);
        atomicAdd(&a.dbg[6], (unsigned long long)dbg_sum_c);
    }
    {
        unsigned h = dbg_hidden;
        for (int off = 32; off > 0; off >>= 1) h += (unsigned)__shfl_xor((int)h, off);
        if (lane == 0 && a.dbg) atomicAdd(&a.dbg[7], (unsigned long long)h);
    }
#endif
}

}
```

Before: 74540 Mfragments/s.

## Compute small-tile coverage masks at setup and store triangle records densely

Moves the per-tile coverage test for small triangles from the binning count pass into triangle setup, so binning only reads a precomputed want mask and no longer loads records for small triangles. Triangle records are also remapped so even and odd slots (fan halves) live in separate dense halves of the array, which keeps records for mostly-empty second fan slots from interleaving with real ones. This improves cache and memory locality in the record reads done by cover and raster. In exchange, setup does extra edge tests per triangle and every record access pays for an index remap.

```diff
diff --git a/softwarerenderer_amd/csrc/swr_binning.hip.h b/softwarerenderer_amd/csrc/swr_binning.hip.h
--- a/softwarerenderer_amd/csrc/swr_binning.hip.h
+++ b/softwarerenderer_amd/csrc/swr_binning.hip.h
@@ -8,10 +8,10 @@
 struct BinArgs {
     const unsigned long long* __restrict__ slot_tb;
     const TriRec* __restrict__ recs;
+    uint32_t odd_base;
     uint32_t slot_lo, slot_hi;
     uint32_t spt;
     int tiles_x;
-    int band_ty0, band_ty1;
     BandMap band;
     int width, height;
     uint32_t* __restrict__ tile_count;
@@ -23,7 +23,7 @@
     uint32_t seq;
     uint32_t replayable;
     const unsigned long long* __restrict__ total;
-    uint8_t* __restrict__ want;
+    const uint8_t* __restrict__ want;
     uint32_t tpw;
     uint32_t bin_blocks;
     int order_tiles_y;
@@ -33,36 +33,6 @@
     uint4* __restrict__ tile_order;
 };
 
-__device__ __forceinline__ bool pair_may_cover(const float sx[3], const float sy[3], int minX, int maxX, int minY, int maxY,
-                                               int tx, int ty, int width, int height, bool is_line) {
-    if (is_line) return true;
-    const int x0 = tx * SWR_TILE, y0 = ty * SWR_TILE;
-    const int startX = max(minX, x0), endX = min(maxX, min(x0 + SWR_TILE - 1, width - 1));
-    const int startY = max(minY, y0), endY = min(maxY, min(y0 + SWR_TILE - 1, height - 1));
-    if (startX > endX || startY > endY) return false;
-    const float ea[3] = { sy[1] - sy[2], sy[2] - sy[0], sy[0] - sy[1] };
-    const float eb[3] = { sx[2] - sx[1], sx[0] - sx[2], sx[1] - sx[0] };
-    const float rx[3] = { sx[1], sx[2], sx[0] };
-    const float ry[3] = { sy[1], sy[2], sy[0] };
-    const float fxs = (float)startX, fxe = (float)endX, fys = (float)startY, fye = (float)endY;
-    const float lim = 1.0e15f;
-    const bool tame = fabsf(sx[0]) < lim && fabsf(sx[1]) < lim && fabsf(sx[2]) < lim && fabsf(sy[0]) < lim && fabsf(sy[1]) < lim && fabsf(sy[2]) < lim;
-    if (!tame) return true;
-    bool any_neg = false, any_pos = false;
-#pragma unroll
-    for (int k = 0; k < 3; ++k) {
-        const float a = ea[k], b = eb[k];
-        const float dxs = fxs - rx[k], dxe = fxe - rx[k], dys = fys - ry[k], dye = fye - ry[k];
-        const float ax_s = a * dxs, ax_e = a * dxe, by_s = b * dys, by_e = b * dye;
-        const float emax = fmaxf(ax_s, ax_e) + fmaxf(by_s, by_e);
-        const float emin = fminf(ax_s, ax_e) + fminf(by_s, by_e);
-        const float m = fabsf(a) * fmaxf(fabsf(dxs), fabsf(dxe)) + fabsf(b) * fmaxf(fabsf(dys), fabsf(dye));
-        const float delta = m * (64.0f / 16777216.0f);
-        any_neg = any_neg || emax < -delta;
-        any_pos = any_pos || emin > delta;
-    }
-    return !(any_neg && any_pos);
-}
 
 __device__ __forceinline__ void bin_overflow(const BinArgs& a) {
     a.counters->overflow = 1u;
@@ -128,28 +98,15 @@
     int minX, maxX, minY, maxY;
     bool is_line;
 };
-__device__ __forceinline__ SlotData slot_none() {
+__device__ __forceinline__ SlotData slot_load(const BinArgs& a, uint32_t slot, unsigned long long tb) {
     SlotData s;
-    s.tminx = s.tminy = s.nx = s.ny = 0;
     s.sx[0] = s.sx[1] = s.sx[2] = s.sy[0] = s.sy[1] = s.sy[2] = 0.f;
     s.minX = s.minY = 0; s.maxX = s.maxY = -1; s.is_line = false;
-    return s;
-}
-__device__ __forceinline__ bool slot_tiles(const BinArgs& a, unsigned long long tb, SlotData& s) {
-    if (tb == SWR_TB_INVALID) return false;
-    s.tminx = (int)(tb & 0xffff);
-    const int tmaxx = (int)((tb >> 16) & 0xffff);
-    s.tminy = max((int)((tb >> 32) & 0xffff), a.band_ty0);
-    const int tmaxy = min((int)((tb >> 48) & 0xffff), a.band_ty1 - 1);
-    s.nx = tmaxx - s.tminx + 1;
-    s.ny = tmaxy - s.tminy + 1;
-    if (s.ny <= 0) { s.nx = 0; s.ny = 0; return false; }
-    return true;
-}
-__device__ __forceinline__ SlotData slot_load(const BinArgs& a, uint32_t slot, unsigned long long tb, bool with_rec_small) {
-    SlotData s = slot_none();
-    if (slot_tiles(a, tb, s) && (with_rec_small || s.nx * s.ny > 8)) {
-        const float4* __restrict__ rq = reinterpret_cast<const float4*>(a.recs + slot);
+    SlotTiles st;
+    slot_tiles(a.band, tb, st);
+    s.tminx = st.tminx; s.tminy = st.tminy; s.nx = st.nx; s.ny = st.ny;
+    if (s.nx * s.ny > SWR_SMALL_TILES) {
+        const float4* __restrict__ rq = reinterpret_cast<const float4*>(a.recs + rec_index(slot, a.odd_base));
         const float4 r0 = rq[0], r1 = rq[1], r3 = rq[3];
         s.sx[0] = r0.x; s.sx[1] = r0.y; s.sx[2] = r0.z; s.sy[0] = r0.w; s.sy[1] = r1.x; s.sy[2] = r1.y;
         const uint32_t bbx = __float_as_uint(r3.y), bby = __float_as_uint(r3.z);
@@ -241,28 +198,23 @@
 #define SWR_BIN_TABLE (1 << SWR_BIN_TABLE_LOG2)
 template <bool FILL>
 __device__ __forceinline__ void bin_block_slots(const BinArgs& a, uint32_t slot, unsigned long long tb, uint32_t want_in, uint32_t* s_key, uint32_t* s_val) {
-    const SlotData sd = slot_load(a, slot, tb, !FILL);
+    const SlotData sd = slot_load(a, slot, tb);
     const int nt = sd.nx * sd.ny;
-    const bool big = nt > 8;
+    const bool big = nt > SWR_SMALL_TILES;
     const int nt_small = big ? 0 : nt;
     if (!__syncthreads_or(nt != 0)) return;
     for (int e = threadIdx.x; e < SWR_BIN_TABLE; e += 256) { s_key[e] = 0u; s_val[e] = 0u; }
     __syncthreads();
-    uint32_t packed[8];
-    int wtx = sd.tminx, wty = sd.tminy;
-    uint32_t wmask = (FILL && nt_small) ? want_in : 0u;
-#pragma unroll
-    for (int i = 0; i < 8; ++i) {
+    uint32_t packed[SWR_SMALL_TILES];
+    SlotTiles st; st.tminx = sd.tminx; st.tminy = sd.tminy; st.nx = sd.nx; st.ny = sd.ny;
+    SmallTileWalk w(st);
+    const uint32_t wmask = nt_small ? want_in : 0u;
+#pragma unroll
+    for (int i = 0; i < SWR_SMALL_TILES; ++i) {
         packed[i] = 0u;
         if (i < nt_small) {
-            bool want;
-            if (FILL) want = ((wmask >> i) & 1u) != 0u;
-            else {
-                want = band_local_row(a.band, wty) >= 0 && pair_may_cover(sd.sx, sd.sy, sd.minX, sd.maxX, sd.minY, sd.maxY, wtx, wty, a.width, a.height, sd.is_line);
-                wmask |= want ? (1u << i) : 0u;
-            }
-            if (want) {
-                const uint32_t tile = (uint32_t)(band_local_row(a.band, wty) * a.tiles_x + wtx);
+            if ((wmask >> i) & 1u) {
+                const uint32_t tile = (uint32_t)(band_local_row(a.band, w.ty) * a.tiles_x + w.tx);
                 uint32_t e = (tile * 0x9E3779B1u) >> (32 - SWR_BIN_TABLE_LOG2);
                 bool placed = false;
                 for (int probe = 0; probe < 16; ++probe) {
@@ -281,11 +233,9 @@
                     atomicAdd(&a.tile_count[tile], 1u);
                 }
             }
-            ++wtx;
-            if (wtx >= sd.tminx + sd.nx) { wtx = sd.tminx; ++wty; }
-        }
-    }
-    if (!FILL && nt_small) a.want[slot] = (uint8_t)wmask;
+            w.next();
+        }
+    }
     __syncthreads();
     for (int e = threadIdx.x; e < SWR_BIN_TABLE; e += 256) {
         const uint32_t key = s_key[e];
@@ -298,7 +248,7 @@
     if (FILL) {
         __syncthreads();
 #pragma unroll
-        for (int i = 0; i < 8; ++i) {
+        for (int i = 0; i < SWR_SMALL_TILES; ++i) {
             if (packed[i] & 0x80000000u) {
                 const uint32_t at = s_val[packed[i] & 0xfffu] + ((packed[i] >> 12) & 0x7ffffu);
                 if (at < a.list_capacity) a.tile_list[at] = slot;
@@ -325,7 +275,7 @@
     const uint32_t first = a.slot_lo + (wave_id * a.tpw + lane_id) * a.spt;
     auto in_round = [&](uint32_t si) { return has_tri && si < a.spt && first + si < a.slot_hi; };
     auto tb_of = [&](uint32_t si) { return in_round(si) ? a.slot_tb[first + si] : SWR_TB_INVALID; };
-    auto want_of = [&](uint32_t si) { return (FILL && in_round(si)) ? (uint32_t)a.want[first + si] : 0u; };
+    auto want_of = [&](uint32_t si) { return in_round(si) ? (uint32_t)a.want[first + si] : 0u; };
     unsigned long long tb = tb_of(0);
     uint32_t wm = want_of(0);
     for (uint32_t si = 0; si < a.spt; ++si) {
diff --git a/softwarerenderer_amd/csrc/swr_device.h b/softwarerenderer_amd/csrc/swr_device.h
--- a/softwarerenderer_amd/csrc/swr_device.h
+++ b/softwarerenderer_amd/csrc/swr_device.h
@@ -117,6 +117,83 @@
 __host__ __device__ __forceinline__ BandMap band_map(const FrameParams& fp) {
     BandMap b; b.ty0 = fp.band_ty0; b.ty1 = fp.band_ty1; b.il_k = fp.il_k; b.il_world = fp.il_world; b.il_rank = fp.il_rank;
     return b;
+}
+
+__host__ __device__ __forceinline__ uint32_t rec_index(uint32_t slot, uint32_t odd_base) {
+    if (odd_base == 0u) return slot;
+    return (slot & 1u) ? odd_base + (slot >> 1) : (slot >> 1);
+}
+__host__ __device__ __forceinline__ uint32_t record_odd_base(uint64_t triangles) { return (uint32_t)((triangles + 1u) & ~(uint64_t)1u); }
+
+__device__ __forceinline__ bool pair_may_cover(const float sx[3], const float sy[3], int minX, int maxX, int minY, int maxY,
+                                               int tx, int ty, int width, int height, bool is_line) {
+    if (is_line) return true;
+    const int x0 = tx * SWR_TILE, y0 = ty * SWR_TILE;
+    const int startX = max(minX, x0), endX = min(maxX, min(x0 + SWR_TILE - 1, width - 1));
+    const int startY = max(minY, y0), endY = min(maxY, min(y0 + SWR_TILE - 1, height - 1));
+    if (startX > endX || startY > endY) return false;
+    const float ea[3] = { sy[1] - sy[2], sy[2] - sy[0], sy[0] - sy[1] };
+    const float eb[3] = { sx[2] - sx[1], sx[0] - sx[2], sx[1] - sx[0] };
+    const float rx[3] = { sx[1], sx[2], sx[0] };
+    const float ry[3] = { sy[1], sy[2], sy[0] };
+    const float fxs = (float)startX, fxe = (float)endX, fys = (float)startY, fye = (float)endY;
+    const float lim = 1.0e15f;
+    const bool tame = fabsf(sx[0]) < lim && fabsf(sx[1]) < lim && fabsf(sx[2]) < lim && fabsf(sy[0]) < lim && fabsf(sy[1]) < lim && fabsf(sy[2]) < lim;
+    if (!tame) return true;
+    bool any_neg = false, any_pos = false;
+#pragma unroll
+    for (int k = 0; k < 3; ++k) {
+        const float a = ea[k], b = eb[k];
+        const float dxs = fxs - rx[k], dxe = fxe - rx[k], dys = fys - ry[k], dye = fye - ry[k];
+        const float ax_s = a * dxs, ax_e = a * dxe, by_s = b * dys, by_e = b * dye;
+        const float emax = fmaxf(ax_s, ax_e) + fmaxf(by_s, by_e);
+        const float emin = fminf(ax_s, ax_e) + fminf(by_s, by_e);
+        const float m = fabsf(a) * fmaxf(fabsf(dxs), fabsf(dxe)) + fabsf(b) * fmaxf(fabsf(dys), fabsf(dye));
+        const float delta = m * (64.0f / 16777216.0f);
+        any_neg = any_neg || emax < -delta;
+        any_pos = any_pos || emin > delta;
+    }
+    return !(any_neg && any_pos);
+}
+
+struct SlotTiles { int tminx, tminy, nx, ny; };
+__device__ __forceinline__ bool slot_tiles(const BandMap& band, unsigned long long tb, SlotTiles& s) {
+    s.tminx = s.tminy = s.nx = s.ny = 0;
+    if (tb == SWR_TB_INVALID) return false;
+    s.tminx = (int)(tb & 0xffff);
+    const int tmaxx = (int)((tb >> 16) & 0xffff);
+    s.tminy = max((int)((tb >> 32) & 0xffff), band.ty0);
+    const int tmaxy = min((int)((tb >> 48) & 0xffff), band.ty1 - 1);
+    s.nx = tmaxx - s.tminx + 1;
+    s.ny = tmaxy - s.tminy + 1;
+    if (s.ny <= 0) { s.nx = 0; s.ny = 0; return false; }
+    return true;
+}
+#define SWR_SMALL_TILES 8
+struct SmallTileWalk {
+    int tx, ty, x_lo, x_end;
+    __device__ __forceinline__ explicit SmallTileWalk(const SlotTiles& s) : tx(s.tminx), ty(s.tminy), x_lo(s.tminx), x_end(s.tminx + s.nx) {}
+    __device__ __forceinline__ void next() { ++tx; if (tx >= x_end) { tx = x_lo; ++ty; } }
+};
+__device__ __forceinline__ uint32_t small_want_mask(const BandMap& band, unsigned long long tb, const float sx[3], const float sy[3],
+                                                    int minX, int maxX, int minY, int maxY, int width, int height, bool is_line) {
+    SlotTiles st;
+    if (!slot_tiles(band, tb, st)) return 0u;
+    const int nt = st.nx * st.ny;
+    if (nt > SWR_SMALL_TILES) return 0u;
+    uint32_t mask = 0u;
+    SmallTileWalk w(st);
+#pragma unroll 1
+    for (int i0 = 0; i0 < nt; i0 += 2) {
+#pragma unroll
+        for (int j = 0; j < 2; ++j) {
+            const int i = i0 + j;
+            const bool want = i < nt && band_local_row(band, w.ty) >= 0 && pair_may_cover(sx, sy, minX, maxX, minY, maxY, w.tx, w.ty, width, height, is_line);
+            mask |= want ? (1u << i) : 0u;
+            w.next();
+        }
+    }
+    return mask;
 }
 
 __device__ __forceinline__ bool is_neg_bits(float f) { return (__float_as_uint(f) >> 31) != 0u; }
diff --git a/softwarerenderer_amd/csrc/swr_flush.h b/softwarerenderer_amd/csrc/swr_flush.h
--- a/softwarerenderer_amd/csrc/swr_flush.h
+++ b/softwarerenderer_amd/csrc/swr_flush.h
@@ -83,11 +83,15 @@
     int mode;
     bool cc, cd;
     UploadLayout up = {};
+    uint32_t odd_base = 0;
 };
 
 static bool b_needs_vnorm(const Batch& b) { return !b.draws.empty() && kernel_class(b.draws[0].p.program) != 0; }
 static bool b_has_user_program(const Batch& b) { return !b.draws.empty() && b.draws[0].p.program >= SWR_PROG_USER_BASE; }
 static bool b_has_user_vertex(const Batch& b) { return b_has_user_program(b) && b.draws[0].prog && b.draws[0].prog->vertex_fn; }
+#ifndef SWR_DENSE_RECORDS
+#define SWR_DENSE_RECORDS 1
+#endif
 const unsigned long long kMaxPairs = 1ull << 30;
 
 size_t pair_capacity(const swr_context* c) {
@@ -139,10 +143,11 @@
     BinArgs ba;
     ba.slot_tb = c->d_slot_tb.as<unsigned long long>();
     ba.recs = S.d_recs.as<TriRec>();
+    ba.odd_base = P.odd_base;
     ba.slot_lo = lo; ba.slot_hi = hi;
     ba.spt = b.wireframe ? 6u : 2u;
     ba.width = c->W; ba.height = c->H;
-    ba.tiles_x = c->tiles_x; ba.band_ty0 = c->band_ty0; ba.band_ty1 = c->band_ty1;
+    ba.tiles_x = c->tiles_x;
     ba.band = host_band_map(c);
     ba.tile_count = S.d_tile_count.as<uint32_t>();
     ba.tile_start = S.d_tile_start.as<uint32_t>();
@@ -214,6 +219,7 @@
         ScopedSpan sp(c, ST_COVER, F);
         CoverArgs ca;
         ca.recs = S.d_recs.as<TriRec>();
+        ca.odd_base = P.odd_base;
         ca.tile_list = c->d_tile_list.as<uint32_t>();
         ca.pair_tile = c->d_pair_tile.as<uint32_t>();
         ca.masks = S.d_masks.as<uint4>();
@@ -370,12 +376,14 @@
         VOut* a_pool = S.d_vout.as<VOut>() + g.V;
         uint32_t a_pool_base = (uint32_t)g.V;
         TriRec* a_recs = S.d_recs.as<TriRec>();
+        uint32_t a_odd_base = P.odd_base;
         unsigned long long* a_tb = c->d_slot_tb.as<unsigned long long>();
+        uint8_t* a_want = c->d_want.as<uint8_t>();
         Counters* a_counters = c->d_counters.as<Counters>();
         const Ctrl* a_ctrl = c->d_ctrl.as<Ctrl>();
         uint32_t a_seq = b.seq;
         int a_count = count_stats, a_wire = b.wireframe ? 1 : 0;
-        void* args[] = { &d_draws, &d_tblocks, &a_vout, &a_pool, &a_pool_base, &a_recs, &a_tb, &fp, &a_counters, &a_ctrl, &a_seq,
+        void* args[] = { &d_draws, &d_tblocks, &a_vout, &a_pool, &a_pool_base, &a_recs, &a_odd_base, &a_tb, &a_want, &fp, &a_counters, &a_ctrl, &a_seq,
                          &a_count, &a_wire, &d_visible, &a_vnorm };
         SWR_HIP(c, launch(vprog ? vprog->setup_fn : nullptr, (const void*)k_setup, g.tblocks.size(), args));
     }
@@ -418,7 +426,8 @@
     if ((rc = ensure(c, S.d_upload, P.up.bytes))) return rc;
     if ((rc = ensure(c, S.d_vout, (size_t)(V + 4 * T) * sizeof(VOut)))) return rc;
     if (b_needs_vnorm(b) && (rc = ensure(c, S.d_vnorm, S.d_vout.cap / 4))) return rc;
-    if ((rc = ensure(c, S.d_recs, (size_t)(spt * T) * sizeof(TriRec)))) return rc;
+    P.odd_base = (b.wireframe || !SWR_DENSE_RECORDS) ? 0u : record_odd_base(T);
+    if ((rc = ensure(c, S.d_recs, (size_t)(spt * T + 2) * sizeof(TriRec)))) return rc;
     if ((rc = ensure(c, c->d_slot_tb, (size_t)(spt * T) * 8))) return rc;
     if ((rc = ensure(c, c->d_want, (size_t)(spt * T) + 64))) return rc;
     if ((rc = ensure(c, S.d_tile_count, (size_t)n_tiles * 4))) return rc;
diff --git a/softwarerenderer_amd/csrc/swr_geometry.hip.h b/softwarerenderer_amd/csrc/swr_geometry.hip.h
--- a/softwarerenderer_amd/csrc/swr_geometry.hip.h
+++ b/softwarerenderer_amd/csrc/swr_geometry.hip.h
@@ -199,7 +199,8 @@
 __device__ __forceinline__ int setup_triangle(const FrameParams& fp, int cull, uint32_t draw,
                                               const SVert& v0, const SVert& v1, const SVert& v2,
                                               uint32_t r0, uint32_t r1, uint32_t r2,
-                                              TriRec* __restrict__ rec, unsigned long long* __restrict__ tb, bool wireframe,
+                                              TriRec* __restrict__ rec, unsigned long long* __restrict__ tb, uint32_t* __restrict__ wnt,
+                                              bool wireframe,
                                               float4* __restrict__ rec_regs = nullptr ) {
     const int rw = fp.width, rh = fp.height;
     const SVert* o[3] = { &v2, &v1, &v0 };
@@ -240,6 +241,7 @@
                                  __uint_as_float(flags | SWR_FLAG_LINE));
             tb[e] = (unsigned long long)(minX / SWR_TILE) | ((unsigned long long)(maxX / SWR_TILE) << 16) |
                     ((unsigned long long)(minY / SWR_TILE) << 32) | ((unsigned long long)(maxY / SWR_TILE) << 48);
+            wnt[e] = small_want_mask(band_map(fp), tb[e], sx, sy, minX, maxX, minY, maxY, rw, rh, true);
         }
         return 0;
     }
@@ -267,6 +269,7 @@
     }
     tb[0] = (unsigned long long)(minX / SWR_TILE) | ((unsigned long long)(maxX / SWR_TILE) << 16) |
             ((unsigned long long)(minY / SWR_TILE) << 32) | ((unsigned long long)(maxY / SWR_TILE) << 48);
+    wnt[0] = small_want_mask(band_map(fp), tb[0], sx, sy, minX, maxX, minY, maxY, rw, rh, false);
     return 1;
 }
 
@@ -277,7 +280,9 @@
                                                VOut* __restrict__ clip_pool,
                                                uint32_t clip_pool_base,
                                                TriRec* __restrict__ recs,
+                                               uint32_t odd_base,
                                                unsigned long long* __restrict__ slot_tb,
+                                               uint8_t* __restrict__ want,
                                                FrameParams fp,
                                                Counters* __restrict__ counters ,
                                                const Ctrl* __restrict__ ctrl, uint32_t seq, int count_stats, int wireframe,
@@ -304,6 +309,7 @@
         const uint32_t per_fan = wireframe ? 3u : 1u;
         const uint32_t slot = 2u * per_fan * gt;
         unsigned long long tbs[6] = { SWR_TB_INVALID, SWR_TB_INVALID, SWR_TB_INVALID, SWR_TB_INVALID, SWR_TB_INVALID, SWR_TB_INVALID };
+        uint32_t wnt[6] = { 0u, 0u, 0u, 0u, 0u, 0u };
 
         const uint16_t* __restrict__ ip = dp->idx + 3u * local;
         const uint32_t r0 = dp->vert_base + ip[0], r1 = dp->vert_base + ip[1], r2 = dp->vert_base + ip[2];
@@ -372,23 +378,24 @@
                     if (vnorm) for (int k = 0; k < n; ++k) vnorm[pbase + (uint32_t)k] = make_float4(poly[k].nrm[0], poly[k].nrm[1], poly[k].nrm[2], 0.0f);
 #endif
                     n_setup += setup_triangle(fp, dp->cull, SWR_FRAG_DRAW(dp, bm), poly[0], poly[1], poly[2],
-                                              pbase, pbase + 1, pbase + 2, recs + slot, &tbs[0], wireframe != 0);
+                                              pbase, pbase + 1, pbase + 2, recs + rec_index(slot, odd_base), &tbs[0], &wnt[0], wireframe != 0);
                     if (n == 4) n_setup += setup_triangle(fp, dp->cull, SWR_FRAG_DRAW(dp, bm), poly[0], poly[2], poly[3],
-                                                          pbase, pbase + 2, pbase + 3, recs + slot + per_fan, &tbs[3], wireframe != 0);
+                                                          pbase, pbase + 2, pbase + 3, recs + rec_index(slot + per_fan, odd_base), &tbs[3], &wnt[3], wireframe != 0);
                 }
             } else {
                 if (!wireframe) {
-                    rec_valid = setup_triangle(fp, dp->cull, SWR_FRAG_DRAW(dp, bm), v[0], v[1], v[2], r0, r1, r2, recs + slot, &tbs[0], false, rec_q) != 0;
+                    rec_valid = setup_triangle(fp, dp->cull, SWR_FRAG_DRAW(dp, bm), v[0], v[1], v[2], r0, r1, r2, nullptr, &tbs[0], &wnt[0], false, rec_q) != 0;
                     n_setup += rec_valid ? 1u : 0u;
                 } else
-                n_setup += setup_triangle(fp, dp->cull, SWR_FRAG_DRAW(dp, bm), v[0], v[1], v[2], r0, r1, r2, recs + slot, &tbs[0], wireframe != 0);
+                n_setup += setup_triangle(fp, dp->cull, SWR_FRAG_DRAW(dp, bm), v[0], v[1], v[2], r0, r1, r2, recs + rec_index(slot, odd_base), &tbs[0], &wnt[0], wireframe != 0);
             }
         }
         if (wireframe) {
 #pragma unroll
-            for (int k = 0; k < 6; ++k) slot_tb[slot + k] = tbs[k];
+            for (int k = 0; k < 6; ++k) { slot_tb[slot + k] = tbs[k]; want[slot + k] = (uint8_t)wnt[k]; }
         } else {
             *reinterpret_cast<ulonglong2*>(slot_tb + slot) = make_ulonglong2(tbs[0], tbs[3]);
+            *reinterpret_cast<uint16_t*>(want + slot) = (uint16_t)(wnt[0] | (wnt[3] << 8));
         }
     }
 
@@ -402,11 +409,12 @@
             sw[4 * lane + 0] = rec_q[0]; sw[4 * lane + 1] = rec_q[1]; sw[4 * lane + 2] = rec_q[2]; sw[4 * lane + 3] = rec_q[3];
             __builtin_amdgcn_fence(__ATOMIC_ACQ_REL, "workgroup");
             __builtin_amdgcn_wave_barrier();
-            float4* dst = reinterpret_cast<float4*>(recs + 2u * (size_t)(dp->tri_base + bm.first + wv * 64u));
+            const uint32_t slot0 = 2u * (dp->tri_base + bm.first + wv * 64u);
+            float4* dst = reinterpret_cast<float4*>(recs);
 #pragma unroll
             for (int k = 0; k < 4; ++k) {
                 const uint32_t e = (uint32_t)k * 64u + lane, j = e >> 2;
-                if ((vmask >> j) & 1ull) dst[8u * j + (e & 3u)] = sw[e];
+                if ((vmask >> j) & 1ull) dst[4u * (size_t)rec_index(slot0 + 2u * j, odd_base) + (e & 3u)] = sw[e];
             }
         }
     }
diff --git a/softwarerenderer_amd/csrc/swr_raster_c.hip.h b/softwarerenderer_amd/csrc/swr_raster_c.hip.h
--- a/softwarerenderer_amd/csrc/swr_raster_c.hip.h
+++ b/softwarerenderer_amd/csrc/swr_raster_c.hip.h
@@ -43,6 +43,7 @@
 
 struct CoverArgs {
     const TriRec* __restrict__ recs;
+    uint32_t odd_base;
     const uint32_t* __restrict__ tile_list;
     const uint32_t* __restrict__ pair_tile;
     uint4* __restrict__ masks;
@@ -90,10 +91,11 @@
             s_rows[threadIdx.x][2] = (uint16_t)tile; s_rows[threadIdx.x][3] = (uint16_t)(tile >> 16);
             const int tx = (int)(tile % (uint32_t)a.fp.tiles_x), ty = band_global_row(band_map(a.fp), (int)(tile / (uint32_t)a.fp.tiles_x));
             const int x0 = tx * SWR_TILE, y0 = ty * SWR_TILE;
-            const float4 r3 = reinterpret_cast<const float4*>(a.recs + slot)[3];
+            const uint32_t ri = rec_index(slot, a.odd_base);
+            const float4 r3 = reinterpret_cast<const float4*>(a.recs + ri)[3];
             {
-                const float2 r2zw = reinterpret_cast<const float2*>(a.recs + slot)[5];
-                a.refs[p_own] = make_uint4(slot, __float_as_uint(r2zw.x), __float_as_uint(r2zw.y), __float_as_uint(r3.x));
+                const float2 r2zw = reinterpret_cast<const float2*>(a.recs + ri)[5];
+                a.refs[p_own] = make_uint4(ri, __float_as_uint(r2zw.x), __float_as_uint(r2zw.y), __float_as_uint(r3.x));
             }
             const uint32_t bbx = __float_as_uint(r3.y), bby = __float_as_uint(r3.z);
             const int w = min((int)(bbx >> 16), min(x0 + SWR_TILE - 1, a.fp.width - 1)) - max((int)(bbx & 0xffffu), x0) + 1;
@@ -148,7 +150,7 @@
         const int tx = (int)(tile % (uint32_t)a.fp.tiles_x), ty = band_global_row(band_map(a.fp), (int)(tile / (uint32_t)a.fp.tiles_x));
         const int x0 = tx * SWR_TILE, y0 = ty * SWR_TILE;
         const int tile_end_x = min(x0 + SWR_TILE - 1, a.fp.width - 1), tile_end_y = min(y0 + SWR_TILE - 1, a.fp.height - 1);
-        const float4* __restrict__ rq = reinterpret_cast<const float4*>(a.recs + slot);
+        const float4* __restrict__ rq = reinterpret_cast<const float4*>(a.recs + rec_index(slot, a.odd_base));
         const float4 r0 = rq[0], r1 = rq[1], r2 = rq[2], r3 = rq[3];
         const float s0x = r0.x, s1x = r0.y, s2x = r0.z, s0y = r0.w, s1y = r1.x, s2y = r1.y;
         const uint32_t bbx = __float_as_uint(r3.y), bby = __float_as_uint(r3.z);
```

Result: faster. 78000 Mfragments/s (median of 6 runs) (+4.6%).
